# maxgillett/tinysplat

Measured on AMD Instinct MI355X. Metric: Gaussians*pixels/s fwd+bwd, higher is better.
Workload: dtype f32; 1 GPU; 1000000 random Gaussians, SH degree 3, 1920x1080, fwd+bwd (RGB), BASELINE configs[2]; max_per_tile=614, parallelism=single GPU, tile_lists=16x16 (gsplat's) (auto), gaussian_order=as generated (i.i.d.)

## Files before the change

### include/tinysplat_hip.h

```cpp
#ifndef TINYSPLAT_HIP_H
#define TINYSPLAT_HIP_H

#include <stdint.h>

#ifdef __cplusplus
extern "C" {
#endif

#define TS_ABI_VERSION 8

#define TS_E_BADARG (-1)
#define TS_E_DEGREE (-2)

#define TS_TILE 16
#define TS_SPLAT_RECORD_FLOATS 12
#define TS_PARTIAL_ROW_FLOATS 12

int ts_abi_version(void);

typedef struct ts_camera {
    float fx, fy, cx, cy;
    int32_t img_width, img_height;
    int32_t tile_bounds_x, tile_bounds_y;
    int32_t tile_row0, tile_rows;
    float glob_scale;
    float clip_thresh;
    int32_t wide_tiles;
    int32_t hints;
} ts_camera;
#define TS_HINT_BALANCED_WALK 1
#define TS_HINT_COOP_SPLIT (1 << 20)
#define TS_CAM_LIST_SEGMENTS(s) (((s) & 15) << 8)
#define TS_CAM_WHOLE_TILES(w16) (((w16) & 15) << 12)
#define TS_CAM_COOP_TILES(c16) (((c16) & 15) << 16)
int64_t ts_final_floats(const ts_camera* cam_host, int32_t channels);
int32_t ts_cut_tiles(const ts_camera* cam_host, int32_t* band, int32_t* whole);
int32_t ts_num_tiles(const ts_camera* cam_host);


#define TS_PROJECT_LOG_SCALES 1
#define TS_PROJECT_RAW_QUATS 2

int ts_project_fwd(int32_t n, const float* means3d, const float* scales, const float* quats,
                   const float* viewmat, const float* projmat, const ts_camera* cam_host,
                   int32_t flags, float* xys, float* depths, int32_t* radii, float* conics,
                   int32_t* num_tiles_hit, float* cov3d, void* stream);

int ts_project_bwd(int32_t n, const float* means3d, const float* scales, const float* quats,
                   const float* viewmat, const float* projmat, const ts_camera* cam_host,
                   int32_t flags, const int32_t* radii, const float* v_xy, const float* v_depth,
                   const float* v_conic, const float* v_cov3d,
                   float* v_means3d, float* v_scales, float* v_quats, void* stream);


int ts_sh_fwd(int32_t n, int32_t degrees_to_use, int32_t num_bases, const float* viewdirs,
              const float* coeffs, float* colors, void* stream);

int ts_sh_bwd(int32_t n, int32_t degrees_to_use, int32_t num_bases, const float* viewdirs,
              const float* v_colors, float* v_coeffs, void* stream);

int ts_sh_colors_fwd(int32_t n, int32_t degrees_to_use, int32_t num_bases, const float* means3d,
                     const float* origin, const float* colors_dc, const float* colors_rest,
                     float* colors, uint8_t* clamp_mask, const int32_t* live, void* stream);
int ts_sh_colors_bwd(int32_t n, int32_t degrees_to_use, int32_t num_bases, const float* means3d,
                     const float* origin, const uint8_t* clamp_mask, const float* v_colors,
                     float* v_colors_dc, float* v_colors_rest, void* stream);
int ts_colors_pack_fwd(int32_t n, int32_t degrees_to_use, int32_t num_bases, const float* means3d,
                       const float* origin, const float* colors_dc, const float* colors_rest,
                       uint8_t* clamp_mask, const int32_t* live, int32_t channels, int32_t flags,
                       const float* xys, const int32_t* radii, const float* conics, const float* opacity,
                       const int32_t* cum_tiles_hit, const ts_camera* cam_host, const float* depths,
                       float* splats, void* stream);


int64_t ts_scan_ws_ints(int32_t n);
int ts_scan_tiles(int32_t n, const int32_t* num_tiles_hit, int32_t* cum_tiles_hit,
                  int32_t* scan_ws, int32_t* total_out, void* stream);

int64_t ts_bin_ws_ints(int32_t n, int32_t num_tiles);

int ts_bin_count(int32_t n, const float* xys, const int32_t* radii, const float* splats,
                 const ts_camera* cam_host, int32_t* bin_ws, void* stream);

int ts_tile_offsets(int32_t n, int32_t num_tiles, int32_t* bin_ws, int32_t* tile_bins,
                    const int32_t* cum_tiles_hit, int64_t capacity, void* stream);
int ts_tile_offsets_stats(int32_t n, int32_t num_tiles, int32_t* bin_ws, int32_t* tile_bins,
                          const int32_t* cum_tiles_hit, int64_t capacity, int32_t* longest_list, void* stream);

int ts_bin_scatter(int32_t n, const float* xys, const int32_t* radii, const float* splats,
                   const ts_camera* cam_host, const int32_t* bin_ws, int32_t* bucket_ids, int32_t* scratch,
                   void* stream);

int ts_sort_tiles(int32_t num_tiles, const int32_t* tile_bins, const float* depths,
                  const int32_t* bucket_ids, int32_t* gaussian_ids_sorted, int32_t* sort_ws,
                  int32_t* zeroed_counter, void* stream);
int ts_sort_tiles_above(int32_t num_tiles, const int32_t* tile_bins, const float* depths,
                        const int32_t* bucket_ids, int32_t* gaussian_ids_sorted, int32_t* sort_ws,
                        int32_t* zeroed_counter, void* stream);

int32_t ts_bin_group_form(int32_t n);
int ts_bin_count_groups(int32_t n, const float* xys, const int32_t* radii, const float* splats,
                        const ts_camera* cam_host, int32_t* bin_ws, void* stream);
int ts_group_offsets(int32_t n, int32_t num_tiles, int32_t* bin_ws, int32_t* tile_bins,
                     const int32_t* cum_tiles_hit, int64_t capacity, int32_t* longest_list, void* stream);
int ts_bin_scatter_groups(int32_t n, const float* xys, const int32_t* radii, const float* splats,
                          const ts_camera* cam_host, int32_t* bin_ws, int32_t* tile_bins, int32_t* bucket_ids,
                          int32_t* scratch, void* stream);
int32_t ts_bin_one_walk_form(int32_t n, int32_t num_tiles);
int32_t ts_bin_stage_capacity(void);
int ts_bin_emit_groups(int32_t n, const float* xys, const int32_t* radii, const float* splats,
                       const ts_camera* cam_host, const int32_t* cum_tiles_hit, int64_t capacity, int32_t* bin_ws,
                       int32_t* scratch, void* stream);
int ts_emit_offsets(int32_t n, int32_t num_tiles, int32_t* bin_ws, int32_t* tile_bins,
                    const int32_t* cum_tiles_hit, int64_t capacity, int32_t* longest_list, void* stream);
int ts_bin_gather_groups(int32_t n, int32_t num_tiles, int32_t* bin_ws, int32_t* tile_bins, int32_t* bucket_ids,
                         const int32_t* scratch, void* stream);
int ts_sort_tiles_stats(int32_t num_tiles, const int32_t* tile_bins, const float* depths,
                        const int32_t* bucket_ids, int32_t* gaussian_ids_sorted, int32_t* sort_ws,
                        int32_t* zeroed_counter, int32_t n, const int32_t* bin_ws, int32_t* longest_list,
                        void* stream);
int ts_sort_tiles_above_stats(int32_t num_tiles, const int32_t* tile_bins, const float* depths,
                              const int32_t* bucket_ids, int32_t* gaussian_ids_sorted, int32_t n,
                              const int32_t* bin_ws, int32_t* longest_list, void* stream);

#define TS_RASTER_LOGIT_OPACITY 1

int ts_pack_splats(int32_t n, int32_t channels, int32_t flags, const float* xys, const int32_t* radii,
                   const float* conics, const float* colors, const float* opacity,
                   const int32_t* cum_tiles_hit, const ts_camera* cam_host, const float* depths,
                   float* splats, void* stream);

#define TS_RASTER_CLAMP_RGB 2
#define TS_RASTER_SPLIT_BLOCKS 4
#define TS_RASTER_NARROW_WAVES 8
#define TS_RASTER_FLAG_GEN(g) (((g) & 0xff) << 8)
int ts_raster_fwd(int32_t channels, int32_t flags, const ts_camera* cam_host, const int32_t* tile_bins,
                  const int32_t* gaussian_ids_sorted, const float* splats, const float* background,
                  float* out_img, float* final_Ts, int32_t* final_index, uint8_t* clamp_mask,
                  void* stream);
int ts_raster_fwd_planes(int32_t channels, int32_t flags, const ts_camera* cam_host, const int32_t* tile_bins,
                         const int32_t* gaussian_ids_sorted, const float* splats, const float* background,
                         float* out_img, float* out_depth, float* final_Ts, int32_t* final_index,
                         uint8_t* clamp_mask, void* stream);

int ts_raster_fwd_sort(int32_t channels, int32_t flags, const ts_camera* cam_host, const int32_t* tile_bins,
                       const int32_t* bucket_ids, const float* depths, int32_t* gaussian_ids_sorted,
                       const float* splats, const float* background, float* out_img, float* out_depth,
                       float* final_Ts, int32_t* final_index, uint8_t* clamp_mask, void* stream);

int ts_raster_bwd(int32_t channels, int32_t flags, int64_t num_intersects, const ts_camera* cam_host,
                  const int32_t* tile_bins, const int32_t* gaussian_ids_sorted, const float* splats,
                  const float* background, const float* final_Ts, const int32_t* final_index,
                  const float* v_out_img, const float* v_out_alpha, const uint8_t* clamp_mask,
                  float* partials, uint8_t* row_flags, void* stream);
int ts_raster_bwd_planes(int32_t channels, int32_t flags, int64_t num_intersects, const ts_camera* cam_host,
                         const int32_t* tile_bins, const int32_t* gaussian_ids_sorted, const float* splats,
                         const float* background, const float* final_Ts, const int32_t* final_index,
                         const float* v_out_img, const float* v_out_depth, int32_t planes,
                         const float* v_out_alpha, const uint8_t* clamp_mask,
                         float* partials, uint8_t* row_flags, void* stream);

int ts_reduce_partials(int32_t n, int32_t channels, int32_t flags, const int32_t* num_tiles_hit,
                       const int32_t* cum_tiles_hit, const float* partials,
                       const uint8_t* row_flags, const float* splats, float* v_xy, float* v_conic,
                       float* v_colors, float* v_opacity, float* v_depth, const uint8_t* color_mask,
                       void* stream);

#define TS_FRAME_TIGHT 1
#define TS_FRAME_SPLIT 2
#define TS_FRAME_NARROW_WAVES 8
#define TS_FRAME_DIRECT_SCATTER 32
#define TS_FRAME_PLANES 64
#define TS_FRAME_LIST_STATS 256
#define TS_FRAME_SEPARATE_SORT 128
#define TS_FRAME_STRIPE 16
#define TS_FRAME_GROUP_COUNTS 1024
#define TS_FRAME_ONE_WALK 2048
#define TS_FRAME_SURVIVORS 512
typedef struct ts_frame {
    int32_t n, num_bases, sh_degree, channels, flags;
    int32_t flag_gen;
    ts_camera cam;
    const float *means, *scales, *quats, *opacities, *colors_dc, *colors_rest;
    const float *view34, *projview, *origin, *background;
    float *xys, *depths, *conics, *colors, *splats;
    int32_t *radii, *num_tiles_hit, *cum_tiles_hit;
    uint8_t* sh_mask;
    int32_t *scan_ws, *bin_ws, *tile_bins;
    int32_t* total_host;
    int64_t num_intersects;
    int64_t capacity;
    int32_t *bucket_ids, *gaussian_ids_sorted;
    float *out_img, *final_Ts;
    int32_t* final_index;
    uint8_t* clamp_mask;
    const float* v_out_img;
    float* partials;
    uint8_t* row_flags;
    float *v_xy, *v_conic, *v_colors, *v_depth, *v_opacity;
    float *v_means, *v_scales, *v_quats, *v_colors_dc, *v_colors_rest;
    float* out_depth;
    const float* v_out_depth;
    int32_t* survivors;
} ts_frame;
int32_t ts_frame_struct_bytes(void);
int ts_frame_fwd_project(const ts_frame* f, void* stream);
int ts_frame_fwd_prepare(const ts_frame* f, void* stream);
int ts_frame_fwd_composite(const ts_frame* f, void* stream);
int ts_frame_bwd_composite(const ts_frame* f, void* stream);
int ts_frame_bwd_params(const ts_frame* f, void* stream);

typedef void (*ts_entry_probe)(const char* entry, int32_t end, void* user);
int ts_set_entry_probe(ts_entry_probe fn, void* user);

#define TS_MAX_RANKS 16
#define TS_EXPORT_RECORD_FLOATS 16
typedef struct ts_stripes {
    int32_t num;
    int32_t row[TS_MAX_RANKS + 1];
} ts_stripes;
int64_t ts_route_ws_ints(int32_t n, int32_t num_ranks);
int ts_route_count(int32_t n, const float* xys, const int32_t* radii, const ts_camera* cam_host,
                   const ts_stripes* stripes_host, int32_t* route_ws, int32_t* counts, void* stream);
int ts_route_count_padded(int32_t n, const float* xys, const int32_t* radii, const ts_camera* cam_host,
                          const ts_stripes* stripes_host, const int32_t* group_base_host, int32_t* route_ws,
                          int32_t* counts, void* stream);
int ts_route_pack(int32_t n, int32_t gid_base, const float* xys, const int32_t* radii, const float* depths,
                  const float* splats, const ts_camera* cam_host, const ts_stripes* stripes_host,
                  const int32_t* route_ws, float* records, void* stream);
int ts_import_records(int32_t m, const float* records, const ts_camera* cam_host, float* xys, float* depths,
                      int32_t* radii, int32_t* num_tiles_hit, void* stream);
int ts_import_pack(int32_t m, const float* records, const int32_t* cum_tiles_hit, const ts_camera* cam_host,
                   float* splats, void* stream);
int ts_reduce_partials_rows(int32_t n, int32_t channels, int32_t flags, const int32_t* num_tiles_hit,
                            const int32_t* cum_tiles_hit, const float* partials, const uint8_t* row_flags,
                            const float* splats, float* grad_rows, void* stream);
int ts_route_accumulate(int32_t n, int32_t channels, const float* xys, const int32_t* radii, const float* splats,
                        const uint8_t* color_mask, const ts_camera* cam_host, const ts_stripes* stripes_host,
                        const int32_t* route_ws, const float* grad_rows, float* v_xy, float* v_conic,
                        float* v_colors, float* v_depth, float* v_opacity, void* stream);

int ts_shard_owner_fwd(const ts_frame* fo, const ts_stripes* stripes_host, int32_t* route_ws, int32_t* counts,
                       void* stream);
int ts_shard_owner_fwd_padded(const ts_frame* fo, const ts_stripes* stripes_host, const int32_t* group_base_host,
                              int32_t* route_ws, int32_t* counts, void* stream);
int ts_shard_owner_fwd_fused(int32_t n, int32_t degrees_to_use, int32_t num_bases, const float* means3d,
                             const float* scales, const float* quats, const float* view34, const float* projview,
                             const ts_camera* cam_host, int32_t project_flags, const float* origin,
                             const float* colors_dc, const float* colors_rest, const float* opacity, int32_t channels,
                             int32_t raster_flags, float* xys, float* depths, int32_t* radii, float* conics,
                             int32_t* num_tiles_hit, uint8_t* clamp_mask, float* splats, const ts_stripes* stripes_host,
                             const int32_t* group_base_host, int32_t* route_ws, int32_t* counts, void* stream);
int ts_shard_owner_bwd_fused(int32_t n, int32_t channels, int32_t degrees_to_use, int32_t num_bases, const float* means3d,
                             const float* scales, const float* quats, const float* view34, const float* projview,
                             const float* origin, const float* xys, const int32_t* radii, const float* splats,
                             const uint8_t* color_mask, const ts_camera* cam_host, const ts_stripes* stripes_host,
                             const int32_t* route_ws, const float* grad_rows, float* v_xy, float* v_conic,
                             float* v_colors, float* v_depth, float* v_opacity, float* v_colors_dc, float* v_colors_rest,
                             float* v_means3d, float* v_scales, float* v_quats, void* stream);
int ts_shard_stripe_fwd_import(const ts_frame* fs, const float* records, void* stream);
int ts_shard_stripe_bwd(const ts_frame* fs, float* grad_rows, void* stream);
int ts_shard_owner_bwd(const ts_frame* fo, const ts_stripes* stripes_host, const int32_t* route_ws,
                       const float* grad_rows, void* stream);

typedef struct ts_rank_step {
    ts_stripes stripes;
    int32_t group_base[TS_MAX_RANKS + 1];
    int32_t gid_base;
    int32_t send_rows, recv_rows;
    int32_t* route_ws;
    int32_t* counts;
    float *send, *recv;
    float *grad_rows, *back;
} ts_rank_step;
int32_t ts_rank_step_struct_bytes(void);
int ts_shard_rank_fwd_a(const ts_frame* fo, const ts_rank_step* r, void* stream);
int ts_shard_rank_fwd_b(const ts_frame* fs, const ts_rank_step* r, void* stream);
int ts_shard_rank_bwd_a(const ts_frame* fs, const ts_rank_step* r, void* stream);
int ts_shard_rank_bwd_b(const ts_frame* fo, const ts_rank_step* r, void* stream);


int64_t ts_photometric_ws_floats(int32_t height, int32_t width);
int ts_photometric_loss_rgbd(int32_t height, int32_t width, int32_t pixel_floats, const float* image,
                             const float* target, const float* depth_target, float w_l1,
                             float w_ssim, float w_depth, float* ws, float* v_image, void* stream);
int ts_photometric_loss(int32_t height, int32_t width, const float* image, const float* target,
                        float w_l1, float w_ssim, float* ws, float* v_image, void* stream);
int ts_photometric_loss_planes(int32_t height, int32_t width, const float* image, const float* depth,
                               const float* target, const float* depth_target, float w_l1, float w_ssim,
                               float w_depth, float* ws, float* v_image, float* v_depth, void* stream);
int ts_photometric_loss_reduce(int32_t height, int32_t width, float w_l1, float w_ssim, float w_depth,
                               const float* ws, float* out4, void* stream);

#define TS_ADAM_MAX_TENSORS 8
int ts_adam_step(int32_t num_tensors, float* const* params_host, const float* const* grads_host,
                 float* const* exp_avg_host, float* const* exp_avg_sq_host, const int64_t* numel_host,
                 const float* lr_host, const int32_t* steps_host, float beta1, float beta2, float eps,
                 void* stream);

#define TS_ADAM_MEANS 0
#define TS_ADAM_COLORS_DC 1
#define TS_ADAM_COLORS_REST 2
#define TS_ADAM_SCALES 3
#define TS_ADAM_QUATS 4
#define TS_ADAM_OPACITIES 5
typedef struct ts_adam {
    float* exp_avg[6];
    float* exp_avg_sq[6];
    float lr[6];
    int32_t step[6];
    float beta1, beta2, eps;
} ts_adam;
int ts_sh_colors_bwd_adam(int32_t n, int32_t degrees_to_use, int32_t num_bases, const float* means3d,
                          const float* origin, const uint8_t* clamp_mask, const float* v_colors,
                          float* colors_dc, float* colors_rest, const ts_adam* adam_host, void* stream);
int ts_project_bwd_adam(int32_t n, float* means3d, float* scales, float* quats, const float* viewmat,
                        const float* projmat, const ts_camera* cam_host, int32_t flags, const int32_t* radii,
                        const float* v_xy, const float* v_depth, const float* v_conic, float* opacities,
                        const float* v_opacity, const ts_adam* adam_host, void* stream);
int ts_frame_bwd_params_adam(const ts_frame* f, const ts_adam* adam_host, void* stream);

#define TS_DENSIFY_CLONE 1
#define TS_DENSIFY_SPLIT 2
#define TS_DENSIFY_PRUNE 4

typedef struct ts_densify_policy {
    float interval_densify;
    float max_dim;
    float tau_means;
    float scale_thresh;
} ts_densify_policy;

int ts_grad_accum(int32_t n, const float* v_xy, float* accum, void* stream);

int ts_densify_classify(int32_t n, const float* accum, const float* scales, const float* opacities,
                        const ts_densify_policy* policy, uint8_t* flags, void* stream);

int64_t ts_densify_ws_ints(int32_t n);
int ts_densify_plan(int32_t n, const uint8_t* flags, int32_t* ws, int32_t* counts, int32_t* src_of,
                    void* stream);

#define TS_GATHER_MAX_TENSORS 8
int ts_gather_rows(int32_t num_tensors, const float* const* src_host, float* const* dst_host,
                   const int32_t* row_floats_host, int32_t dst_rows, int32_t copy_rows,
                   const int32_t* src_of, void* stream);

int ts_split_fixup(int32_t rows, const int32_t* src_of_split, const float* means, const float* scales,
                   const float* quats, const float* z, float* means_out, float* scales_out,
                   void* stream);

int32_t ts_ply_row_floats(int32_t k_rest);
int ts_ply_pack_rows(int32_t n, int32_t k_rest, const float* means, const float* colors_dc,
                     const float* colors_rest, const float* opacities, const float* scales,
                     const float* quats, float* rows, void* stream);
int ts_ply_unpack_rows(int32_t n, int32_t k_rest, const float* rows, float* means, float* colors_dc,
                       float* colors_rest, float* opacities, float* scales, float* quats,
// ... 171 lines not shown
```

### tinysplat_amd/_lib.py

```python
from __future__ import annotations

import ctypes
import os
from ctypes import POINTER, c_double, c_float, c_int32, c_int64, c_void_p
from pathlib import Path

LIB_PATH = Path(os.environ["TS_LIB_PATH"]) if os.environ.get("TS_LIB_PATH") else \
    Path(__file__).resolve().parent / "csrc" / "libtinysplat_hip.so"
ABI_VERSION = 8
HINT_BALANCED_WALK = 1
HINT_COOP_SPLIT = 1 << 20
RASTER_LOGIT_OPACITY = 1
RASTER_CLAMP_RGB = 2
RASTER_SPLIT_BLOCKS = 4
RASTER_NARROW_WAVES = 8
FRAME_TIGHT = 1
FRAME_SPLIT = 2
FRAME_NARROW_WAVES = 8
FRAME_STRIPE = 16
FRAME_DIRECT_SCATTER = 32
FRAME_PLANES = 64
FRAME_SEPARATE_SORT = 128
FRAME_LIST_STATS = 256
FRAME_SURVIVORS = 512
FRAME_GROUP_COUNTS = 1024
FRAME_ONE_WALK = 2048
PARTIAL_ROW_FLOATS = 12


class TsCamera(ctypes.Structure):
    _fields_ = [
        ("fx", c_float), ("fy", c_float), ("cx", c_float), ("cy", c_float),
        ("img_width", c_int32), ("img_height", c_int32),
        ("tile_bounds_x", c_int32), ("tile_bounds_y", c_int32),
        ("tile_row0", c_int32), ("tile_rows", c_int32),
        ("glob_scale", c_float), ("clip_thresh", c_float),
        ("wide_tiles", c_int32), ("hints", c_int32),
    ]


_P = c_void_p
_CAM = POINTER(TsCamera)


class TsDensifyPolicy(ctypes.Structure):
    _fields_ = [("interval_densify", c_float), ("max_dim", c_float), ("tau_means", c_float),
                ("scale_thresh", c_float)]


class TsFrame(ctypes.Structure):
    _fields_ = ([("n", c_int32), ("num_bases", c_int32), ("sh_degree", c_int32), ("channels", c_int32),
                 ("flags", c_int32), ("flag_gen", c_int32), ("cam", TsCamera)]
                + [(name, c_void_p) for name in (
                    "means", "scales", "quats", "opacities", "colors_dc", "colors_rest",
                    "view34", "projview", "origin", "background",
                    "xys", "depths", "conics", "colors", "splats",
                    "radii", "num_tiles_hit", "cum_tiles_hit", "sh_mask",
                    "scan_ws", "bin_ws", "tile_bins", "total_host")]
                + [("num_intersects", c_int64), ("capacity", c_int64)]
                + [(name, c_void_p) for name in (
                    "bucket_ids", "gaussian_ids_sorted", "out_img", "final_Ts", "final_index", "clamp_mask",
                    "v_out_img", "partials", "row_flags",
                    "v_xy", "v_conic", "v_colors", "v_depth", "v_opacity",
                    "v_means", "v_scales", "v_quats", "v_colors_dc", "v_colors_rest",
                    "out_depth", "v_out_depth", "survivors")])


_FRAME = POINTER(TsFrame)


class TsAdam(ctypes.Structure):
    _fields_ = [("exp_avg", c_void_p * 6), ("exp_avg_sq", c_void_p * 6), ("lr", c_float * 6), ("step", c_int32 * 6),
                ("beta1", c_float), ("beta2", c_float), ("eps", c_float)]


_ADAM = POINTER(TsAdam)

MAX_RANKS = 16


class TsStripes(ctypes.Structure):
    _fields_ = [("num", c_int32), ("row", c_int32 * (MAX_RANKS + 1))]


_STRIPES = POINTER(TsStripes)


class TsRankStep(ctypes.Structure):
    _fields_ = [("stripes", TsStripes), ("group_base", c_int32 * (MAX_RANKS + 1)), ("gid_base", c_int32),
                ("send_rows", c_int32), ("recv_rows", c_int32), ("route_ws", c_void_p), ("counts", c_void_p),
                ("send", c_void_p), ("recv", c_void_p), ("grad_rows", c_void_p), ("back", c_void_p)]


_RANK = POINTER(TsRankStep)

TSDF_NO_CULL = 1
TSDF_PLANES = 6


class TsTsdfCamera(ctypes.Structure):
    _fields_ = [("view", c_float * 12), ("proj", c_float * 12), ("planes", c_float * (TSDF_PLANES * 5)),
                ("width", c_int32), ("height", c_int32), ("depth", c_void_p)]

ENTRY_PROBE = ctypes.CFUNCTYPE(None, ctypes.c_char_p, c_int32, c_void_p)

SIGNATURES = {
    "ts_abi_version": (c_int32, []),
    "ts_project_fwd": (c_int32, [c_int32, _P, _P, _P, _P, _P, _CAM, c_int32, _P, _P, _P, _P, _P, _P, _P]),
    "ts_project_bwd": (c_int32, [c_int32, _P, _P, _P, _P, _P, _CAM, c_int32, _P, _P, _P, _P, _P, _P, _P, _P, _P]),
    "ts_sh_fwd": (c_int32, [c_int32, c_int32, c_int32, _P, _P, _P, _P]),
    "ts_sh_bwd": (c_int32, [c_int32, c_int32, c_int32, _P, _P, _P, _P]),
    "ts_sh_colors_fwd": (c_int32, [c_int32, c_int32, c_int32, _P, _P, _P, _P, _P, _P, _P, _P]),
    "ts_sh_colors_bwd": (c_int32, [c_int32, c_int32, c_int32, _P, _P, _P, _P, _P, _P, _P]),
    "ts_scan_ws_ints": (c_int64, [c_int32]),
    "ts_scan_tiles": (c_int32, [c_int32, _P, _P, _P, _P, _P]),
    "ts_bin_ws_ints": (c_int64, [c_int32, c_int32]),
    "ts_bin_count": (c_int32, [c_int32, _P, _P, _P, _CAM, _P, _P]),
    "ts_tile_offsets": (c_int32, [c_int32, c_int32, _P, _P, _P, c_int64, _P]),
    "ts_tile_offsets_stats": (c_int32, [c_int32, c_int32, _P, _P, _P, c_int64, _P, _P]),
    "ts_bin_scatter": (c_int32, [c_int32, _P, _P, _P, _CAM, _P, _P, _P, _P]),
    "ts_sort_tiles": (c_int32, [c_int32, _P, _P, _P, _P, _P, _P, _P]),
    "ts_sort_tiles_above": (c_int32, [c_int32, _P, _P, _P, _P, _P, _P, _P]),
    "ts_bin_group_form": (c_int32, [c_int32]),
    "ts_bin_count_groups": (c_int32, [c_int32, _P, _P, _P, _CAM, _P, _P]),
    "ts_group_offsets": (c_int32, [c_int32, c_int32, _P, _P, _P, c_int64, _P, _P]),
    "ts_bin_scatter_groups": (c_int32, [c_int32, _P, _P, _P, _CAM, _P, _P, _P, _P, _P]),
    "ts_bin_one_walk_form": (c_int32, [c_int32, c_int32]),
    "ts_bin_stage_capacity": (c_int32, []),
    "ts_bin_emit_groups": (c_int32, [c_int32, _P, _P, _P, _CAM, _P, c_int64, _P, _P, _P]),
    "ts_emit_offsets": (c_int32, [c_int32, c_int32, _P, _P, _P, c_int64, _P, _P]),
    "ts_bin_gather_groups": (c_int32, [c_int32, c_int32, _P, _P, _P, _P, _P]),
    "ts_sort_tiles_stats": (c_int32, [c_int32, _P, _P, _P, _P, _P, _P, c_int32, _P, _P, _P]),
    "ts_sort_tiles_above_stats": (c_int32, [c_int32, _P, _P, _P, _P, c_int32, _P, _P, _P]),
    "ts_num_tiles": (c_int32, [_CAM]),
    "ts_final_floats": (c_int64, [_CAM, c_int32]),
    "ts_cut_tiles": (c_int32, [_CAM, _P, _P]),
    "ts_colors_pack_fwd": (c_int32, [c_int32, c_int32, c_int32, _P, _P, _P, _P, _P, _P, c_int32, c_int32,
                                     _P, _P, _P, _P, _P, _CAM, _P, _P, _P]),
    "ts_pack_splats": (c_int32, [c_int32, c_int32, c_int32, _P, _P, _P, _P, _P, _P, _CAM, _P, _P, _P]),
    "ts_raster_fwd": (c_int32, [c_int32, c_int32, _CAM, _P, _P, _P, _P, _P, _P, _P, _P, _P]),
    "ts_raster_bwd": (c_int32, [c_int32, c_int32, c_int64, _CAM, _P, _P, _P, _P, _P, _P, _P, _P, _P, _P, _P, _P]),
    "ts_raster_fwd_planes": (c_int32, [c_int32, c_int32, _CAM, _P, _P, _P, _P, _P, _P, _P, _P, _P, _P]),
    "ts_raster_fwd_sort": (c_int32, [c_int32, c_int32, _CAM, _P, _P, _P, _P, _P, _P, _P, _P, _P, _P, _P, _P]),
    "ts_raster_bwd_planes": (c_int32, [c_int32, c_int32, c_int64, _CAM, _P, _P, _P, _P, _P, _P, _P, _P, c_int32,
                                       _P, _P, _P, _P, _P]),
    "ts_bench_stream_read": (c_int32, [_P, c_int64, _P, _P]),
    "ts_bench_gather48": (c_int32, [_P, _P, c_int64, _P, _P]),
    "ts_photometric_ws_floats": (c_int64, [c_int32, c_int32]),
    "ts_photometric_loss": (c_int32, [c_int32, c_int32, _P, _P, c_float, c_float, _P, _P, _P]),
    "ts_photometric_loss_rgbd": (c_int32, [c_int32, c_int32, c_int32, _P, _P, _P, c_float, c_float, c_float, _P, _P, _P]),
    "ts_photometric_loss_planes": (c_int32, [c_int32, c_int32, _P, _P, _P, _P, c_float, c_float, c_float, _P, _P, _P,
                                             _P]),
    "ts_photometric_loss_reduce": (c_int32, [c_int32, c_int32, c_float, c_float, c_float, _P, _P, _P]),
    "ts_adam_step": (c_int32, [c_int32, _P, _P, _P, _P, _P, _P, _P, c_float, c_float, c_float, _P]),
    "ts_sh_colors_bwd_adam": (c_int32, [c_int32, c_int32, c_int32, _P, _P, _P, _P, _P, _P, _ADAM, _P]),
    "ts_project_bwd_adam": (c_int32, [c_int32, _P, _P, _P, _P, _P, _CAM, c_int32, _P, _P, _P, _P, _P, _P, _ADAM, _P]),
    "ts_frame_bwd_params_adam": (c_int32, [_FRAME, _ADAM, _P]),
    "ts_grad_accum": (c_int32, [c_int32, _P, _P, _P]),
    "ts_densify_classify": (c_int32, [c_int32, _P, _P, _P, POINTER(TsDensifyPolicy), _P, _P]),
    "ts_densify_ws_ints": (c_int64, [c_int32]),
    "ts_densify_plan": (c_int32, [c_int32, _P, _P, _P, _P, _P]),
    "ts_gather_rows": (c_int32, [c_int32, _P, _P, _P, c_int32, c_int32, _P, _P]),
    "ts_split_fixup": (c_int32, [c_int32, _P, _P, _P, _P, _P, _P, _P, _P]),
    "ts_ply_row_floats": (c_int32, [c_int32]),
    "ts_ply_pack_rows": (c_int32, [c_int32, c_int32, _P, _P, _P, _P, _P, _P, _P, _P]),
    "ts_ply_unpack_rows": (c_int32, [c_int32, c_int32, _P, _P, _P, _P, _P, _P, _P, _P]),
    "ts_reduce_partials": (c_int32, [c_int32, c_int32, c_int32, _P, _P, _P, _P, _P, _P, _P, _P, _P, _P, _P, _P]),
    "ts_route_ws_ints": (c_int64, [c_int32, c_int32]),
    "ts_route_count": (c_int32, [c_int32, _P, _P, _CAM, _STRIPES, _P, _P, _P]),
    "ts_route_count_padded": (c_int32, [c_int32, _P, _P, _CAM, _STRIPES, _P, _P, _P, _P]),
    "ts_route_pack": (c_int32, [c_int32, c_int32, _P, _P, _P, _P, _CAM, _STRIPES, _P, _P, _P]),
    "ts_import_records": (c_int32, [c_int32, _P, _CAM, _P, _P, _P, _P, _P]),
    "ts_import_pack": (c_int32, [c_int32, _P, _P, _CAM, _P, _P]),
    "ts_reduce_partials_rows": (c_int32, [c_int32, c_int32, c_int32, _P, _P, _P, _P, _P, _P, _P]),
    "ts_route_accumulate": (c_int32, [c_int32, c_int32, _P, _P, _P, _P, _CAM, _STRIPES, _P, _P, _P, _P, _P, _P, _P, _P]),
    "ts_shard_owner_fwd": (c_int32, [_FRAME, _STRIPES, _P, _P, _P]),
    "ts_shard_owner_fwd_padded": (c_int32, [_FRAME, _STRIPES, _P, _P, _P, _P]),
    "ts_shard_owner_fwd_fused": (c_int32, [c_int32, c_int32, c_int32, _P, _P, _P, _P, _P, _CAM, c_int32, _P, _P, _P, _P,
                                           c_int32, c_int32, _P, _P, _P, _P, _P, _P, _P, _STRIPES, _P, _P, _P, _P]),
    "ts_shard_owner_bwd_fused": (c_int32, [c_int32, c_int32, c_int32, c_int32, _P, _P, _P, _P, _P, _P, _P, _P, _P, _P,
                                           _CAM, _STRIPES, _P, _P, _P, _P, _P, _P, _P, _P, _P, _P, _P, _P, _P]),
    "ts_shard_stripe_fwd_import": (c_int32, [_FRAME, _P, _P]),
    "ts_shard_stripe_bwd": (c_int32, [_FRAME, _P, _P]),
    "ts_shard_owner_bwd": (c_int32, [_FRAME, _STRIPES, _P, _P, _P]),
    "ts_rank_step_struct_bytes": (c_int32, []),
    "ts_shard_rank_fwd_a": (c_int32, [_FRAME, _RANK, _P]),
    "ts_shard_rank_fwd_b": (c_int32, [_FRAME, _RANK, _P]),
    "ts_shard_rank_bwd_a": (c_int32, [_FRAME, _RANK, _P]),
    "ts_shard_rank_bwd_b": (c_int32, [_FRAME, _RANK, _P]),
    "ts_frame_struct_bytes": (c_int32, []),
    "ts_frame_fwd_project": (c_int32, [_FRAME, _P]),
    "ts_frame_fwd_prepare": (c_int32, [_FRAME, _P]),
    "ts_frame_fwd_composite": (c_int32, [_FRAME, _P]),
    "ts_frame_bwd_composite": (c_int32, [_FRAME, _P]),
    "ts_frame_bwd_params": (c_int32, [_FRAME, _P]),
    "ts_set_entry_probe": (c_int32, [_P, _P]),
    "ts_knn_ws_bytes": (c_int64, [c_int32, c_int32, c_int32]),
    "ts_knn": (c_int32, [c_int32, _P, c_int32, _P, c_int32, _P, _P, _P, _P, _P]),
    "ts_init_from_points": (c_int32, [c_int32, c_int32, _P, _P, _P, _P, _P, _P, _P, _P, _P, _P, _P, _P, _P, _P]),
    "ts_opacity_entropy_ws_bytes": (c_int64, [c_int32]),
    "ts_opacity_entropy": (c_int32, [c_int32, _P, _P, _P, _P, _P]),
    "ts_density_sample_ws_bytes": (c_int64, [c_int32]),
    "ts_density_sample": (c_int32, [c_int32, c_int32, c_int32, _P, _P, _P, _P, _P, _P, _P, _P, _P, _P, _P]),
    "ts_density_loss_ws_bytes": (c_int64, [c_int32]),
    "ts_density_loss": (c_int32, [c_int32, c_int32, _P, _P, _P, _P, _P, _P, _P, _P, c_int32, c_int32, _P, _P, c_int32,
                                  c_float, _P, _P, _P, _P, _P, _P, _P, _P, _P, _P]),
    "ts_segment_sum_ws_bytes": (c_int64, [c_int64, c_int32]),
    "ts_segment_sum": (c_int32, [c_int64, c_int32, c_int32, _P, _P, _P, _P, _P, _P, _P]),
    "ts_extract_pack": (c_int32, [c_int32, _P, _P, _P, _P, _P, _P, _P]),
    "ts_extract_rays": (c_int32, [c_int32, _P, c_int32, c_int32, _P, c_int32, _P, _P, _P, _P, _P, _P]),
    "ts_extract_samples": (c_int32, [c_int32, c_int32, c_int32, c_float, _P, _P, _P, _P, _P, _P, _P]),
    "ts_extract_march": (c_int32, [c_int32, c_int32, c_int32, c_float, c_float, _P, _P, _P, _P, _P, _P, _P, _P, _P, _P,
                                   _P, _P, _P]),
    "ts_extract_normals": (c_int32, [c_int32, c_int32, _P, _P, _P, _P, _P]),
    "ts_extract_chunk_bytes": (c_int64, [c_int32, c_int32, c_int32]),
    "ts_mesh_boxes": (c_int32, [c_int32, _P, _P, _P, c_float, _P, _P]),
    "ts_mesh_mark": (c_int32, [c_int32, _P, _P, _P, _P, _P]),
    "ts_mesh_chunk_bytes": (c_int64, [c_int32, c_int32]),
    "ts_mesh_corners": (c_int32, [c_int32, _P, _P, _P, _P, _P]),
    "ts_mesh_density": (c_int32, [c_int32, c_int32, _P, _P, _P, _P, _P, _P, _P, _P]),
    "ts_mesh_count": (c_int32, [c_int32, _P, _P, _P, c_float, _P, _P, _P]),
    "ts_mesh_emit": (c_int32, [c_int32, _P, _P, _P, c_float, _P, _P, _P, _P, _P, _P]),
    "ts_tsdf_camera_bytes": (c_int32, []),
    "ts_tsdf_mark": (c_int32, [c_int32, _P, c_int64, _P, _P, c_float, c_float, _P, _P]),
    "ts_tsdf_chunk_bytes": (c_int64, [c_int32]),
    "ts_tsdf_integrate": (c_int32, [c_int32, _P, _P, _P, _P, c_int32, c_int32, c_float, c_float, c_float, c_int32, _P, _P,
                                    _P]),
    "ts_tsdf_field": (c_int32, [c_int32, _P, _P, c_int32, _P, _P]),
    "ts_mesh_count_observed": (c_int32, [c_int32, _P, _P, _P, c_float, _P, _P, _P]),
    "ts_mesh_emit_observed": (c_int32, [c_int32, _P, _P, _P, c_float, _P, _P, _P, _P, _P, _P]),
    "ts_field_colors": (c_int32, [c_int32, c_int32, _P, _P, _P, _P, _P, _P, c_int32, c_int32, _P, _P]),
    "ts_simplify_count": (c_int32, [c_int32, c_int32, _P, _P, _P, _P, _P, _P]),
    "ts_simplify_keys": (c_int32, [c_int32, _P, _P, _P, _P, _P]),
    "ts_simplify_ws_bytes": (c_int64, [c_int64]),
    "ts_simplify_accumulate": (c_int32, [c_int32, c_int32, c_int32, _P, _P, _P, _P, c_int32, c_int64, _P, _P, c_int64,
                                         c_int64, _P, _P, _P]),
    "ts_simplify_solve": (c_int32, [c_int32, _P, _P, _P, _P, _P, c_double, _P, _P]),
    "ts_simplify_faces": (c_int32, [c_int32, c_int32, _P, _P, _P, _P, _P]),
    "ts_clean_degenerate": (c_int32, [c_int32, _P, _P, _P]),
    "ts_clean_edge_keys": (c_int32, [c_int32, c_int32, _P, _P, _P]),
    "ts_clean_face_weights": (c_int32, [c_int32, c_int32, _P, _P, _P, _P]),
    "ts_clean_mark": (c_int32, [c_int32, c_int64, _P, _P, _P, _P]),
    "ts_clean_components": (c_int32, [c_int32, c_int32, _P, _P, _P, _P]),
    "ts_splat_keys": (c_int32, [c_int32, _P, _P, _P, _P]),
    "ts_splat_pack": (c_int32, [c_int32, c_int32, _P, _P, _P, _P, _P, _P, _P, _P]),
    "ts_splat_unpack": (c_int32, [c_int32, _P, _P, _P, _P, _P, _P, _P]),
    "ts_undistort_image": (c_int32, [_P, c_int32, c_int32, POINTER(c_float), POINTER(c_float), POINTER(c_float),
                                     c_int32, c_int32, c_int32, _P, _P]),
    "ts_jpeg_ws_bytes": (c_int64, [c_int32, c_int32, c_int32, c_int32]),
    "ts_jpeg_max_bytes": (c_int64, [c_int32, c_int32, c_int32, c_int32]),
    "ts_jpeg_header": (c_int64, [c_int32, c_int32, c_int32, c_int32, c_int32, _P, c_int64]),
    "ts_jpeg_encode": (c_int32, [_P, c_int32, c_int32, c_int32, c_int32, c_int32, c_int32, c_int32, _P, _P, c_int64, _P,
                                 _P, _P]),
    "ts_image_metrics_ws_bytes": (c_int64, [c_int32, c_int32]),
    "ts_image_metrics": (c_int32, [c_int32, c_int32, c_int32, _P, _P, c_int32, _P, _P, _P]),
    "ts_depth_prior_project": (c_int32, [c_int32, c_int64, c_int64, _P, _P, _P, _P, _P, _P, _P, _P, _P, _P]),
    "ts_depth_prior_mark": (c_int32, [c_int64, _P, _P, _P]),
    "ts_depth_prior_gather": (c_int32, [c_int64, _P, _P, _P, _P, _P, _P, _P, _P, _P, _P, _P, _P, _P, _P]),
    "ts_depth_prior_fit": (c_int32, [c_int32, _P, _P, _P, _P, c_int32, _P, _P]),
    "ts_depth_prior_apply": (c_int32, [_P, c_int32, c_int32, c_int32, c_int32, _P, c_int32, _P, _P]),
    "ts_label_votes": (c_int32, [c_int32, _CAM, _P, _P, _P, _P, _P, c_int32, _P, _P]),
    "ts_votes_labels": (c_int32, [c_int32, c_int32, _P, c_double, _P, _P, _P]),
}

_lib = None


class HipLibraryError(RuntimeError):
    pass


def load() -> ctypes.CDLL:
    global _lib
    if _lib is not None:
        return _lib
    if not LIB_PATH.exists():
        raise HipLibraryError(
            f"{LIB_PATH} is missing: tinysplat_amd has no CPU or PyTorch fallback. "
            "Build it with `python -m tinysplat_amd._build` (needs hipcc, targets gfx950).")
    stamp = LIB_PATH.with_suffix(LIB_PATH.suffix + ".flags")
    if stamp.exists() and "-DTS_" in stamp.read_text() and os.environ.get("TS_ALLOW_VARIANT_LIB") != "1":
        raise HipLibraryError(
            f"{LIB_PATH} was built with developer -DTS_* overrides (ablation variant; its results may be "
            "wrong). Rebuild with `python -m tinysplat_amd._build`, or set TS_ALLOW_VARIANT_LIB=1.")
    lib = ctypes.CDLL(str(LIB_PATH))
    for name, (res, args) in SIGNATURES.items():
        try:
            fn = getattr(lib, name)
        except AttributeError as e:
            raise HipLibraryError(f"{LIB_PATH} does not export {name}") from e
        fn.restype = res
# ... 23 lines not shown
```

### tinysplat_amd/csrc/binning.hip

```cpp
#include <hip/hip_runtime.h>

#include "../../include/tinysplat_hip.h"
#include "host_util.h"
#include "pack.h"
#include "splat_math.h"

namespace {

constexpr int kThreads = 256;
constexpr int kScanItems = 4;
constexpr int kScanBlock = kThreads * kScanItems;

__device__ __forceinline__ int wave_inclusive_scan(int v) {
    const int lane = threadIdx.x & 63;
#pragma unroll
    for (int d = 1; d < 64; d <<= 1) {
        const int u = __shfl_up(v, d, 64);
        if (lane >= d) v += u;
    }
    return v;
}

template <int WAVES = 4>
__device__ __forceinline__ int block_inclusive_scan(int v, int* total) {
    __shared__ int wave_sums[WAVES];
    const int lane = threadIdx.x & 63, wave = threadIdx.x >> 6;
    int inc = wave_inclusive_scan(v);
    if (lane == 63) wave_sums[wave] = inc;
    __syncthreads();
    int add = 0, tot = 0;
#pragma unroll
    for (int w = 0; w < WAVES; ++w) {
        const int s = wave_sums[w];
        if (w < wave) add += s;
        tot += s;
    }
    *total = tot;
    __syncthreads();
    return inc + add;
}

__global__ __launch_bounds__(kThreads) void scan_local_kernel(int n, const int* __restrict__ in,
                                                              int* __restrict__ out,
                                                              int* __restrict__ block_sums,
                                                              int* __restrict__ total_out) {
    const int base = blockIdx.x * kScanBlock + threadIdx.x * kScanItems;
    int v[kScanItems];
    int sum = 0;
#pragma unroll
    for (int k = 0; k < kScanItems; ++k) {
        v[k] = (base + k < n) ? in[base + k] : 0;
        sum += v[k];
        v[k] = sum;
    }
    int total;
    const int inc = block_inclusive_scan(sum, &total);
    const int excl = inc - sum;
#pragma unroll
    for (int k = 0; k < kScanItems; ++k)
        if (base + k < n) {
            out[base + k] = v[k] + excl;
            if (total_out && gridDim.x == 1 && base + k == n - 1)
                __hip_atomic_store(total_out, v[k] + excl, __ATOMIC_RELEASE, __HIP_MEMORY_SCOPE_SYSTEM);
        }
    if (threadIdx.x == 0) block_sums[blockIdx.x] = total;
}

__global__ __launch_bounds__(kThreads) void scan_add_kernel(int n, int* __restrict__ out,
                                                            const int* __restrict__ block_sums,
                                                            int* __restrict__ total_out) {
    __shared__ int red[kThreads / 64];
    int part = 0;
    for (int j = threadIdx.x; j < (int)blockIdx.x; j += kThreads) part += block_sums[j];
#pragma unroll
    for (int d = 32; d >= 1; d >>= 1) part += __shfl_xor(part, d, 64);
    if ((threadIdx.x & 63) == 0) red[threadIdx.x >> 6] = part;
    __syncthreads();
    int add = 0;
#pragma unroll
    for (int w = 0; w < kThreads / 64; ++w) add += red[w];
    const int base = blockIdx.x * kScanBlock + threadIdx.x * kScanItems;
#pragma unroll
    for (int k = 0; k < kScanItems; ++k)
        if (base + k < n) {
            const int v = out[base + k] + add;
            if (blockIdx.x != 0) out[base + k] = v;
            if (total_out && base + k == n - 1)
                __hip_atomic_store(total_out, v, __ATOMIC_RELEASE, __HIP_MEMORY_SCOPE_SYSTEM);
        }
}

#ifndef TS_BIN_THREADS
#define TS_BIN_THREADS 1024
#endif
constexpr int kBinThreads = TS_BIN_THREADS;
#ifndef TS_BIN_CHUNK
#define TS_BIN_CHUNK 4096
#endif
constexpr int kBinChunkMin = TS_BIN_CHUNK;
constexpr int kBinMaxChunks = 512;
constexpr int kBinWindowMax = 36864;
constexpr int kBinTargetBlocks = 1;

__host__ __device__ inline int bin_num_chunks(int n) {
    int per = n / 192;
    per = per < 1024 ? 1024 : (per > kBinChunkMin ? kBinChunkMin : per);
    int b = (n + per - 1) / per;
    if (b < 1) b = 1;
    if (b > kBinMaxChunks) b = kBinMaxChunks;
    return b;
}

inline int bin_window_tiles(int n, int num_tiles) {
    const int chunks = bin_num_chunks(n);
    int nwin = (kBinTargetBlocks + chunks - 1) / chunks;
    const int max_win = (num_tiles + 255) / 256;
    if (nwin > max_win) nwin = max_win;
    if (nwin < 1) nwin = 1;
    int window = (num_tiles + nwin - 1) / nwin;
    window = (window + 63) & ~63;
    if (window > kBinWindowMax) window = kBinWindowMax;
    return window;
}

using ts::TightTest;

#ifndef TS_BIN_PRE
#define TS_BIN_PRE 2
#endif
constexpr int kBinPre = TS_BIN_PRE;
template <typename Emit>
__device__ __forceinline__ void walk_chunk(int g0, int g1, const float* __restrict__ xys,
                                           const int* __restrict__ radii,
                                           const float4* __restrict__ splats, const ts_camera& cam,
                                           Emit emit) {
    const int ws = cam.wide_tiles ? 1 : 0;
    const int tbx = (cam.tile_bounds_x + ws) >> ws;
    const bool tight_lists = splats != nullptr;
    for (int base = g0 + threadIdx.x; base < g1; base += kBinPre * kBinThreads) {
        int r[kBinPre];
        float2 xy[kBinPre];
        float4 q0[kBinPre], q1[kBinPre];
#pragma unroll
        for (int u = 0; u < kBinPre; ++u) {
            const int i = base + u * kBinThreads;
            r[u] = i < g1 ? radii[i] : 0;
        }
#pragma unroll
        for (int u = 0; u < kBinPre; ++u) {
            const int i = base + u * kBinThreads;
            xy[u] = make_float2(0.f, 0.f);
            q0[u] = q1[u] = make_float4(0.f, 0.f, 0.f, 0.f);
            if (r[u] > 0) {
                xy[u] = reinterpret_cast<const float2*>(xys)[i];
                if (tight_lists) { q0[u] = splats[3 * (size_t)i]; q1[u] = splats[3 * (size_t)i + 1]; }
            }
        }
// ... 471 lines not shown
struct PassRanks {
    unsigned int r[(ITEMS + 1) / 2];
    __device__ __forceinline__ PassRanks() {
#pragma unroll
        for (int u = 0; u < (ITEMS + 1) / 2; ++u) r[u] = 0u;
    }
    __device__ __forceinline__ void set(int u, int v) { r[u / 2] |= (unsigned int)v << (16 * (u & 1)); }
    __device__ __forceinline__ int get(int u) const { return (int)((r[u / 2] >> (16 * (u & 1))) & 0xffffu); }
};

template <int ITEMS, typename Load>
__device__ __forceinline__ void place_pass(FineGroup& sh, unsigned int* buf, int m, Load load, bool publish,
                                           const GroupLists& g, int* __restrict__ bucket_ids) {
    static_assert(ITEMS * kFineThreads <= 65536, "16-bit ranks inside a pass");
    const int tid = threadIdx.x;
    unsigned int w[ITEMS];
    PassRanks<ITEMS> rank;
#pragma unroll
    for (int u = 0; u < ITEMS; ++u) {
        const int k = u * kFineThreads + tid;
        if (k < m) w[u] = load(k);
    }
#pragma unroll
    for (int u = 0; u < ITEMS; ++u) {
        const int k = u * kFineThreads + tid;
        if (k < m) rank.set(u, atomicAdd(&sh.hist[w[u] >> kCoarseIdBits], 1));
    }
    __syncthreads();
    if (tid < 64) {
        int c;
        const int ex = scan_lists(sh.hist, tid, c);
        if (publish) publish_lists(sh, g, tid, c, ex);
        if (tid < kCoarseTiles) {
            sh.loff[tid] = ex;
            sh.gbase[tid] = sh.cursor[tid];
            sh.cursor[tid] += c;
            sh.hist[tid] = 0;
        }
    }
    __syncthreads();
#pragma unroll
    for (int u = 0; u < ITEMS; ++u) {
        const int k = u * kFineThreads + tid;
        if (k < m) buf[sh.loff[w[u] >> kCoarseIdBits] + rank.get(u)] = w[u];
    }
    __syncthreads();
#pragma unroll
    for (int u = 0; u < ITEMS; ++u) {
        const int k = u * kFineThreads + tid;
        if (k < m) {
            const unsigned int e = buf[k];
            const int t = (int)(e >> kCoarseIdBits);
            bucket_ids[sh.gbase[t] + (k - sh.loff[t])] = (int)(e & kCoarseIdMask);
        }
    }
    __syncthreads();
}

__global__ __launch_bounds__(kFineThreads) void bin_scatter_fine_kernel(int num_tiles,
                                                                        const int* __restrict__ tile_start,
                                                                        const int* __restrict__ scratch,
                                                                        int* __restrict__ bucket_ids) {
    __shared__ FineGroup sh;
    __shared__ unsigned int buf[kFinePass];
    const int t0 = blockIdx.x << kCoarseShift, t1 = min(num_tiles, t0 + kCoarseTiles);
    if ((int)threadIdx.x < t1 - t0) sh.cursor[threadIdx.x] = tile_start[t0 + threadIdx.x];
    const int begin = tile_start[t0], end = tile_start[t1];
    if ((int)threadIdx.x < kCoarseTiles) sh.hist[threadIdx.x] = 0;
    __syncthreads();
    for (int c0 = begin; c0 < end; c0 += kFinePass)
        place_pass<kFineAhead>(sh, buf, min(kFinePass, end - c0),
                               [&](int k) { return (unsigned int)scratch[c0 + k]; }, false, GroupLists{}, bucket_ids);
}

__global__ __launch_bounds__(kFineThreads) void bin_scatter_fine_groups_kernel(int num_tiles,
                                                                               int* __restrict__ tile_start,
                                                                               int* __restrict__ tile_bins,
                                                                               int* __restrict__ group_max,
                                                                               const int* __restrict__ scratch,
                                                                               int* __restrict__ bucket_ids) {
    if (tile_start[num_tiles + 1] != 0) return;
    __shared__ FineGroup sh;
    __shared__ unsigned int buf[kFinePass];
    const int t0 = blockIdx.x << kCoarseShift, t1 = min(num_tiles, t0 + kCoarseTiles);
    const int begin = tile_start[t0], end = tile_start[t1];
    if ((int)threadIdx.x < kCoarseTiles) {
        sh.hist[threadIdx.x] = 0;
        sh.cursor[threadIdx.x] = 0;
    }
    __syncthreads();
    const GroupLists lists{t0, t1, begin, tile_start, tile_bins, group_max};
    const bool counted = end - begin > kFinePass || end == begin;
    if (counted) {
        for (int c0 = begin; c0 < end; c0 += kFinePass) {
            const int m = min(kFinePass, end - c0);
            unsigned int w[kFineAhead];
#pragma unroll
            for (int u = 0; u < kFineAhead; ++u) {
                const int k = u * kFineThreads + (int)threadIdx.x;
                if (k < m) w[u] = (unsigned int)scratch[c0 + k];
            }
#pragma unroll
            for (int u = 0; u < kFineAhead; ++u) {
                const int k = u * kFineThreads + (int)threadIdx.x;
                if (k < m) atomicAdd(&sh.hist[w[u] >> kCoarseIdBits], 1);
            }
        }
        publish_counted(sh, lists);
    }
    for (int c0 = begin; c0 < end; c0 += kFinePass)
        place_pass<kFineAhead>(sh, buf, min(kFinePass, end - c0),
                               [&](int k) { return (unsigned int)scratch[c0 + k]; }, !counted, lists, bucket_ids);
}

#ifndef TS_STAGE_CAP
#define TS_STAGE_CAP 20480
#endif
constexpr int kStageCap = TS_STAGE_CAP;
constexpr int kEmitMaxGroups = 2048;
static_assert((size_t)kStageCap * 6 + (size_t)kEmitMaxGroups * 8 <= 144 * 1024, "LDS budget of a binning workgroup");
static_assert(kEmitMaxGroups <= 2 * kBinThreads && kEmitMaxGroups <= 65536, "two groups per thread, 16-bit group index");
static_assert(kEmitMaxGroups <= kGoLdsGroups, "the offsets launch keeps the column totals in LDS");

struct BinGeometry {
    int chunks, chunk, groups;
    long long tile_start, guard, spare;
    long long group_totals, group_max;
    long long counts, starts, col_total, rows_end;
};
inline BinGeometry bin_geometry(int n, int num_tiles) {
    const long long nt = num_tiles < 0 ? 0 : num_tiles;
    BinGeometry g;
    g.chunks = bin_num_chunks(n);
    g.chunk = n > 0 ? (n + g.chunks - 1) / g.chunks : 1;
    g.groups = (int)((nt + kCoarseTiles - 1) >> kCoarseShift);
    const long long rows = (long long)g.chunks * g.groups;
    g.tile_start = g.chunks * nt;
    g.guard = g.tile_start + nt + 1;
    g.spare = g.guard + 1;
    g.group_totals = rows;
    g.group_max = nt + 1;
    g.counts = g.group_max + g.groups;
    g.starts = g.counts + rows;
    g.col_total = g.starts + rows;
    g.rows_end = g.col_total + g.groups;
    return g;
}
inline bool one_walk_form(int n, int num_tiles) {
    if (!two_hop(n) || num_tiles <= 0) return false;
    const BinGeometry g = bin_geometry(n, num_tiles);
    return g.groups <= kEmitMaxGroups && g.rows_end <= g.tile_start;
}

__global__ __launch_bounds__(kBinThreads) void bin_scatter_emit_kernel(
    int n, int chunk, const float* __restrict__ xys, const int* __restrict__ radii,
    const float4* __restrict__ splats, const ts_camera cam, int groups, const int* __restrict__ cum,
    long long capacity, int* __restrict__ counts, int* __restrict__ starts, int* __restrict__ scratch) {
    extern __shared__ int lds[];
    __shared__ int staged;
    const int g0 = min(n, (int)blockIdx.x * chunk), g1 = min(n, g0 + chunk);
    const int total = cum[n - 1];
    const int chunk_base = g0 > 0 ? cum[g0 - 1] : 0;
    const int chunk_end = g1 > g0 ? cum[g1 - 1] : chunk_base;
    int* hist = lds;
    int* cursor = lds + groups;
    unsigned int* words = reinterpret_cast<unsigned int*>(lds + 2 * groups);
    unsigned short* grp = reinterpret_cast<unsigned short*>(words + kStageCap);
    const int tid = threadIdx.x;
    for (int j = tid; j < groups; j += kBinThreads) hist[j] = 0;
    if (tid == 0) staged = 0;
    __syncthreads();
    if (total < 0 || (capacity >= 0 && (long long)total > capacity)) return;
    const int room = chunk_end - chunk_base;
    walk_chunk(g0, g1, xys, radii, splats, cam, [&](int t, int i) {
        const int g = t >> kCoarseShift;
        atomicAdd(&hist[g], 1);
        const unsigned long long m = __ballot(1);
        const int rank = (int)__builtin_amdgcn_mbcnt_hi((unsigned int)(m >> 32),
                                                        __builtin_amdgcn_mbcnt_lo((unsigned int)m, 0u));
        int base = 0;
        if (rank == 0) base = atomicAdd(&staged, (int)__popcll(m));
        base = __builtin_amdgcn_readfirstlane(base);
        const int slot = base + rank;
        if (slot < kStageCap) {
            words[slot] = (unsigned int)i | ((unsigned int)(t & (kCoarseTiles - 1)) << kCoarseIdBits);
            grp[slot] = (unsigned short)g;
        }
    });
    __syncthreads();
    const int pairs = staged;
    const bool sound = pairs <= room;
    {
        const int a = 2 * tid;
        const int h0 = a < groups ? hist[a] : 0, h1 = a + 1 < groups ? hist[a + 1] : 0;
        int all;
        const int ex = block_inclusive_scan<kBinThreads / 64>(h0 + h1, &all) - h0 - h1;
        int* crow = counts + (size_t)blockIdx.x * groups;
        int* srow = starts + (size_t)blockIdx.x * groups;
        if (a < groups) {
            cursor[a] = ex;
            crow[a] = sound ? h0 : 0;
            srow[a] = chunk_base + ex;
        }
        if (a + 1 < groups) {
            cursor[a + 1] = ex + h0;
            crow[a + 1] = sound ? h1 : 0;
            srow[a + 1] = chunk_base + ex + h0;
        }
    }
    __syncthreads();
    if (!sound) return;
    int* dst = scratch + chunk_base;
    if (pairs <= kStageCap) {
        constexpr int kPer = kStageCap / kBinThreads;
        static_assert(kStageCap % kBinThreads == 0, "whole staging rounds");
        unsigned int w[kPer];
        int at[kPer];
#pragma unroll
        for (int u = 0; u < kPer; ++u) {
            const int j = u * kBinThreads + tid;
            if (j < pairs) {
                w[u] = words[j];
                at[u] = atomicAdd(&cursor[grp[j]], 1);
            }
        }
        __syncthreads();
#pragma unroll
        for (int u = 0; u < kPer; ++u)
            if (u * kBinThreads + tid < pairs) words[at[u]] = w[u];
        __syncthreads();
#pragma unroll
        for (int u = 0; u < kPer; ++u) {
            const int j = u * kBinThreads + tid;
            if (j < pairs) dst[j] = (int)words[j];
        }
    } else {
        walk_chunk(g0, g1, xys, radii, splats, cam, [&](int t, int i) {
            dst[atomicAdd(&cursor[t >> kCoarseShift], 1)] = i | ((t & (kCoarseTiles - 1)) << kCoarseIdBits);
        });
    }
}

#ifndef TS_RUN_AHEAD
#define TS_RUN_AHEAD 20
#endif
constexpr int kRunItems = TS_RUN_AHEAD;
constexpr int kRunPass = kFineThreads * kRunItems;
#ifndef TS_RUNS_IN_FLIGHT
#define TS_RUNS_IN_FLIGHT 8
#endif
constexpr int kRunAhead = TS_RUNS_IN_FLIGHT;
__global__ __launch_bounds__(kFineThreads) void bin_scatter_fine_runs_kernel(
    int num_tiles, int groups, int chunks, const int* __restrict__ counts, const int* __restrict__ starts,
    int* __restrict__ tile_start, int* __restrict__ tile_bins, int* __restrict__ group_max,
    const int* __restrict__ scratch, int* __restrict__ bucket_ids) {
    extern __shared__ unsigned int buf[];
    const int my_count = (int)threadIdx.x < chunks ? counts[(size_t)threadIdx.x * groups + blockIdx.x] : 0;
    const int my_start = (int)threadIdx.x < chunks ? starts[(size_t)threadIdx.x * groups + blockIdx.x] : 0;
    const int begin = tile_start[min(num_tiles, (int)(blockIdx.x << kCoarseShift))];
    if (tile_start[num_tiles + 1] != 0) return;
    __shared__ FineGroup sh;
    __shared__ int roff[kBinMaxChunks + 1], rsrc[kBinMaxChunks];
    constexpr int kWaves = kFineThreads / 64;
    const int tid = threadIdx.x, lane = tid & 63, wave = tid >> 6;
    const int t0 = blockIdx.x << kCoarseShift, t1 = min(num_tiles, t0 + kCoarseTiles);
    if (tid < kCoarseTiles) {
        sh.hist[tid] = 0;
        sh.cursor[tid] = 0;
    }
    int total;
    {
        const int c = my_count;
        const int inc = block_inclusive_scan<kWaves>(c, &total);
        if (tid < chunks) {
            roff[tid] = inc - c;
            rsrc[tid] = my_start;
        }
        if (tid == 0) roff[chunks] = total;
    }
    __syncthreads();
    auto for_runs = [&](int c0, int m, auto op) {
#pragma unroll 1
        for (int b0 = wave; b0 < chunks; b0 += kWaves * kRunAhead) {
            int len[kRunAhead], src[kRunAhead], dst[kRunAhead];
            unsigned int v[kRunAhead];
#pragma unroll
            for (int u = 0; u < kRunAhead; ++u) {
                const int b = b0 + u * kWaves;
                len[u] = src[u] = dst[u] = 0;
                if (b < chunks) {
                    const int o = roff[b], c = roff[b + 1] - o;
                    const int lo = max(0, c0 - o) + lane;
                    len[u] = min(c, c0 + m - o) - lo;
                    src[u] = rsrc[b] + lo;
                    dst[u] = o - c0 + lo;
                }
            }
#pragma unroll
            for (int u = 0; u < kRunAhead; ++u)
                if (len[u] > 0) v[u] = (unsigned int)scratch[src[u]];
#pragma unroll
            for (int u = 0; u < kRunAhead; ++u)
                if (len[u] > 0) op(dst[u], v[u]);
#pragma unroll
            for (int u = 0; u < kRunAhead; ++u)
                for (int j = 64; j < len[u]; j += 64) op(dst[u] + j, (unsigned int)scratch[src[u] + j]);
        }
    };
    const GroupLists lists{t0, t1, begin, tile_start, tile_bins, group_max};
    const bool counted = total > kRunPass || total == 0;
    if (counted) {
        for_runs(0, total, [&](int, unsigned int w) { atomicAdd(&sh.hist[w >> kCoarseIdBits], 1); });
        publish_counted(sh, lists);
    }
    for (int c0 = 0; c0 < total; c0 += kRunPass) {
        const int m = min(kRunPass, total - c0);
        for_runs(c0, m, [&](int k, unsigned int w) { buf[k] = w; });
        __syncthreads();
        place_pass<kRunItems>(sh, buf, m, [&](int k) { return buf[k]; }, !counted, lists, bucket_ids);
    }
}

struct ListStats {
    const int* group_max;
    const int* guard;
    int* longest_out;
    int groups;
};
__device__ __forceinline__ void store_longest(const ListStats& st) {
    __shared__ int longest;
    if (threadIdx.x == 0) longest = 0;
    __syncthreads();
    int m = 0;
    for (int g = threadIdx.x; g < st.groups; g += kThreads) m = max(m, st.group_max[g]);
#pragma unroll
    for (int d = 32; d >= 1; d >>= 1) m = max(m, __shfl_xor(m, d, 64));
    if ((threadIdx.x & 63) == 0) atomicMax(&longest, m);
    __syncthreads();
    if (threadIdx.x == 0 && *st.guard == 0) *st.longest_out = longest;
}

constexpr int kSortCap = 4096;

#include "sort_network.h"

struct IdKeyArray {
    volatile int* ids;
    const float* depths;
};

__device__ __forceinline__ void cmpswap(IdKeyArray a, int i, int j) {
    const int x = a.ids[i], y = a.ids[j];
    if (make_key(a.depths, x) > make_key(a.depths, y)) { a.ids[i] = y; a.ids[j] = x; }
}

template <typename Ptr>
__device__ __forceinline__ void bitonic_network(Ptr a, int n) {
    int lg = 0;
    while ((1 << lg) < n) ++lg;
    const int half = (1 << lg) >> 1;
    for (int lk = 1; lk <= lg; ++lk) {
        const int k = 1 << lk, hk = k >> 1;
        for (int p = threadIdx.x; p < half; p += kThreads) {
            const int base = (p >> (lk - 1)) << lk, off = p & (hk - 1);
            const int i = base + off, j = base + k - 1 - off;
            if (j < n) cmpswap(a, i, j);
        }
        __syncthreads();
        for (int ld = lk - 2; ld >= 0; --ld) {
            const int d = 1 << ld;
            for (int p = threadIdx.x; p < half; p += kThreads) {
                const int i = ((p >> ld) << (ld + 1)) | (p & (d - 1)), j = i + d;
                if (j < n) cmpswap(a, i, j);
            }
            __syncthreads();
        }
    }
}

template <int E>
__device__ __forceinline__ void sort_tile_regs(const int* g, const float* __restrict__ depths,
                                               int* out, int n, unsigned long long* lds) {
    const int t = threadIdx.x;
    unsigned long long k[E];
#pragma unroll
    for (int e = 0; e < E; ++e) {
        const int i = t * E + e;
        k[e] = i < n ? make_key(depths, g[i]) : ~0ull;
    }
    __syncthreads();
    bitonic_regs<E, kThreads>(k, t, min(pow2_at_least(n), kThreads * E), lds);
// ... 190 lines not shown
        c0 = colors[3 * i]; c1 = colors[3 * i + 1]; c2 = colors[3 * i + 2];
        if (a.channels == 4) c3 = a.depths[i];
    }
    ts::pack_one(a, i, c0, c1, c2, c3);
}

}

extern "C" {

int32_t ts_num_tiles(const ts_camera* cam) {
    if (!cam) return 0;
    const int tbx = cam->wide_tiles ? (cam->tile_bounds_x + 1) / 2 : cam->tile_bounds_x;
    return cam->tile_rows * tbx;
}

int64_t ts_scan_ws_ints(int32_t n) {
    return n <= 0 ? 1 : (int64_t)((n + kScanBlock - 1) / kScanBlock);
}

int ts_scan_tiles(int32_t n, const int32_t* num_tiles_hit, int32_t* cum_tiles_hit,
                  int32_t* scan_ws, int32_t* total_out, void* stream) {
    if (n < 0) return TS_E_BADARG;
    if (n == 0) return 0;
    if (!num_tiles_hit || !cum_tiles_hit || !scan_ws) return TS_E_BADARG;
    hipStream_t s = (hipStream_t)stream;
    const int nb = (n + kScanBlock - 1) / kScanBlock;
    hipLaunchKernelGGL(scan_local_kernel, dim3(nb), dim3(kThreads), 0, s, n, num_tiles_hit,
                       cum_tiles_hit, scan_ws, total_out);
    if (nb > 1)
        hipLaunchKernelGGL(scan_add_kernel, dim3(nb), dim3(kThreads), 0, s, n, cum_tiles_hit, scan_ws,
                           total_out);
    return launch_status();
}

int64_t ts_bin_ws_ints(int32_t n, int32_t num_tiles) { return bin_geometry(n, num_tiles).spare + 1; }

int ts_bin_count(int32_t n, const float* xys, const int32_t* radii, const float* splats,
                 const ts_camera* cam, int32_t* bin_ws, void* stream) {
    if (n < 0 || !cam || !bin_ws) return TS_E_BADARG;
    const int nt = ts_num_tiles(cam);
    if (nt <= 0) return 0;
    if (n > 0 && (!xys || !radii)) return TS_E_BADARG;
    const BinGeometry g = bin_geometry(n, nt);
    const int window = bin_window_tiles(n, nt);
    const int windows = (nt + window - 1) / window;
    const size_t lds = (size_t)window * sizeof(int);
    if (lds > 64 * 1024)
        (void)hipFuncSetAttribute(reinterpret_cast<const void*>(&bin_count_kernel),
                                  hipFuncAttributeMaxDynamicSharedMemorySize, (int)lds);
    hipLaunchKernelGGL(bin_count_kernel, dim3(g.chunks, windows), dim3(kBinThreads), lds,
                       (hipStream_t)stream, n, g.chunk, xys, radii,
                       reinterpret_cast<const float4*>(splats), *cam, nt, window, bin_ws);
    return launch_status();
}

int ts_tile_offsets(int32_t n, int32_t num_tiles, int32_t* bin_ws, int32_t* tile_bins,
                    const int32_t* cum_tiles_hit, int64_t capacity, void* stream) {
    return ts_tile_offsets_stats(n, num_tiles, bin_ws, tile_bins, cum_tiles_hit, capacity, nullptr, stream);
}

int ts_tile_offsets_stats(int32_t n, int32_t num_tiles, int32_t* bin_ws, int32_t* tile_bins,
                          const int32_t* cum_tiles_hit, int64_t capacity, int32_t* longest_list, void* stream) {
    if (n < 0 || num_tiles < 0) return TS_E_BADARG;
    if (num_tiles == 0) return 0;
    if (!bin_ws || !tile_bins) return TS_E_BADARG;
    const BinGeometry g = bin_geometry(n, num_tiles);
    int* tile_total = bin_ws + g.tile_start;
    const int per_group = (g.chunks + kScanGroups - 1) / kScanGroups;
    hipStream_t s = (hipStream_t)stream;
    hipLaunchKernelGGL(column_scan_kernel, dim3((num_tiles + kColTiles - 1) / kColTiles),
                       dim3(kColTiles * kScanGroups), 0, s, num_tiles, g.chunks, per_group, bin_ws, tile_total, true);
    hipLaunchKernelGGL(tile_offsets_kernel, dim3(1), dim3(kOffsetsThreads), 0, s, num_tiles, tile_total,
                       tile_bins, bin_ws + g.spare,
                       (cum_tiles_hit && n > 0) ? cum_tiles_hit + (n - 1) : nullptr, (long long)capacity, longest_list);
    return launch_status();
}

int32_t ts_bin_group_form(int32_t n) { return two_hop(n) ? 1 : 0; }

int ts_bin_count_groups(int32_t n, const float* xys, const int32_t* radii, const float* splats,
                        const ts_camera* cam, int32_t* bin_ws, void* stream) {
    if (!cam || !bin_ws || !xys || !radii || !two_hop(n)) return TS_E_BADARG;
    const int nt = ts_num_tiles(cam);
    if (nt <= 0) return 0;
    const BinGeometry g = bin_geometry(n, nt);
    hipLaunchKernelGGL(group_bin_count_kernel, dim3(g.chunks), dim3(kBinThreads), (size_t)g.groups * sizeof(int),
                       (hipStream_t)stream, n, g.chunk, xys, radii, reinterpret_cast<const float4*>(splats), *cam,
                       g.groups, bin_ws);
    return launch_status();
}

}

namespace {
template <bool BASES>
int group_offsets(const BinGeometry& g, int num_tiles, int* bin_ws, int* tile_bins, const int* total_ptr,
                  long long capacity, int* longest_list, hipStream_t s) {
    int* counts = bin_ws + (BASES ? 0 : g.counts);
    int* col_total = nullptr;
    if ((long long)g.chunks * g.groups > kGoSingleMax || g.groups > kGoLdsGroups) {
        col_total = bin_ws + (BASES ? g.group_totals : g.col_total);
        const int per_group = (g.chunks + kScanGroups - 1) / kScanGroups;
        hipLaunchKernelGGL(column_scan_kernel, dim3((g.groups + kColTiles - 1) / kColTiles),
                           dim3(kColTiles * kScanGroups), 0, s, g.groups, g.chunks, per_group, counts, col_total, BASES);
        counts = nullptr;
    }
    hipLaunchKernelGGL(group_tile_offsets_kernel<BASES>, dim3(1), dim3(kGoThreads), 0, s, num_tiles, g.groups, g.chunks,
                       counts, (const int*)col_total, bin_ws + g.tile_start, tile_bins, bin_ws + g.spare, total_ptr,
                       capacity, longest_list);
    return launch_status();
}
}

extern "C" {

int ts_group_offsets(int32_t n, int32_t num_tiles, int32_t* bin_ws, int32_t* tile_bins,
                     const int32_t* cum_tiles_hit, int64_t capacity, int32_t* longest_list, void* stream) {
    if (num_tiles < 0 || !two_hop(n)) return TS_E_BADARG;
    if (num_tiles == 0) return 0;
    if (!bin_ws || !tile_bins) return TS_E_BADARG;
    return group_offsets<true>(bin_geometry(n, num_tiles), num_tiles, bin_ws, tile_bins,
                               cum_tiles_hit ? cum_tiles_hit + (n - 1) : nullptr, (long long)capacity, longest_list,
                               (hipStream_t)stream);
}

int ts_bin_scatter_groups(int32_t n, const float* xys, const int32_t* radii, const float* splats,
                          const ts_camera* cam, int32_t* bin_ws, int32_t* tile_bins, int32_t* bucket_ids,
                          int32_t* scratch, void* stream) {
    if (!cam || !xys || !radii || !bin_ws || !tile_bins || !bucket_ids || !scratch || !two_hop(n))
        return TS_E_BADARG;
    const int nt = ts_num_tiles(cam);
    if (nt <= 0) return 0;
    const BinGeometry g = bin_geometry(n, nt);
    int* tile_start = bin_ws + g.tile_start;
    hipStream_t s = (hipStream_t)stream;
    const auto coarse = (cam->hints & TS_HINT_BALANCED_WALK) ? bin_scatter_coarse_kernel<true, true>
                                                             : bin_scatter_coarse_kernel<false, true>;
    hipLaunchKernelGGL(coarse, dim3(g.chunks), dim3(kBinThreads), (size_t)g.groups * sizeof(int), s, n, g.chunk, xys,
                       radii, reinterpret_cast<const float4*>(splats), *cam, nt, (const int*)bin_ws,
                       (const int*)tile_start, scratch);
    hipLaunchKernelGGL(bin_scatter_fine_groups_kernel, dim3(g.groups), dim3(kFineThreads), 0, s, nt, tile_start,
                       tile_bins, bin_ws + g.group_max, (const int*)scratch, bucket_ids);
    return launch_status();
}

int32_t ts_bin_one_walk_form(int32_t n, int32_t num_tiles) { return one_walk_form(n, num_tiles) ? 1 : 0; }

int32_t ts_bin_stage_capacity(void) { return kStageCap; }

int ts_bin_emit_groups(int32_t n, const float* xys, const int32_t* radii, const float* splats,
                       const ts_camera* cam, const int32_t* cum_tiles_hit, int64_t capacity, int32_t* bin_ws,
                       int32_t* scratch, void* stream) {
    if (!cam || !xys || !radii || !cum_tiles_hit || !bin_ws || !scratch) return TS_E_BADARG;
    const int nt = ts_num_tiles(cam);
    if (!one_walk_form(n, nt) || (cam->hints & TS_HINT_BALANCED_WALK)) return TS_E_BADARG;
    const BinGeometry g = bin_geometry(n, nt);
    const size_t lds = (size_t)g.groups * 8 + (size_t)kStageCap * 6;
    (void)hipFuncSetAttribute(reinterpret_cast<const void*>(&bin_scatter_emit_kernel),
                              hipFuncAttributeMaxDynamicSharedMemorySize, (int)lds);
    hipLaunchKernelGGL(bin_scatter_emit_kernel, dim3(g.chunks), dim3(kBinThreads), lds, (hipStream_t)stream, n, g.chunk,
                       xys, radii, reinterpret_cast<const float4*>(splats), *cam, g.groups, cum_tiles_hit,
                       (long long)capacity, bin_ws + g.counts, bin_ws + g.starts, scratch);
    return launch_status();
}

int ts_emit_offsets(int32_t n, int32_t num_tiles, int32_t* bin_ws, int32_t* tile_bins,
                    const int32_t* cum_tiles_hit, int64_t capacity, int32_t* longest_list, void* stream) {
    if (!one_walk_form(n, num_tiles) || !bin_ws || !tile_bins || !cum_tiles_hit) return TS_E_BADARG;
    return group_offsets<false>(bin_geometry(n, num_tiles), num_tiles, bin_ws, tile_bins, cum_tiles_hit + (n - 1),
                                (long long)capacity, longest_list, (hipStream_t)stream);
}

int ts_bin_gather_groups(int32_t n, int32_t num_tiles, int32_t* bin_ws, int32_t* tile_bins, int32_t* bucket_ids,
                         const int32_t* scratch, void* stream) {
    if (!one_walk_form(n, num_tiles) || !bin_ws || !tile_bins || !bucket_ids || !scratch) return TS_E_BADARG;
    const BinGeometry g = bin_geometry(n, num_tiles);
    const size_t lds = (size_t)kRunPass * sizeof(int);
    (void)hipFuncSetAttribute(reinterpret_cast<const void*>(&bin_scatter_fine_runs_kernel),
                              hipFuncAttributeMaxDynamicSharedMemorySize, (int)lds);
    hipLaunchKernelGGL(bin_scatter_fine_runs_kernel, dim3(g.groups), dim3(kFineThreads), lds, (hipStream_t)stream,
                       num_tiles, g.groups, g.chunks, (const int*)(bin_ws + g.counts), (const int*)(bin_ws + g.starts),
                       bin_ws + g.tile_start, tile_bins, bin_ws + g.group_max, scratch, bucket_ids);
    return launch_status();
}

int ts_bin_scatter(int32_t n, const float* xys, const int32_t* radii, const float* splats,
                   const ts_camera* cam, const int32_t* bin_ws, int32_t* bucket_ids, int32_t* scratch,
                   void* stream) {
    if (n < 0 || !cam) return TS_E_BADARG;
    if (n == 0) return 0;
    if (!xys || !radii || !bin_ws || !bucket_ids) return TS_E_BADARG;
    const int nt = ts_num_tiles(cam);
    if (nt <= 0) return 0;
    const BinGeometry g = bin_geometry(n, nt);
    const int* tile_start = bin_ws + g.tile_start;
    hipStream_t s = (hipStream_t)stream;
    if (scratch && two_hop(n)) {
        const auto coarse = (cam->hints & TS_HINT_BALANCED_WALK) ? bin_scatter_coarse_kernel<true, false>
                                                                 : bin_scatter_coarse_kernel<false, false>;
        hipLaunchKernelGGL(coarse, dim3(g.chunks), dim3(kBinThreads), (size_t)g.groups * sizeof(int), s, n, g.chunk, xys,
                           radii, reinterpret_cast<const float4*>(splats), *cam, nt, bin_ws, tile_start, scratch);
        hipLaunchKernelGGL(bin_scatter_fine_kernel, dim3(g.groups), dim3(kFineThreads), 0, s, nt, tile_start,
                           (const int*)scratch, bucket_ids);
        return launch_status();
    }
    const int window = bin_window_tiles(n, nt);
    const int windows = (nt + window - 1) / window;
    const size_t lds = (size_t)window * sizeof(int);
    if (lds > 64 * 1024)
        (void)hipFuncSetAttribute(reinterpret_cast<const void*>(&bin_scatter_kernel),
                                  hipFuncAttributeMaxDynamicSharedMemorySize, (int)lds);
    hipLaunchKernelGGL(bin_scatter_kernel, dim3(g.chunks, windows), dim3(kBinThreads), lds, s, n, g.chunk, xys, radii,
                       reinterpret_cast<const float4*>(splats), *cam, nt, window, bin_ws, tile_start, bucket_ids);
    return launch_status();
}

}

namespace {
inline bool list_stats(int n, int num_tiles, const int32_t* bin_ws, int32_t* longest_list, ListStats* st) {
    *st = ListStats{nullptr, nullptr, nullptr, 0};
    if (!longest_list) return true;
    if (!bin_ws || !two_hop(n) || num_tiles <= 0) return false;
    const BinGeometry g = bin_geometry(n, num_tiles);
    *st = ListStats{bin_ws + g.group_max, bin_ws + g.guard, longest_list, g.groups};
    return true;
}
}

extern "C" {

int ts_sort_tiles(int32_t num_tiles, const int32_t* tile_bins, const float* depths,
                  const int32_t* bucket_ids, int32_t* gaussian_ids_sorted, int32_t* sort_ws,
                  int32_t* zeroed_counter, void* stream) {
    return ts_sort_tiles_stats(num_tiles, tile_bins, depths, bucket_ids, gaussian_ids_sorted, sort_ws, zeroed_counter,
                               0, nullptr, nullptr, stream);
}

int ts_sort_tiles_stats(int32_t num_tiles, const int32_t* tile_bins, const float* depths,
                        const int32_t* bucket_ids, int32_t* gaussian_ids_sorted, int32_t* sort_ws,
                        int32_t* zeroed_counter, int32_t n, const int32_t* bin_ws, int32_t* longest_list,
                        void* stream) {
    if (num_tiles < 0) return TS_E_BADARG;
    if (num_tiles == 0) return 0;
    if (!tile_bins || !depths || !bucket_ids || !gaussian_ids_sorted || !sort_ws) return TS_E_BADARG;
    ListStats stats;
    if (!list_stats(n, num_tiles, bin_ws, longest_list, &stats)) return TS_E_BADARG;
    hipStream_t s = (hipStream_t)stream;
    int32_t* counter = zeroed_counter ? zeroed_counter : sort_ws;
    int32_t* list = zeroed_counter ? sort_ws : sort_ws + 1;
    if (!zeroed_counter) {
        hipError_t e = hipMemsetAsync(sort_ws, 0, sizeof(int32_t), s);
        if (e != hipSuccess) return (int)e;
    }
    hipLaunchKernelGGL(sort_tiles_small_kernel, dim3((num_tiles + kThreads / 64 - 1) / (kThreads / 64)),
                       dim3(kThreads), 0, s, (int)num_tiles, tile_bins, depths, bucket_ids,
                       gaussian_ids_sorted, counter, list, stats);
    hipLaunchKernelGGL(sort_tiles_mid_kernel, dim3(num_tiles), dim3(kThreads), 0, s, tile_bins, depths,
                       bucket_ids, gaussian_ids_sorted, (int*)nullptr, (int*)nullptr);
    const int grid = num_tiles < 768 ? num_tiles : 768;
    hipLaunchKernelGGL(sort_tiles_large_kernel, dim3(grid), dim3(kThreads), 0, s, tile_bins, depths,
                       bucket_ids, gaussian_ids_sorted, counter, list);
    return launch_status();
}

int ts_sort_tiles_above(int32_t num_tiles, const int32_t* tile_bins, const float* depths,
                        const int32_t* bucket_ids, int32_t* gaussian_ids_sorted, int32_t* sort_ws,
                        int32_t* zeroed_counter, void* stream) {
    (void)sort_ws; (void)zeroed_counter;
    return ts_sort_tiles_above_stats(num_tiles, tile_bins, depths, bucket_ids, gaussian_ids_sorted, 0, nullptr, nullptr,
                                     stream);
}

int ts_sort_tiles_above_stats(int32_t num_tiles, const int32_t* tile_bins, const float* depths,
                              const int32_t* bucket_ids, int32_t* gaussian_ids_sorted, int32_t n,
                              const int32_t* bin_ws, int32_t* longest_list, void* stream) {
    if (num_tiles < 0) return TS_E_BADARG;
    if (num_tiles == 0) return 0;
    if (!tile_bins || !depths || !bucket_ids || !gaussian_ids_sorted) return TS_E_BADARG;
    ListStats stats;
    if (!list_stats(n, num_tiles, bin_ws, longest_list, &stats)) return TS_E_BADARG;
    hipLaunchKernelGGL(sort_tiles_above_kernel, dim3(num_tiles), dim3(kThreads), 0, (hipStream_t)stream, tile_bins,
                       depths, bucket_ids, gaussian_ids_sorted, stats);
    return launch_status();
}

int ts_pack_splats(int32_t n, int32_t channels, int32_t flags, const float* xys, const int32_t* radii,
                   const float* conics, const float* colors, const float* opacity,
                   const int32_t* cum_tiles_hit, const ts_camera* cam, const float* depths, float* splats,
                   void* stream) {
    if (n < 0 || !cam || (channels != 3 && channels != 4)) return TS_E_BADARG;
    if (n == 0) return 0;
    if (!xys || !radii || !conics || !colors || !opacity || !cum_tiles_hit || !splats)
        return TS_E_BADARG;
    ts::PackArgs a;
    a.channels = channels; a.flags = (int)flags; a.xys = xys; a.radii = radii; a.conics = conics;
    a.opacity = opacity; a.cum_tiles_hit = cum_tiles_hit; a.depths = depths;
    a.splats = reinterpret_cast<float4*>(splats); a.cam = *cam;
    hipLaunchKernelGGL(pack_splats_kernel, dim3((n + kThreads - 1) / kThreads), dim3(kThreads), 0,
                       (hipStream_t)stream, n, a, colors);
    return launch_status();
}

}
```

### tinysplat_amd/csrc/frame.hip

```cpp
#include <hip/hip_runtime.h>

#include <atomic>
#include <cstdlib>
#if !defined(TS_NO_ROCTX) && __has_include(<rocprofiler-sdk-roctx/roctx.h>)
#include <rocprofiler-sdk-roctx/roctx.h>
#define TS_HAVE_ROCTX 1
#else
#define TS_HAVE_ROCTX 0
#endif

#include "../../include/tinysplat_hip.h"
#include "raster_survivors.h"

struct TsRange {
#if TS_HAVE_ROCTX
    explicit TsRange(const char* name) { roctxRangePush(name); }
    ~TsRange() { roctxRangePop(); }
#else
    explicit TsRange(const char*) {}
#endif
};

static std::atomic<ts_entry_probe> g_probe{nullptr};
static std::atomic<void*> g_probe_user{nullptr};

struct TsEntry {
    explicit TsEntry(const char* label) : fn_(g_probe.load(std::memory_order_relaxed)), label_(label) {
        if (fn_) {
            std::atomic_thread_fence(std::memory_order_acquire);
            user_ = g_probe_user.load(std::memory_order_relaxed);
            fn_(label_, 0, user_);
        }
    }
    ~TsEntry() {
        if (fn_) fn_(label_, 1, user_);
    }
    ts_entry_probe fn_;
    const char* label_;
    void* user_ = nullptr;
};
#define TS_ENTRY(label, call) ((void)TsEntry(label), (call))

#define TS_TRY(call)                 \
    do {                             \
        const int e_ = (call);       \
        if (e_ != 0) return e_;      \
    } while (0)

namespace {
inline bool bad(const ts_frame* f) {
    return !f || f->n < 0 || (f->channels != 3 && f->channels != 4) || f->num_bases < 1;
}
inline int num_tiles(const ts_frame* f) { return ts_num_tiles(&f->cam); }
inline int32_t* mapped_pointer(int32_t* host) {
    static thread_local int32_t* last_host = nullptr;
    static thread_local int32_t* last_dev = nullptr;
    static thread_local int last_device = -1;
    int device = -1;
    if (hipGetDevice(&device) != hipSuccess) return nullptr;
    if (host == last_host && device == last_device) return last_dev;
    void* dev = nullptr;
    if (hipHostGetDevicePointer(&dev, host, 0) != hipSuccess || !dev) {
        (void)hipGetLastError();
        return nullptr;
    }
    last_host = host;
    last_device = device;
    last_dev = static_cast<int32_t*>(dev);
    return last_dev;
}
inline bool segmented(const ts_frame* f) {
    return ((f->cam.hints >> 8) & 15) > 1 && !f->cam.wide_tiles && !(f->flags & TS_FRAME_NARROW_WAVES);
}
inline int bwd_split(const ts_frame* f) {
    return ((f->flags & TS_FRAME_SPLIT) && !segmented(f)) ? TS_RASTER_SPLIT_BLOCKS : 0;
}
inline int small_n_fused() {
    static const int v = [] {
        const char* e = getenv("TS_SMALL_N_FUSED");
        return e ? atoi(e) : 262144;
    }();
    return v;
}
inline bool survivors(const ts_frame* f) {
    return (f->flags & TS_FRAME_SURVIVORS) && f->survivors && f->final_Ts && f->num_intersects > 0 &&
           f->cam.wide_tiles == 0 &&
           !(f->flags & (TS_FRAME_SPLIT | TS_FRAME_NARROW_WAVES | TS_FRAME_SEPARATE_SORT));
}
enum class ListForm { direct, matrix, group, one_walk };
inline ListForm list_form(const ts_frame* f) {
    if ((f->flags & TS_FRAME_DIRECT_SCATTER) || !ts_bin_group_form(f->n)) return ListForm::direct;
    if (!(f->flags & TS_FRAME_GROUP_COUNTS)) return ListForm::matrix;
    if ((f->flags & TS_FRAME_ONE_WALK) && !(f->cam.hints & TS_HINT_BALANCED_WALK) &&
        ts_bin_one_walk_form(f->n, num_tiles(f)))
        return ListForm::one_walk;
    return ListForm::group;
}
inline const float* tight_records(const ts_frame* f) { return (f->flags & TS_FRAME_TIGHT) ? f->splats : nullptr; }
inline int32_t* longest_word(const ts_frame* f) {
    if ((f->flags & TS_FRAME_LIST_STATS) && f->total_host) {
        int32_t* dev = mapped_pointer(f->total_host);
        if (dev) return dev + 1;
    }
    return nullptr;
}
inline int raster_flags(const ts_frame* f) {
    return TS_RASTER_CLAMP_RGB | ((f->flags & TS_FRAME_SPLIT) ? TS_RASTER_SPLIT_BLOCKS : 0) |
           ((f->flags & TS_FRAME_NARROW_WAVES) ? TS_RASTER_NARROW_WAVES : 0);
}
}

extern "C" {

int32_t ts_frame_struct_bytes(void) { return (int32_t)sizeof(ts_frame); }

int ts_set_entry_probe(ts_entry_probe fn, void* user) {
    g_probe_user.store(user, std::memory_order_relaxed);
    g_probe.store(fn, std::memory_order_release);
    return 0;
}

int ts_frame_fwd_project(const ts_frame* f, void* stream) {
    TsRange range_("ts_frame_fwd_project");
    if (bad(f)) return TS_E_BADARG;
    TS_TRY(TS_ENTRY("ts_project_fwd",
                    ts_project_fwd(f->n, f->means, f->scales, f->quats, f->view34, f->projview, &f->cam, 3, f->xys,
                                   f->depths, f->radii, f->conics, f->num_tiles_hit, nullptr, stream)));
    int32_t* total_dev = f->total_host ? mapped_pointer(f->total_host) : nullptr;
    TS_TRY(TS_ENTRY("ts_scan_tiles",
                    ts_scan_tiles(f->n, f->num_tiles_hit, f->cum_tiles_hit, f->scan_ws, total_dev, stream)));
    if (f->n > 0 && f->total_host && !total_dev) {
        const hipError_t e = hipMemcpyAsync(f->total_host, f->cum_tiles_hit + (f->n - 1), sizeof(int32_t),
                                            hipMemcpyDeviceToHost, (hipStream_t)stream);
        if (e != hipSuccess) return (int)e;
    }
    return 0;
}

int ts_frame_fwd_prepare(const ts_frame* f, void* stream) {
    TsRange range_("ts_frame_fwd_prepare");
    if (bad(f)) return TS_E_BADARG;
    TS_TRY(TS_ENTRY("ts_colors_pack_fwd",
                    ts_colors_pack_fwd(f->n, f->sh_degree, f->num_bases, f->means, f->origin, f->colors_dc,
                                       f->num_bases > 1 ? f->colors_rest : nullptr, f->sh_mask,
                                       (f->flags & TS_FRAME_STRIPE) ? f->num_tiles_hit : nullptr, f->channels,
                                       TS_RASTER_LOGIT_OPACITY, f->xys, f->radii, f->conics, f->opacities,
                                       f->cum_tiles_hit, &f->cam, f->channels == 4 ? f->depths : nullptr, f->splats,
                                       stream)));
    const float* tight = tight_records(f);
    switch (list_form(f)) {
    case ListForm::one_walk:
        return 0;
    case ListForm::group:
        TS_TRY(TS_ENTRY("ts_bin_count",
                        ts_bin_count_groups(f->n, f->xys, f->radii, tight, &f->cam, f->bin_ws, stream)));
        return TS_ENTRY("ts_tile_offsets",
                        ts_group_offsets(f->n, num_tiles(f), f->bin_ws, f->tile_bins, f->cum_tiles_hit, f->capacity,
                                         longest_word(f), stream));
    case ListForm::matrix:
    case ListForm::direct:
        TS_TRY(TS_ENTRY("ts_bin_count", ts_bin_count(f->n, f->xys, f->radii, tight, &f->cam, f->bin_ws, stream)));
        return TS_ENTRY("ts_tile_offsets",
                        ts_tile_offsets_stats(f->n, num_tiles(f), f->bin_ws, f->tile_bins, f->cum_tiles_hit,
                                              f->capacity, longest_word(f), stream));
    }
    return TS_E_BADARG;
}

int ts_frame_fwd_composite(const ts_frame* f, void* stream) {
    TsRange range_("ts_frame_fwd_composite");
    if (bad(f) || f->num_intersects < 0) return TS_E_BADARG;
    const bool planes = (f->flags & TS_FRAME_PLANES) != 0;
    if (planes && (f->channels != 4 || !f->out_depth)) return TS_E_BADARG;
    const bool fused_sort = f->num_intersects > 0 && f->cam.wide_tiles == 0 &&
                            !(f->flags & (TS_FRAME_NARROW_WAVES | TS_FRAME_SEPARATE_SORT));
    const ListForm form = list_form(f);
    const float* tight = tight_records(f);
    const bool listed = f->num_intersects > 0;
    int32_t* scratch = f->gaussian_ids_sorted;
    switch (form) {
    case ListForm::one_walk:
        TS_TRY(TS_ENTRY("ts_bin_scatter",
                        ts_bin_emit_groups(f->n, f->xys, f->radii, tight, &f->cam, f->cum_tiles_hit, f->capacity,
                                           f->bin_ws, scratch, stream)));
        TS_TRY(TS_ENTRY("ts_tile_offsets",
                        ts_emit_offsets(f->n, num_tiles(f), f->bin_ws, f->tile_bins, f->cum_tiles_hit, f->capacity,
                                        longest_word(f), stream)));
        if (listed)
            TS_TRY(TS_ENTRY("ts_bin_scatter",
                            ts_bin_gather_groups(f->n, num_tiles(f), f->bin_ws, f->tile_bins, f->bucket_ids, scratch,
                                                 stream)));
        break;
    case ListForm::group:
        if (listed)
            TS_TRY(TS_ENTRY("ts_bin_scatter",
                            ts_bin_scatter_groups(f->n, f->xys, f->radii, tight, &f->cam, f->bin_ws, f->tile_bins,
                                                  f->bucket_ids, scratch, stream)));
        break;
    case ListForm::matrix:
    case ListForm::direct:
        if (listed)
            TS_TRY(TS_ENTRY("ts_bin_scatter",
                            ts_bin_scatter(f->n, f->xys, f->radii, tight, &f->cam, f->bin_ws, f->bucket_ids,
                                           form == ListForm::matrix ? scratch : nullptr, stream)));
        break;
    }
    if (listed) {
        int32_t* counter = f->bin_ws + (ts_bin_ws_ints(f->n, num_tiles(f)) - 1);
        int32_t* longest = (form == ListForm::group || form == ListForm::one_walk) ? longest_word(f) : nullptr;
        if (fused_sort)
            TS_TRY(TS_ENTRY("ts_sort_tiles",
                            ts_sort_tiles_above_stats(num_tiles(f), f->tile_bins, f->depths, f->bucket_ids,
                                                      f->gaussian_ids_sorted, f->n, f->bin_ws, longest, stream)));
        else
            TS_TRY(TS_ENTRY("ts_sort_tiles",
                            ts_sort_tiles_stats(num_tiles(f), f->tile_bins, f->depths, f->bucket_ids,
                                                f->gaussian_ids_sorted, f->bin_ws, counter, f->n, f->bin_ws, longest,
                                                stream)));
    }
    if (fused_sort)
        return TS_ENTRY("ts_raster_fwd",
                        ts_surv::raster_fwd_sort(f->channels, raster_flags(f), &f->cam, f->tile_bins, f->bucket_ids,
                                                 f->depths, f->gaussian_ids_sorted, f->splats, f->background,
                                                 f->out_img, planes ? f->out_depth : nullptr, f->final_Ts,
                                                 f->final_index, f->clamp_mask, survivors(f) ? f->survivors : nullptr,
                                                 stream));
    return TS_ENTRY("ts_raster_fwd",
                    ts_raster_fwd_planes(f->channels, raster_flags(f), &f->cam, f->tile_bins, f->gaussian_ids_sorted,
                                         f->splats, f->background, f->out_img, planes ? f->out_depth : nullptr,
                                         f->final_Ts, f->final_index, f->clamp_mask, stream));
}

int ts_frame_bwd_composite(const ts_frame* f, void* stream) {
    TsRange range_("ts_frame_bwd_composite");
    if (bad(f) || f->num_intersects < 0) return TS_E_BADARG;
    const bool planes = (f->flags & TS_FRAME_PLANES) != 0;
    const bool surv = survivors(f);
    TS_TRY(TS_ENTRY("ts_raster_bwd",
                    ts_surv::raster_bwd(f->channels,
                                        ((raster_flags(f) & ~(TS_RASTER_CLAMP_RGB | TS_RASTER_SPLIT_BLOCKS)) | bwd_split(f)) |
                                            TS_RASTER_FLAG_GEN(f->flag_gen),
                                        f->num_intersects, &f->cam, f->tile_bins, f->gaussian_ids_sorted, f->splats,
                                        f->background, f->final_Ts, f->final_index, f->v_out_img,
                                        planes ? f->v_out_depth : nullptr, planes ? 1 : 0, nullptr, f->clamp_mask,
                                        f->partials, f->row_flags, surv ? f->bucket_ids : nullptr,
                                        surv ? f->survivors : nullptr, stream)));
    const bool stripe = (f->flags & TS_FRAME_STRIPE) != 0;
    return TS_ENTRY("ts_reduce_partials",
                    ts_reduce_partials(f->n, f->channels,
                                       TS_RASTER_LOGIT_OPACITY | bwd_split(f) | TS_RASTER_FLAG_GEN(f->flag_gen),
                                       f->num_tiles_hit, f->cum_tiles_hit, f->partials, f->row_flags, f->splats,
                                       f->v_xy, f->v_conic, f->v_colors, f->v_opacity,
                                       f->channels == 4 ? f->v_depth : nullptr, stripe ? f->sh_mask : nullptr, stream));
}

int ts_frame_bwd_params(const ts_frame* f, void* stream) {
    TsRange range_("ts_frame_bwd_params");
    if (bad(f)) return TS_E_BADARG;
    TS_TRY(TS_ENTRY("ts_sh_colors_bwd",
                    ts_sh_colors_bwd(f->n, f->sh_degree, f->num_bases, f->means, f->origin,
                                     (f->flags & TS_FRAME_STRIPE) ? nullptr : f->sh_mask, f->v_colors, f->v_colors_dc,
                                     f->num_bases > 1 ? f->v_colors_rest : nullptr, stream)));
    return TS_ENTRY("ts_project_bwd",
                    ts_project_bwd(f->n, f->means, f->scales, f->quats, f->view34, f->projview, &f->cam, 3, f->radii,
                                   f->v_xy, f->v_depth, f->v_conic, nullptr, f->v_means, f->v_scales, f->v_quats,
                                   stream));
}

int ts_frame_bwd_params_adam(const ts_frame* f, const ts_adam* adam, void* stream) {
    TsRange range_("ts_frame_bwd_params_adam");
    if (bad(f) || !adam) return TS_E_BADARG;
    TS_TRY(TS_ENTRY("ts_sh_colors_bwd_adam",
                    ts_sh_colors_bwd_adam(f->n, f->sh_degree, f->num_bases, f->means, f->origin,
                                          (f->flags & TS_FRAME_STRIPE) ? nullptr : f->sh_mask, f->v_colors,
                                          const_cast<float*>(f->colors_dc),
                                          f->num_bases > 1 ? const_cast<float*>(f->colors_rest) : nullptr, adam,
                                          stream)));
    return TS_ENTRY("ts_project_bwd_adam",
                    ts_project_bwd_adam(f->n, const_cast<float*>(f->means), const_cast<float*>(f->scales),
                                        const_cast<float*>(f->quats), f->view34, f->projview, &f->cam, 3, f->radii,
                                        f->v_xy, f->v_depth, f->v_conic, const_cast<float*>(f->opacities), f->v_opacity,
                                        adam, stream));
}


int ts_shard_owner_fwd(const ts_frame* fo, const ts_stripes* stripes, int32_t* route_ws, int32_t* counts,
                       void* stream) {
    return ts_shard_owner_fwd_padded(fo, stripes, nullptr, route_ws, counts, stream);
}

int ts_shard_owner_fwd_padded(const ts_frame* fo, const ts_stripes* stripes, const int32_t* group_base,
                              int32_t* route_ws, int32_t* counts, void* stream) {
    TsRange range_("ts_shard_owner_fwd");
    if (bad(fo) || !stripes) return TS_E_BADARG;
    if (fo->n > 0 && fo->n <= small_n_fused())
        return TS_ENTRY("ts_owner_fwd_fused",
                        ts_shard_owner_fwd_fused(fo->n, fo->sh_degree, fo->num_bases, fo->means, fo->scales, fo->quats,
                                                 fo->view34, fo->projview, &fo->cam, 3, fo->origin, fo->colors_dc,
                                                 fo->num_bases > 1 ? fo->colors_rest : nullptr, fo->opacities,
                                                 fo->channels, TS_RASTER_LOGIT_OPACITY, fo->xys, fo->depths, fo->radii,
                                                 fo->conics, fo->num_tiles_hit, fo->sh_mask, fo->splats, stripes,
                                                 group_base, route_ws, counts, stream));
    TS_TRY(TS_ENTRY("ts_project_fwd",
                    ts_project_fwd(fo->n, fo->means, fo->scales, fo->quats, fo->view34, fo->projview, &fo->cam, 3,
                                   fo->xys, fo->depths, fo->radii, fo->conics, fo->num_tiles_hit, nullptr, stream)));
    TS_TRY(TS_ENTRY("ts_colors_pack_fwd",
                    ts_colors_pack_fwd(fo->n, fo->sh_degree, fo->num_bases, fo->means, fo->origin, fo->colors_dc,
                                       fo->num_bases > 1 ? fo->colors_rest : nullptr, fo->sh_mask, nullptr,
                                       fo->channels, TS_RASTER_LOGIT_OPACITY, fo->xys, fo->radii, fo->conics,
                                       fo->opacities, fo->num_tiles_hit, &fo->cam,
                                       fo->channels == 4 ? fo->depths : nullptr, fo->splats, stream)));
    return TS_ENTRY("ts_route_count",
                    ts_route_count_padded(fo->n, fo->xys, fo->radii, &fo->cam, stripes, group_base, route_ws, counts,
                                          stream));
}

int ts_shard_stripe_fwd_import(const ts_frame* fs, const float* records, void* stream) {
    TsRange range_("ts_shard_stripe_fwd_import");
    if (bad(fs)) return TS_E_BADARG;
    if (fs->n > 0) {
        TS_TRY(TS_ENTRY("ts_import_records",
                        ts_import_records(fs->n, records, &fs->cam, fs->xys, fs->depths, fs->radii, fs->num_tiles_hit,
                                          stream)));
        int32_t* total_dev = fs->total_host ? mapped_pointer(fs->total_host) : nullptr;
        TS_TRY(TS_ENTRY("ts_scan_tiles",
                        ts_scan_tiles(fs->n, fs->num_tiles_hit, fs->cum_tiles_hit, fs->scan_ws, total_dev, stream)));
        if (fs->total_host && !total_dev) {
            const hipError_t e = hipMemcpyAsync(fs->total_host, fs->cum_tiles_hit + (fs->n - 1), sizeof(int32_t),
                                                hipMemcpyDeviceToHost, (hipStream_t)stream);
            if (e != hipSuccess) return (int)e;
        }
        TS_TRY(TS_ENTRY("ts_import_pack",
                        ts_import_pack(fs->n, records, fs->cum_tiles_hit, &fs->cam, fs->splats, stream)));
    }
    TS_TRY(TS_ENTRY("ts_bin_count",
                    ts_bin_count(fs->n, fs->xys, fs->radii, tight_records(fs), &fs->cam, fs->bin_ws, stream)));
    return TS_ENTRY("ts_tile_offsets",
// ... 81 lines not shown
```

### tinysplat_amd/csrc/pack.h

```cpp
#pragma once

#include <hip/hip_runtime.h>

#include "../../include/tinysplat_hip.h"
#include "splat_math.h"

namespace ts {

struct PackArgs {
    int channels, flags;
    const float* xys;
    const int* radii;
    const float* conics;
    const float* opacity;
    const int* cum_tiles_hit;
    const float* depths;
    float4* splats;
    ts_camera cam;
};

__device__ __forceinline__ void pack_one(const PackArgs& a, int i, float c0, float c1, float c2, float c3) {
    const int r = a.radii[i];
    if (r <= 0) return;
    const float2 xy = reinterpret_cast<const float2*>(a.xys)[i];
    const TileBox b = tile_bbox(xy.x, xy.y, (float)r, a.cam.tile_bounds_x, a.cam.tile_bounds_y,
                                a.cam.tile_row0, a.cam.tile_rows);
    const int w = b.maxx - b.minx, h = b.maxy - b.miny;
    const int cnt = h > 0 ? w * h : 0;
    if (cnt <= 0) return;
    const int excl = a.cum_tiles_hit[i] - cnt;
    const int slot_base = excl - b.miny * w - b.minx;
    float op = a.opacity[i];
    if (a.flags & TS_RASTER_LOGIT_OPACITY) op = 1.0f / (1.0f + expf(-op));
    a.splats[3 * (size_t)i] = make_float4(xy.x, xy.y, op, a.conics[3 * i]);
    a.splats[3 * (size_t)i + 1] = make_float4(a.conics[3 * i + 1], a.conics[3 * i + 2], c0, c1);
    a.splats[3 * (size_t)i + 2] =
        make_float4(c2, c3, __int_as_float(slot_base), __int_as_float(w | (b.minx << 16)));
}

}
```

### tinysplat_amd/csrc/project.hip

```cpp
#include <hip/hip_runtime.h>

#include "../../include/tinysplat_hip.h"
#include "host_util.h"
#include "pack.h"
#include "splat_math.h"
#include "adam_math.h"

namespace {

constexpr int kThreads = 256;
#ifndef TS_SH_THREADS_FWD
#define TS_SH_THREADS_FWD 128
#endif
#ifndef TS_SH_THREADS_BWD
#define TS_SH_THREADS_BWD 256
#endif
typedef float f4v __attribute__((ext_vector_type(4)));
__device__ __forceinline__ void store4(float4* p, float a, float b, float c, float d) {
    f4v v = {a, b, c, d};
    __builtin_nontemporal_store(v, reinterpret_cast<f4v*>(p));
}
constexpr int kShThreadsFwd = TS_SH_THREADS_FWD, kShThreadsBwd = TS_SH_THREADS_BWD;
__device__ __forceinline__ float4 load4_stream(const float4* p) {
    const f4v v = __builtin_nontemporal_load(reinterpret_cast<const f4v*>(p));
// ... 62 lines not shown
        const float m[3] = {ADAM ? pm[0] : means3d[3 * i], ADAM ? pm[1] : means3d[3 * i + 1], ADAM ? pm[2] : means3d[3 * i + 2]};
        float s[3] = {ADAM ? ps[0] : scales[3 * i], ADAM ? ps[1] : scales[3 * i + 1], ADAM ? ps[2] : scales[3 * i + 2]};
        float4 qv;
        if (ADAM) qv = make_float4(pq[0], pq[1], pq[2], pq[3]);
        else qv = reinterpret_cast<const float4*>(quats)[i];
        float q[4] = {qv.x, qv.y, qv.z, qv.w};
        float inv_n = 1.0f;
        prep_inputs(flags, s, q, &inv_n);
        const float2 vxy = reinterpret_cast<const float2*>(v_xy)[i];
        const float vx[2] = {vxy.x, vxy.y};
        const float vc[3] = {v_conic[3 * i], v_conic[3 * i + 1], v_conic[3 * i + 2]};
        float vcov[6];
        if (v_cov3d) {
            for (int k = 0; k < 6; ++k) vcov[k] = v_cov3d[6 * (size_t)i + k];
        }
        ts::project_one_vjp(C, m, s, q, vx, v_depth ? v_depth[i] : 0.0f, vc, v_cov3d ? vcov : nullptr, g);
        if (flags & TS_PROJECT_LOG_SCALES) {
            g.v_scale[0] *= s[0]; g.v_scale[1] *= s[1]; g.v_scale[2] *= s[2];
        }
        if (flags & TS_PROJECT_RAW_QUATS) {
            const float dotp = q[0] * g.v_quat[0] + q[1] * g.v_quat[1] + q[2] * g.v_quat[2] +
                               q[3] * g.v_quat[3];
            for (int k = 0; k < 4; ++k) g.v_quat[k] = (g.v_quat[k] - q[k] * dotp) * inv_n;
        }
    }
    if (ADAM) {
        float mo[3], vo[3];
#pragma unroll
        for (int k = 0; k < 3; ++k) { mo[k] = ad.m_means[3 * i + k]; vo[k] = ad.v_means[3 * i + k]; }
#pragma unroll
        for (int k = 0; k < 3; ++k) {
            ts::adam_update(pm[k], g.v_mean[k], mo[k], vo[k], ad.c_means);
            ad.means[3 * i + k] = pm[k]; ad.m_means[3 * i + k] = mo[k]; ad.v_means[3 * i + k] = vo[k];
        }
#pragma unroll
        for (int k = 0; k < 3; ++k) { mo[k] = ad.m_scales[3 * i + k]; vo[k] = ad.v_scales[3 * i + k]; }
#pragma unroll
        for (int k = 0; k < 3; ++k) {
            ts::adam_update(ps[k], g.v_scale[k], mo[k], vo[k], ad.c_scales);
            ad.scales[3 * i + k] = ps[k]; ad.m_scales[3 * i + k] = mo[k]; ad.v_scales[3 * i + k] = vo[k];
        }
        float4 mq = reinterpret_cast<float4*>(ad.m_quats)[i], vq = reinterpret_cast<float4*>(ad.v_quats)[i];
        ts::adam_update(pq[0], g.v_quat[0], mq.x, vq.x, ad.c_quats); ts::adam_update(pq[1], g.v_quat[1], mq.y, vq.y, ad.c_quats);
        ts::adam_update(pq[2], g.v_quat[2], mq.z, vq.z, ad.c_quats); ts::adam_update(pq[3], g.v_quat[3], mq.w, vq.w, ad.c_quats);
        reinterpret_cast<float4*>(ad.quats)[i] = make_float4(pq[0], pq[1], pq[2], pq[3]);
        reinterpret_cast<float4*>(ad.m_quats)[i] = mq;
        reinterpret_cast<float4*>(ad.v_quats)[i] = vq;
        if (ad.opacities) {
            float po = ad.opacities[i], mo1 = ad.m_opac[i], vo1 = ad.v_opac[i];
            ts::adam_update(po, ad.v_opacity[i], mo1, vo1, ad.c_opac);
            ad.opacities[i] = po; ad.m_opac[i] = mo1; ad.v_opac[i] = vo1;
        }
        return;
    }
    v_means3d[3 * i] = g.v_mean[0]; v_means3d[3 * i + 1] = g.v_mean[1];
    v_means3d[3 * i + 2] = g.v_mean[2];
    v_scales[3 * i] = g.v_scale[0]; v_scales[3 * i + 1] = g.v_scale[1];
    v_scales[3 * i + 2] = g.v_scale[2];
    reinterpret_cast<float4*>(v_quats)[i] =
        make_float4(g.v_quat[0], g.v_quat[1], g.v_quat[2], g.v_quat[3]);
}

template <int DEG>
__global__ __launch_bounds__(kThreads) void sh_fwd_kernel(
    int n, int num_bases, const float* __restrict__ viewdirs, const float* __restrict__ coeffs,
    float* __restrict__ colors) {
    constexpr int KA = (DEG + 1) * (DEG + 1);
    constexpr int RS = 3 * KA;
    constexpr int RSP = RS | 1;
    extern __shared__ __align__(16) float lds[];
    const int g0 = blockIdx.x * kThreads;
    const int cnt = min(kThreads, n - g0);
    const int tid = threadIdx.x;
    const size_t row = 3 * (size_t)num_bases;
    const float* src = coeffs + (size_t)g0 * row;
    if (num_bases == KA && cnt == kThreads) {
        const float4* src4 = reinterpret_cast<const float4*>(src);
        constexpr int total4 = kThreads * RS / 4;
        for (int f4 = tid; f4 < total4; f4 += kThreads) {
            const float4 v = src4[f4];
            const int f = 4 * f4;
            const float e[4] = {v.x, v.y, v.z, v.w};
#pragma unroll
            for (int u = 0; u < 4; ++u) {
                const int ff = f + u;
                lds[(ff / RS) * RSP + (ff % RS)] = e[u];
            }
        }
    } else {
        const int total = cnt * RS;
        for (int f = tid; f < total; f += kThreads) {
            const int g = f / RS, j = f % RS;
            lds[g * RSP + j] = src[(size_t)g * row + j];
        }
    }
    __syncthreads();
    if (tid >= cnt) return;
    const int i = g0 + tid;
    float Y[KA];
    ts::sh_basis(DEG, viewdirs[3 * i], viewdirs[3 * i + 1], viewdirs[3 * i + 2], Y);
    const float* r = lds + tid * RSP;
    float c0 = Y[0] * r[0], c1 = Y[0] * r[1], c2 = Y[0] * r[2];
#pragma unroll
    for (int k = 1; k < KA; ++k) {
        c0 = c0 + Y[k] * r[3 * k];
        c1 = c1 + Y[k] * r[3 * k + 1];
        c2 = c2 + Y[k] * r[3 * k + 2];
    }
    colors[3 * i] = c0; colors[3 * i + 1] = c1; colors[3 * i + 2] = c2;
}

template <int DEG>
__global__ __launch_bounds__(kThreads) void sh_bwd_kernel(
    int n, int num_bases, const float* __restrict__ viewdirs, const float* __restrict__ v_colors,
    float* __restrict__ v_coeffs) {
    constexpr int KA = (DEG + 1) * (DEG + 1);
    extern __shared__ __align__(16) float lds[];
    const int RS = 3 * num_bases;
    const int RSP = RS | 1;
    const int g0 = blockIdx.x * kThreads;
    const int cnt = min(kThreads, n - g0);
    const int tid = threadIdx.x;
    if (tid < cnt) {
        const int i = g0 + tid;
        float Y[KA];
        ts::sh_basis(DEG, viewdirs[3 * i], viewdirs[3 * i + 1], viewdirs[3 * i + 2], Y);
        const float v0 = v_colors[3 * i], v1 = v_colors[3 * i + 1], v2 = v_colors[3 * i + 2];
        float* r = lds + tid * RSP;
#pragma unroll
        for (int k = 0; k < KA; ++k) {
            r[3 * k] = Y[k] * v0; r[3 * k + 1] = Y[k] * v1; r[3 * k + 2] = Y[k] * v2;
        }
        for (int j = 3 * KA; j < RS; ++j) r[j] = 0.0f;
    }
    __syncthreads();
    float* dst = v_coeffs + (size_t)g0 * RS;
    const int total = cnt * RS;
    if ((total & 3) == 0) {
        float4* dst4 = reinterpret_cast<float4*>(dst);
        for (int f4 = tid; f4 < total / 4; f4 += kThreads) {
            float e[4];
#pragma unroll
            for (int u = 0; u < 4; ++u) {
                const int ff = 4 * f4 + u;
                e[u] = lds[(ff / RS) * RSP + (ff % RS)];
            }
            dst4[f4] = make_float4(e[0], e[1], e[2], e[3]);
        }
    } else {
        for (int f = tid; f < total; f += kThreads) dst[f] = lds[(f / RS) * RSP + (f % RS)];
    }
}

template <int DEG>
__global__ __launch_bounds__(kShThreadsFwd) void sh_colors_fwd_kernel(
    int n, int num_bases, const float* __restrict__ means, const float* __restrict__ origin,
    const float* __restrict__ dc, const float* __restrict__ rest, float* __restrict__ colors,
    unsigned char* __restrict__ mask, const ts::PackArgs pk) {
    constexpr int KA = (DEG + 1) * (DEG + 1);
    constexpr int RS = 3 * (KA - 1);
    constexpr int RSP = RS | 1;
    extern __shared__ __align__(16) float lds[];
    const int g0 = blockIdx.x * kShThreadsFwd;
    const int cnt = min(kShThreadsFwd, n - g0);
    const int tid = threadIdx.x;
    if (RS > 0) {
        const size_t row = 3 * (size_t)(num_bases - 1);
        const float* src = rest + (size_t)g0 * row;
        if (num_bases == KA && cnt == kShThreadsFwd && ((kShThreadsFwd * RS) & 3) == 0) {
            const float4* src4 = reinterpret_cast<const float4*>(src);
            constexpr int total4 = kShThreadsFwd * RS / 4;
            constexpr int per = (total4 + kShThreadsFwd - 1) / kShThreadsFwd;
            float4 v[per > 0 ? per : 1];
#pragma unroll
            for (int u = 0; u < per; ++u) {
                const int f4 = tid + u * kShThreadsFwd;
                v[u] = f4 < total4 ? load4_stream(src4 + f4) : make_float4(0.f, 0.f, 0.f, 0.f);
            }
#pragma unroll
            for (int u = 0; u < per; ++u) {
                const int f4 = tid + u * kShThreadsFwd;
                if (f4 < total4) {
                    const float e[4] = {v[u].x, v[u].y, v[u].z, v[u].w};
#pragma unroll
                    for (int c = 0; c < 4; ++c) {
                        const int ff = 4 * f4 + c;
                        lds[(ff / RS) * RSP + (ff % RS)] = e[c];
                    }
                }
            }
        } else {
            const int total = cnt * RS;
            for (int f = tid; f < total; f += kShThreadsFwd) {
                const int g = f / RS, j = f % RS;
                lds[g * RSP + j] = src[(size_t)g * row + j];
            }
        }
        __syncthreads();
    }
    if (tid >= cnt) return;
    const int i = g0 + tid;
    float Y[KA];
    ts::sh_basis(DEG, means[3 * i] - origin[0], means[3 * i + 1] - origin[1],
                 means[3 * i + 2] - origin[2], Y);
    float c0 = Y[0] * dc[3 * i], c1 = Y[0] * dc[3 * i + 1], c2 = Y[0] * dc[3 * i + 2];
    const float* r = lds + tid * RSP;
#pragma unroll
    for (int k = 1; k < KA; ++k) {
        c0 = c0 + Y[k] * r[3 * (k - 1)];
        c1 = c1 + Y[k] * r[3 * (k - 1) + 1];
        c2 = c2 + Y[k] * r[3 * (k - 1) + 2];
    }
    c0 = c0 + 0.5f; c1 = c1 + 0.5f; c2 = c2 + 0.5f;
    if (mask) mask[i] = (unsigned char)((c0 >= 0.0f ? 1 : 0) | (c1 >= 0.0f ? 2 : 0) | (c2 >= 0.0f ? 4 : 0));
    c0 = fmaxf(c0, 0.0f); c1 = fmaxf(c1, 0.0f); c2 = fmaxf(c2, 0.0f);
    if (colors) { colors[3 * i] = c0; colors[3 * i + 1] = c1; colors[3 * i + 2] = c2; }
    if (pk.splats) ts::pack_one(pk, i, c0, c1, c2, pk.channels == 4 ? pk.depths[i] : 0.0f);
}

template <int DEG>
__global__ __launch_bounds__(kThreads) void sh_colors_fwd_sparse_kernel(
    int n, int num_bases, const int* __restrict__ live, const float* __restrict__ means,
    const float* __restrict__ origin, const float* __restrict__ dc, const float* __restrict__ rest,
    float* __restrict__ colors, unsigned char* __restrict__ mask, const ts::PackArgs pk) {
    constexpr int KA = (DEG + 1) * (DEG + 1);
    const int i = blockIdx.x * kThreads + threadIdx.x;
    if (i >= n || live[i] == 0) return;
    float Y[KA];
    ts::sh_basis(DEG, means[3 * i] - origin[0], means[3 * i + 1] - origin[1],
                 means[3 * i + 2] - origin[2], Y);
    float c0 = Y[0] * dc[3 * i], c1 = Y[0] * dc[3 * i + 1], c2 = Y[0] * dc[3 * i + 2];
    const float* r = rest + (size_t)i * 3 * (num_bases - 1);
#pragma unroll
    for (int k = 1; k < KA; ++k) {
        c0 = c0 + Y[k] * r[3 * (k - 1)];
        c1 = c1 + Y[k] * r[3 * (k - 1) + 1];
        c2 = c2 + Y[k] * r[3 * (k - 1) + 2];
    }
    c0 = c0 + 0.5f; c1 = c1 + 0.5f; c2 = c2 + 0.5f;
    if (mask) mask[i] = (unsigned char)((c0 >= 0.0f ? 1 : 0) | (c1 >= 0.0f ? 2 : 0) | (c2 >= 0.0f ? 4 : 0));
    c0 = fmaxf(c0, 0.0f); c1 = fmaxf(c1, 0.0f); c2 = fmaxf(c2, 0.0f);
    if (colors) { colors[3 * i] = c0; colors[3 * i + 1] = c1; colors[3 * i + 2] = c2; }
    if (pk.splats) ts::pack_one(pk, i, c0, c1, c2, pk.channels == 4 ? pk.depths[i] : 0.0f);
}

struct ShAdam {
    float *dc, *rest, *m_dc, *v_dc, *m_rest, *v_rest;
    ts::AdamCoef c_dc, c_rest;
};
template <int DEG, bool ADAM>
__global__ __launch_bounds__(kShThreadsBwd) void sh_colors_bwd_kernel(
    int n, int num_bases, const float* __restrict__ means, const float* __restrict__ origin,
    const unsigned char* __restrict__ mask, const float* __restrict__ v_colors,
    float* __restrict__ v_dc, float* __restrict__ v_rest, const ShAdam ad) {
    constexpr int KA = (DEG + 1) * (DEG + 1);
    extern __shared__ __align__(16) float lds[];
    const int RS = 3 * (num_bases - 1);
    const int RSP = RS | 1;
    const int g0 = blockIdx.x * kShThreadsBwd;
    const int cnt = min(kShThreadsBwd, n - g0);
    const int tid = threadIdx.x;
    if (tid < cnt) {
        const int i = g0 + tid;
        float Y[KA];
        ts::sh_basis(DEG, means[3 * i] - origin[0], means[3 * i + 1] - origin[1],
                     means[3 * i + 2] - origin[2], Y);
        const int m = mask ? mask[i] : 7;
        const float v0 = (m & 1) ? v_colors[3 * i] : 0.0f, v1 = (m & 2) ? v_colors[3 * i + 1] : 0.0f,
                    v2 = (m & 4) ? v_colors[3 * i + 2] : 0.0f;
        if (ADAM) {
            const float gd[3] = {Y[0] * v0, Y[0] * v1, Y[0] * v2};
#pragma unroll
            for (int c = 0; c < 3; ++c) {
                float p_ = ad.dc[3 * i + c], m_ = ad.m_dc[3 * i + c], s_ = ad.v_dc[3 * i + c];
                ts::adam_update(p_, gd[c], m_, s_, ad.c_dc);
                ad.dc[3 * i + c] = p_; ad.m_dc[3 * i + c] = m_; ad.v_dc[3 * i + c] = s_;
            }
        } else {
            v_dc[3 * i] = Y[0] * v0; v_dc[3 * i + 1] = Y[0] * v1; v_dc[3 * i + 2] = Y[0] * v2;
        }
        float* r = lds + tid * RSP;
#pragma unroll
        for (int k = 1; k < KA; ++k) {
            r[3 * (k - 1)] = Y[k] * v0; r[3 * (k - 1) + 1] = Y[k] * v1; r[3 * (k - 1) + 2] = Y[k] * v2;
        }
        for (int j = 3 * (KA - 1); j < RS; ++j) r[j] = 0.0f;
    }
    if (RS == 0) return;
    __syncthreads();
    const size_t off = (size_t)g0 * RS;
    float* dst = ADAM ? nullptr : v_rest + off;
    const int total = cnt * RS;
    if ((total & 3) == 0 && ((off) & 3) == 0) {
        float4* dst4 = reinterpret_cast<float4*>(dst);
        for (int f4 = tid; f4 < total / 4; f4 += kShThreadsBwd) {
            float e[4];
#pragma unroll
            for (int u = 0; u < 4; ++u) {
                const int ff = 4 * f4 + u;
                e[u] = lds[(ff / RS) * RSP + (ff % RS)];
            }
            if (ADAM) {
                float4* p4 = reinterpret_cast<float4*>(ad.rest + off) + f4;
                float4* m4 = reinterpret_cast<float4*>(ad.m_rest + off) + f4;
                float4* s4 = reinterpret_cast<float4*>(ad.v_rest + off) + f4;
                float4 pp = *p4, mm = *m4, ss = *s4;
                ts::adam_update(pp.x, e[0], mm.x, ss.x, ad.c_rest); ts::adam_update(pp.y, e[1], mm.y, ss.y, ad.c_rest);
                ts::adam_update(pp.z, e[2], mm.z, ss.z, ad.c_rest); ts::adam_update(pp.w, e[3], mm.w, ss.w, ad.c_rest);
                *p4 = pp; *m4 = mm; *s4 = ss;
            } else {
                store4(dst4 + f4, e[0], e[1], e[2], e[3]);
            }
        }
    } else {
        for (int f = tid; f < total; f += kShThreadsBwd) {
            const float e = lds[(f / RS) * RSP + (f % RS)];
            if (ADAM) {
                float p_ = ad.rest[off + f], m_ = ad.m_rest[off + f], s_ = ad.v_rest[off + f];
                ts::adam_update(p_, e, m_, s_, ad.c_rest);
                ad.rest[off + f] = p_; ad.m_rest[off + f] = m_; ad.v_rest[off + f] = s_;
            } else {
                dst[f] = e;
            }
        }
    }
}

__global__ __launch_bounds__(kThreads) void stream_read_kernel(const float4* __restrict__ src,
                                                               size_t n16, float* __restrict__ sink) {
    constexpr int U = 8;
    const size_t stride = (size_t)gridDim.x * kThreads;
    size_t i = (size_t)blockIdx.x * kThreads + threadIdx.x;
    float4 acc[U];
#pragma unroll
    for (int u = 0; u < U; ++u) acc[u] = make_float4(0.f, 0.f, 0.f, 0.f);
    for (; i + (U - 1) * stride < n16; i += U * stride) {
        float4 v[U];
#pragma unroll
        for (int u = 0; u < U; ++u) {
            const f4v t = __builtin_nontemporal_load(reinterpret_cast<const f4v*>(src + i + u * stride));
            v[u] = make_float4(t.x, t.y, t.z, t.w);
        }
#pragma unroll
        for (int u = 0; u < U; ++u) {
            acc[u].x += v[u].x; acc[u].y += v[u].y; acc[u].z += v[u].z; acc[u].w += v[u].w;
        }
    }
    for (; i < n16; i += stride) {
        const float4 v0 = src[i];
        acc[0].x += v0.x; acc[0].y += v0.y; acc[0].z += v0.z; acc[0].w += v0.w;
    }
    float t = 0.f;
#pragma unroll
    for (int u = 0; u < U; ++u) t += (acc[u].x + acc[u].y) + (acc[u].z + acc[u].w);
    if (t == 123456.789f) sink[0] = t;
}

__global__ __launch_bounds__(kThreads) void gather48_kernel(const float4* __restrict__ records,
                                                            const int* __restrict__ ids, size_t m,
                                                            float* __restrict__ sink) {
    const size_t stride = (size_t)gridDim.x * kThreads;
    float4 a = make_float4(0.f, 0.f, 0.f, 0.f);
    for (size_t j = (size_t)blockIdx.x * kThreads + threadIdx.x; j < m; j += stride) {
        const size_t g = (size_t)ids[j];
        const float4 q0 = records[3 * g], q1 = records[3 * g + 1], q2 = records[3 * g + 2];
        a.x += q0.x + q1.x + q2.x; a.y += q0.y + q1.y + q2.y; a.z += q0.z + q1.z + q2.z; a.w += q0.w + q1.w + q2.w;
    }
    if ((a.x + a.y) + (a.z + a.w) == 123456.789f) sink[0] = a.x;
}

}

extern "C" {

int ts_abi_version(void) { return TS_ABI_VERSION; }

int ts_project_fwd(int32_t n, const float* means3d, const float* scales, const float* quats,
                   const float* viewmat, const float* projmat, const ts_camera* cam,
                   int32_t flags, float* xys, float* depths, int32_t* radii, float* conics,
                   int32_t* num_tiles_hit, float* cov3d, void* stream) {
    if (n < 0 || !cam) return TS_E_BADARG;
    if (n == 0) return 0;
    if (!means3d || !scales || !quats || !viewmat || !projmat || !xys || !depths || !radii ||
        !conics || !num_tiles_hit)
        return TS_E_BADARG;
    const int grid = (n + kThreads - 1) / kThreads;
    hipLaunchKernelGGL(project_fwd_kernel, dim3(grid), dim3(kThreads), 0, (hipStream_t)stream, n,
                       means3d, scales, quats, viewmat, projmat, *cam, (int)flags, xys, depths, radii,
                       conics, num_tiles_hit, cov3d);
    return launch_status();
}

int ts_project_bwd(int32_t n, const float* means3d, const float* scales, const float* quats,
                   const float* viewmat, const float* projmat, const ts_camera* cam,
                   int32_t flags, const int32_t* radii, const float* v_xy, const float* v_depth,
                   const float* v_conic, const float* v_cov3d, float* v_means3d, float* v_scales,
                   float* v_quats, void* stream) {
    if (n < 0 || !cam) return TS_E_BADARG;
    if (n == 0) return 0;
    if (!means3d || !scales || !quats || !viewmat || !projmat || !radii || !v_xy ||
        !v_conic || !v_means3d || !v_scales || !v_quats)
        return TS_E_BADARG;
    const int grid = (n + kThreads - 1) / kThreads;
    hipLaunchKernelGGL(project_bwd_kernel<false>, dim3(grid), dim3(kThreads), 0, (hipStream_t)stream, n,
                       means3d, scales, quats, viewmat, projmat, *cam, (int)flags, radii, v_xy, v_depth,
                       v_conic, v_cov3d, v_means3d, v_scales, v_quats, ProjAdam{});
    return launch_status();
}

static bool adam_group_ok(const ts_adam* a, int k) {
    return a->exp_avg[k] && a->exp_avg_sq[k] && a->step[k] >= 1;
}

int ts_project_bwd_adam(int32_t n, float* means3d, float* scales, float* quats, const float* viewmat,
                        const float* projmat, const ts_camera* cam, int32_t flags, const int32_t* radii,
                        const float* v_xy, const float* v_depth, const float* v_conic, float* opacities,
                        const float* v_opacity, const ts_adam* adam, void* stream) {
    if (n < 0 || !cam || !adam) return TS_E_BADARG;
    if (n == 0) return 0;
    if (!means3d || !scales || !quats || !viewmat || !projmat || !radii || !v_xy || !v_conic) return TS_E_BADARG;
    if (!adam_group_ok(adam, TS_ADAM_MEANS) || !adam_group_ok(adam, TS_ADAM_SCALES) || !adam_group_ok(adam, TS_ADAM_QUATS))
        return TS_E_BADARG;
    if (opacities && (!v_opacity || !adam_group_ok(adam, TS_ADAM_OPACITIES))) return TS_E_BADARG;
    ProjAdam ad{};
    ad.means = means3d; ad.scales = scales; ad.quats = quats; ad.opacities = opacities; ad.v_opacity = v_opacity;
    ad.m_means = adam->exp_avg[TS_ADAM_MEANS]; ad.v_means = adam->exp_avg_sq[TS_ADAM_MEANS];
    ad.m_scales = adam->exp_avg[TS_ADAM_SCALES]; ad.v_scales = adam->exp_avg_sq[TS_ADAM_SCALES];
    ad.m_quats = adam->exp_avg[TS_ADAM_QUATS]; ad.v_quats = adam->exp_avg_sq[TS_ADAM_QUATS];
    ad.m_opac = adam->exp_avg[TS_ADAM_OPACITIES]; ad.v_opac = adam->exp_avg_sq[TS_ADAM_OPACITIES];
    auto coef = [&](int k) { return ts::adam_coef(adam->lr[k], adam->step[k], adam->beta1, adam->beta2, adam->eps); };
    ad.c_means = coef(TS_ADAM_MEANS); ad.c_scales = coef(TS_ADAM_SCALES); ad.c_quats = coef(TS_ADAM_QUATS);
    if (opacities) ad.c_opac = coef(TS_ADAM_OPACITIES);
    const int grid = (n + kThreads - 1) / kThreads;
    hipLaunchKernelGGL(project_bwd_kernel<true>, dim3(grid), dim3(kThreads), 0, (hipStream_t)stream, n,
                       means3d, scales, quats, viewmat, projmat, *cam, (int)flags, radii, v_xy, v_depth,
                       v_conic, (const float*)nullptr, (float*)nullptr, (float*)nullptr, (float*)nullptr, ad);
    return launch_status();
}

static int sh_check(int32_t n, int32_t degree, int32_t num_bases) {
    if (n < 0) return TS_E_BADARG;
    if (num_bases != 1 && num_bases != 4 && num_bases != 9 && num_bases != 16 && num_bases != 25)
        return TS_E_DEGREE;
    if (degree < 0 || degree > 4 || (degree + 1) * (degree + 1) > num_bases) return TS_E_DEGREE;
    return 0;
}

int ts_sh_fwd(int32_t n, int32_t degrees_to_use, int32_t num_bases, const float* viewdirs,
              const float* coeffs, float* colors, void* stream) {
    const int chk = sh_check(n, degrees_to_use, num_bases);
    if (chk) return chk;
    if (n == 0) return 0;
    if (!viewdirs || !coeffs || !colors) return TS_E_BADARG;
    const int grid = (n + kThreads - 1) / kThreads;
    const int ka = (degrees_to_use + 1) * (degrees_to_use + 1);
    const size_t lds = (size_t)kThreads * ((3 * ka) | 1) * sizeof(float);
    hipStream_t s = (hipStream_t)stream;
#define TS_SH_FWD(D)                                                                          \
    hipLaunchKernelGGL(sh_fwd_kernel<D>, dim3(grid), dim3(kThreads), lds, s, n, num_bases,     \
                       viewdirs, coeffs, colors)
    switch (degrees_to_use) {
        case 0: TS_SH_FWD(0); break;
        case 1: TS_SH_FWD(1); break;
        case 2: TS_SH_FWD(2); break;
        case 3: TS_SH_FWD(3); break;
        default: {
            (void)hipFuncSetAttribute(reinterpret_cast<const void*>(&sh_fwd_kernel<4>),
                                hipFuncAttributeMaxDynamicSharedMemorySize, (int)lds);
            TS_SH_FWD(4);
        } break;
    }
#undef TS_SH_FWD
    return launch_status();
}

int ts_sh_bwd(int32_t n, int32_t degrees_to_use, int32_t num_bases, const float* viewdirs,
              const float* v_colors, float* v_coeffs, void* stream) {
    const int chk = sh_check(n, degrees_to_use, num_bases);
    if (chk) return chk;
    if (n == 0) return 0;
    if (!viewdirs || !v_colors || !v_coeffs) return TS_E_BADARG;
    const int grid = (n + kThreads - 1) / kThreads;
    const size_t lds = (size_t)kThreads * ((3 * num_bases) | 1) * sizeof(float);
    hipStream_t s = (hipStream_t)stream;
#define TS_SH_BWD(D)                                                                          \
    do {                                                                                      \
        if (lds > 48 * 1024)                                                                  \
            (void)hipFuncSetAttribute(reinterpret_cast<const void*>(&sh_bwd_kernel<D>),           \
                                hipFuncAttributeMaxDynamicSharedMemorySize, (int)lds);        \
        hipLaunchKernelGGL(sh_bwd_kernel<D>, dim3(grid), dim3(kThreads), lds, s, n, num_bases, \
                           viewdirs, v_colors, v_coeffs);                                     \
    } while (0)
    switch (degrees_to_use) {
        case 0: TS_SH_BWD(0); break;
        case 1: TS_SH_BWD(1); break;
        case 2: TS_SH_BWD(2); break;
        case 3: TS_SH_BWD(3); break;
        default: TS_SH_BWD(4); break;
    }
#undef TS_SH_BWD
    return launch_status();
}

static int launch_colors_fwd(int32_t n, int32_t degrees_to_use, int32_t num_bases, const float* means3d,
                             const float* origin, const float* colors_dc, const float* colors_rest,
                             float* colors, uint8_t* clamp_mask, const int32_t* live, const ts::PackArgs& pk,
                             void* stream) {
    const int chk = sh_check(n, degrees_to_use, num_bases);
    if (chk) return chk;
    if (n == 0) return 0;
    if (!means3d || !origin || !colors_dc || (!colors && !pk.splats) || (num_bases > 1 && !colors_rest))
        return TS_E_BADARG;
    const int grid = (n + kThreads - 1) / kThreads;
    hipStream_t s = (hipStream_t)stream;
    if (live) {
#define TS_SHC_SPARSE(D)                                                                           \
        hipLaunchKernelGGL(sh_colors_fwd_sparse_kernel<D>, dim3(grid), dim3(kThreads), 0, s, n,    \
                           num_bases, live, means3d, origin, colors_dc, colors_rest, colors, clamp_mask, pk)
        switch (degrees_to_use) {
            case 0: TS_SHC_SPARSE(0); break;
            case 1: TS_SHC_SPARSE(1); break;
            case 2: TS_SHC_SPARSE(2); break;
            case 3: TS_SHC_SPARSE(3); break;
            default: TS_SHC_SPARSE(4); break;
        }
#undef TS_SHC_SPARSE
        return launch_status();
    }
    const int ka = (degrees_to_use + 1) * (degrees_to_use + 1);
    const size_t lds = (size_t)kShThreadsFwd * ((3 * (ka - 1)) | 1) * sizeof(float);
    const int grid_d = (n + kShThreadsFwd - 1) / kShThreadsFwd;
#define TS_SHC_FWD(D)                                                                             \
    do {                                                                                          \
        if (lds > 48 * 1024)                                                                      \
            (void)hipFuncSetAttribute(reinterpret_cast<const void*>(&sh_colors_fwd_kernel<D>),    \
                                      hipFuncAttributeMaxDynamicSharedMemorySize, (int)lds);      \
        hipLaunchKernelGGL(sh_colors_fwd_kernel<D>, dim3(grid_d), dim3(kShThreadsFwd), lds, s, n,  \
                           num_bases, means3d, origin, colors_dc, colors_rest, colors, clamp_mask, pk); \
    } while (0)
    switch (degrees_to_use) {
        case 0: TS_SHC_FWD(0); break;
        case 1: TS_SHC_FWD(1); break;
        case 2: TS_SHC_FWD(2); break;
        case 3: TS_SHC_FWD(3); break;
        default: TS_SHC_FWD(4); break;
    }
#undef TS_SHC_FWD
    return launch_status();
}

int ts_sh_colors_fwd(int32_t n, int32_t degrees_to_use, int32_t num_bases, const float* means3d,
                     const float* origin, const float* colors_dc, const float* colors_rest,
                     float* colors, uint8_t* clamp_mask, const int32_t* live, void* stream) {
    ts::PackArgs none;
    none.splats = nullptr;
    if (!colors) return TS_E_BADARG;
    return launch_colors_fwd(n, degrees_to_use, num_bases, means3d, origin, colors_dc, colors_rest, colors,
                             clamp_mask, live, none, stream);
}

int ts_colors_pack_fwd(int32_t n, int32_t degrees_to_use, int32_t num_bases, const float* means3d,
                       const float* origin, const float* colors_dc, const float* colors_rest,
                       uint8_t* clamp_mask, const int32_t* live, int32_t channels, int32_t flags,
                       const float* xys, const int32_t* radii, const float* conics, const float* opacity,
                       const int32_t* cum_tiles_hit, const ts_camera* cam, const float* depths,
                       float* splats, void* stream) {
    if (n < 0 || !cam || (channels != 3 && channels != 4)) return TS_E_BADARG;
    if (n > 0 && (!xys || !radii || !conics || !opacity || !cum_tiles_hit || !splats ||
                  (channels == 4 && !depths)))
        return TS_E_BADARG;
    ts::PackArgs pk;
    pk.channels = channels; pk.flags = (int)flags; pk.xys = xys; pk.radii = radii; pk.conics = conics;
    pk.opacity = opacity; pk.cum_tiles_hit = cum_tiles_hit; pk.depths = depths;
    pk.splats = reinterpret_cast<float4*>(splats); pk.cam = *cam;
    return launch_colors_fwd(n, degrees_to_use, num_bases, means3d, origin, colors_dc, colors_rest, nullptr,
                             clamp_mask, live, pk, stream);
}

static int sh_colors_bwd_launch(int32_t n, int32_t degrees_to_use, int32_t num_bases, const float* means3d,
                                const float* origin, const uint8_t* clamp_mask, const float* v_colors,
                                float* v_colors_dc, float* v_colors_rest, const ShAdam* ad, void* stream) {
    const int grid = (n + kShThreadsBwd - 1) / kShThreadsBwd;
    const size_t lds = (size_t)kShThreadsBwd * ((3 * (num_bases - 1)) | 1) * sizeof(float);
    hipStream_t s = (hipStream_t)stream;
#define TS_SHC_BWD2(D, A)                                                                            \
    do {                                                                                             \
        if (lds > 48 * 1024)                                                                         \
            (void)hipFuncSetAttribute(reinterpret_cast<const void*>(&sh_colors_bwd_kernel<D, A>),    \
                                      hipFuncAttributeMaxDynamicSharedMemorySize, (int)lds);         \
        hipLaunchKernelGGL((sh_colors_bwd_kernel<D, A>), dim3(grid), dim3(kShThreadsBwd), lds, s, n, \
                           num_bases, means3d, origin, clamp_mask, v_colors, v_colors_dc,            \
                           v_colors_rest, ad ? *ad : ShAdam{});                                      \
    } while (0)
#define TS_SHC_BWD(D)                                       \
    do {                                                    \
        if (ad) TS_SHC_BWD2(D, true);                       \
        else TS_SHC_BWD2(D, false);                         \
    } while (0)
    switch (degrees_to_use) {
        case 0: TS_SHC_BWD(0); break;
        case 1: TS_SHC_BWD(1); break;
        case 2: TS_SHC_BWD(2); break;
        case 3: TS_SHC_BWD(3); break;
        default: TS_SHC_BWD(4); break;
    }
#undef TS_SHC_BWD
#undef TS_SHC_BWD2
    return launch_status();
}

int ts_sh_colors_bwd(int32_t n, int32_t degrees_to_use, int32_t num_bases, const float* means3d,
                     const float* origin, const uint8_t* clamp_mask, const float* v_colors,
                     float* v_colors_dc, float* v_colors_rest, void* stream) {
    const int chk = sh_check(n, degrees_to_use, num_bases);
    if (chk) return chk;
    if (n == 0) return 0;
    if (!means3d || !origin || !v_colors || !v_colors_dc || (num_bases > 1 && !v_colors_rest))
        return TS_E_BADARG;
    return sh_colors_bwd_launch(n, degrees_to_use, num_bases, means3d, origin, clamp_mask, v_colors, v_colors_dc,
                                v_colors_rest, nullptr, stream);
}

int ts_sh_colors_bwd_adam(int32_t n, int32_t degrees_to_use, int32_t num_bases, const float* means3d,
                          const float* origin, const uint8_t* clamp_mask, const float* v_colors,
                          float* colors_dc, float* colors_rest, const ts_adam* adam, void* stream) {
    const int chk = sh_check(n, degrees_to_use, num_bases);
    if (chk) return chk;
    if (n == 0) return 0;
    if (!adam || !means3d || !origin || !v_colors || !colors_dc || (num_bases > 1 && !colors_rest)) return TS_E_BADARG;
    if (!adam_group_ok(adam, TS_ADAM_COLORS_DC) || (num_bases > 1 && !adam_group_ok(adam, TS_ADAM_COLORS_REST)))
        return TS_E_BADARG;
    ShAdam ad{};
    ad.dc = colors_dc; ad.rest = colors_rest;
    ad.m_dc = adam->exp_avg[TS_ADAM_COLORS_DC]; ad.v_dc = adam->exp_avg_sq[TS_ADAM_COLORS_DC];
    ad.m_rest = adam->exp_avg[TS_ADAM_COLORS_REST]; ad.v_rest = adam->exp_avg_sq[TS_ADAM_COLORS_REST];
    ad.c_dc = ts::adam_coef(adam->lr[TS_ADAM_COLORS_DC], adam->step[TS_ADAM_COLORS_DC], adam->beta1, adam->beta2, adam->eps);
    if (num_bases > 1)
        ad.c_rest = ts::adam_coef(adam->lr[TS_ADAM_COLORS_REST], adam->step[TS_ADAM_COLORS_REST], adam->beta1, adam->beta2,
                                  adam->eps);
    return sh_colors_bwd_launch(n, degrees_to_use, num_bases, means3d, origin, clamp_mask, v_colors, nullptr, nullptr, &ad,
                                stream);
}

int ts_bench_gather48(const float* records, const int32_t* ids, int64_t m, float* sink, void* stream) {
    if (!records || !ids || !sink || m < 1) return TS_E_BADARG;
    hipLaunchKernelGGL(gather48_kernel, dim3(256 * 8), dim3(kThreads), 0, (hipStream_t)stream,
                       reinterpret_cast<const float4*>(records), ids, (size_t)m, sink);
    return launch_status();
}

int ts_bench_stream_read(const float* src, int64_t n_floats, float* sink, void* stream) {
    if (!src || !sink || n_floats < 4) return TS_E_BADARG;
    const size_t n16 = (size_t)n_floats / 4;
    hipLaunchKernelGGL(stream_read_kernel, dim3(256 * 8), dim3(kThreads), 0, (hipStream_t)stream,
                       reinterpret_cast<const float4*>(src), n16, sink);
    return launch_status();
}

}
```

### tinysplat_amd/frame.py

```python
from __future__ import annotations

import ctypes
import os
import threading
from typing import Optional, Tuple

import torch
import torch.distributed as dist
from torch import Tensor

from ._comm import collective_timer
from . import _lib
from ._lib import TsFrame
from .ops import TileBinning, _camera, _f32c, _need_hip, _stream, _stripe_rows, _tile_bounds, deg_from_sh

TIGHT_BINNING = os.environ.get("TS_TIGHT_BINNING", "1") != "0"

SPLIT_BLOCKS_BELOW = int(os.environ.get("TS_SPLIT_BLOCKS_BELOW", "2400"))

_ls = os.environ.get("TS_LIST_SEGMENTS", "auto")
LIST_SEGMENTS = _ls if _ls == "auto" else max(1, min(8, int(_ls)))
LIST_SEGMENTS_FROM = int(os.environ.get("TS_LIST_SEGMENTS_FROM", "192"))
SEGMENT_ITEMS = int(os.environ.get("TS_SEGMENT_ITEMS", "16384"))


HYBRID_FROM = int(os.environ.get("TS_HYBRID_FROM", "4096"))
HYBRID_SEGS = max(1, min(8, int(os.environ.get("TS_HYBRID_SEGS", "8"))))
HYBRID_WHOLE16 = max(1, min(15, int(os.environ.get("TS_HYBRID_WHOLE16", "13"))))
HYBRID_MID_FROM = int(os.environ.get("TS_HYBRID_MID_FROM", "1537"))
HYBRID_MID_WHOLE16 = max(1, min(15, int(os.environ.get("TS_HYBRID_MID_WHOLE16", "6"))))
HYBRID_MID_COOP16 = max(0, min(15, int(os.environ.get("TS_HYBRID_MID_COOP16", "6"))))
HYBRID_COOP16 = max(0, min(15, int(os.environ.get("TS_HYBRID_COOP16", "3"))))
COOP_SPLIT = os.environ.get("TS_COOP_SPLIT", "1") != "0"


def set_launch_hints(cam, segs: int, w16: int, mode: int, split: bool, skewed: bool = False) -> None:
    cam.hints = (cam.hints & ~0x1FFF00) | (((segs << 8) | (w16 << 12)) if segs > 1 else 0)
    tiles16 = cam.tile_rows * cam.tile_bounds_x
    if mode == 0 and not split and tiles16 >= HYBRID_FROM:
        cam.hints |= (HYBRID_MID_COOP16 if skewed else HYBRID_COOP16) << 16
    elif mode == 0 and not split and tiles16 >= HYBRID_MID_FROM:
        cam.hints |= HYBRID_MID_COOP16 << 16
    if mode == 0 and split and COOP_SPLIT:
        cam.hints |= _lib.HINT_COOP_SPLIT


def _list_segments(tiles16: int, mode: int, split: bool, skewed: bool = False):
    if mode != 0 or tiles16 <= 0:
        return 1, 0
    if not split:
        if HYBRID_SEGS > 1 and tiles16 >= HYBRID_FROM:
            return HYBRID_SEGS, (HYBRID_MID_WHOLE16 if skewed else HYBRID_WHOLE16)
        if HYBRID_SEGS > 1 and tiles16 >= HYBRID_MID_FROM:
            return HYBRID_SEGS, HYBRID_MID_WHOLE16
        return 1, 0
    if LIST_SEGMENTS != "auto":
        return int(LIST_SEGMENTS), 0
    return max(2, min(8, SEGMENT_ITEMS // tiles16)), 0


last_segments = {}


def segments_for_count(cam, segs: int, total: int) -> int:
    if segs > 1 and total >= LIST_SEGMENTS_FROM * cam.tile_rows * cam.tile_bounds_x:
        return segs
    cam.hints &= ~0xFF00
    return 1


def backward_segments(cam, segs: int, total: int, dev_index: int = 0) -> int:
    segs = segments_for_count(cam, segs, total)
    last_segments[dev_index] = segs
    return segs

_wt = os.environ.get("TS_WIDE_TILES", "auto")
WIDE_TILES = int(_wt) if _wt.lstrip("+-").isdigit() else _wt
WIDE_LISTS_FROM = int(os.environ.get("TS_WIDE_LISTS_FROM", "2300"))
BALANCED_WALK_FROM = float(os.environ.get("TS_BALANCED_WALK_FROM", "10"))
_pairs_per_tile = {}


MANY_TILES_FROM = int(os.environ.get("TS_MANY_TILES_FROM", "20000"))
LONG_LIST = int(os.environ.get("TS_LONG_LIST", "2048"))
SKEW_FROM = float(os.environ.get("TS_SKEW_FROM", "4"))
_stats_mode = {}
_longest_list = {}


def _list_mode(dev_index: int, tiles16: int) -> int:
    if WIDE_TILES != "auto":
        if WIDE_TILES not in (0, 2):
            raise ValueError(f"TS_WIDE_TILES / frame.WIDE_TILES = {WIDE_TILES!r}: accepted values are 0, 2 and 'auto'")
        return int(WIDE_TILES)
    prev = _pairs_per_tile.get(dev_index)
    if prev is None:
        return 2 if tiles16 >= MANY_TILES_FROM else 0
    if prev >= WIDE_LISTS_FROM:
        return 2
    st = _longest_list.get(dev_index)
    if tiles16 >= MANY_TILES_FROM and st is not None:
        longest, mode = st
        return 2 if longest < (2 * LONG_LIST if mode == 2 else LONG_LIST) else 0
    return 0


def _skewed(dev_index: int, mode: int) -> bool:
    st, prev = _longest_list.get(dev_index), _pairs_per_tile.get(dev_index)
    if WIDE_TILES != "auto" or mode != 0 or st is None or prev is None or st[1] != 0:
        return False
    return st[0] >= SKEW_FROM * max(prev, 1.0)

last_binning = {}

TRACE = None


def _mark(label):
    if TRACE is not None:
        import time
        TRACE.append((label, time.perf_counter()))


_layouts = {}
_pinned_total = {}
_row_flags = {}
_row_flags_lock = threading.Lock()
_row_flags_tick = [0]

FLAG_GENERATIONS = os.environ.get("TS_FLAG_GENERATIONS", "1") != "0"


FLAGS_SHRINK_AFTER = 256


def row_flags_for(dev: torch.device, rows: int):
    if not FLAG_GENERATIONS:
        return torch.empty((rows,), dtype=torch.uint8, device=dev), 0
    key = (dev.index, _stream(dev))
    with _row_flags_lock:
        slot = _row_flags.get(key)
        if slot is not None and slot[0].numel() > 8 * max(rows, 1 << 20):
            slot[2] += 1
            if slot[2] >= FLAGS_SHRINK_AFTER:
                slot = None
        elif slot is not None:
            slot[2] = 0
        if slot is None or slot[0].numel() < rows:
            if key not in _row_flags and len(_row_flags) >= 32:
                _row_flags.pop(min(_row_flags, key=lambda k_: _row_flags[k_][3]))
            slot = _row_flags[key] = [torch.zeros((int(rows * 1.25) + 4096,), dtype=torch.uint8, device=dev), 0, 0, 0]
        _row_flags_tick[0] += 1
        slot[3] = _row_flags_tick[0]
        slot[1] += 1
        if slot[1] > 255:
            slot[0].zero_()
            slot[1] = 1
        return slot[0], slot[1]

_bg_cache = {}

STRIPE_SPARSE = os.environ.get("TS_STRIPE_SPARSE", "1") != "0"

TWO_HOP_SCATTER = os.environ.get("TS_TWO_HOP_SCATTER", "1") != "0"
INLINE_SORT = os.environ.get("TS_INLINE_SORT", "1") != "0"

DIRECT_GRADS = os.environ.get("TS_DIRECT_GRADS", "1") != "0"

SURVIVORS = os.environ.get("TS_SURVIVORS", "1") != "0"

GROUP_COUNTS = os.environ.get("TS_GROUP_COUNTS", "1") != "0"

ONE_WALK = os.environ.get("TS_ONE_WALK", "1") != "0"

CAPACITY_ALLOC = os.environ.get("TS_CAPACITY_ALLOC", "0") != "0"
CAPACITY_GROWTH = 1.25
_capacity = {}

COUNT_WAIT = os.environ.get("TS_COUNT_WAIT", "spin")
_SPIN_LIMIT = 50_000_000


def alloc_quantum(count: int) -> int:
    count = max(int(count), 1)
    if count <= 65536:
        return 65536
    g = 1 << (count.bit_length() - 4)
    return (count + g - 1) // g * g


def _total_slot(dev: torch.device):
    slot = _pinned_total.get(dev.index)
    if slot is None:
        slot = (torch.zeros((4,), dtype=torch.int32, pin_memory=True), torch.cuda.Event(), threading.Lock())
        _pinned_total[dev.index] = slot
    return slot


class _Frame:
    __slots__ = ("fr", "cam", "n", "nb", "ch", "w", "h", "num_tiles", "total", "split", "segs", "keep",
                 "wf", "tile_bins", "ids", "bucket_ids", "out_img", "out_depth", "planes", "xys", "radii", "nth", "cum",
                 "inputs", "bg")


def _forward(means, scales, quats, opacities, colors_dc, colors_rest, view34, projview, origin, background,
             fx, fy, width, height, sh_degree, with_depth, tile_rows, keep: bool, planes: bool = False) -> _Frame:
    _mark("fwd:enter")
    dev = _need_hip(means, scales, quats, opacities, colors_dc, colors_rest, view34, projview, origin, background)
    n = means.shape[0]
    nb = colors_rest.shape[1] + 1
    if sh_degree < 0 or sh_degree > deg_from_sh(nb):
        raise ValueError("sh_degree exceeds the stored coefficients")
    means, scales, quats = _f32c(means), _f32c(scales), _f32c(quats)
    opacities, colors_dc, colors_rest = _f32c(opacities), _f32c(colors_dc), _f32c(colors_rest)
    view34, projview, origin = _f32c(view34), _f32c(projview), _f32c(origin)
    w, h = int(width), int(height)
    cam = _camera(fx, fy, w / 2, h / 2, h, w, _tile_bounds(h, w), 1.0, tile_rows=tile_rows)
    slot_ = _pinned_total.get(dev.index)
    if slot_ is not None and dev.index in _stats_mode:
        _longest_list[dev.index] = (int(ctypes.c_int32.from_address(slot_[0].data_ptr() + 4).value), _stats_mode[dev.index])
    mode = _list_mode(dev.index, cam.tile_rows * cam.tile_bounds_x)
    cam.wide_tiles = 1 if mode else 0
    prev_i = _pairs_per_tile.get(dev.index)
    if prev_i is not None and n > 0 and prev_i * cam.tile_rows * cam.tile_bounds_x >= BALANCED_WALK_FROM * n:
        cam.hints = _lib.HINT_BALANCED_WALK
    ch = 4 if with_depth else 3
    if with_depth:
        key = (background.data_ptr(), background._version, dev.index)
        hit = _bg_cache.get(key)
        if hit is None:
            if len(_bg_cache) > 16:
                _bg_cache.clear()
            hit = _bg_cache[key] = (_f32c(torch.cat([background, background[:1]])), background)
        bg = hit[0]
    else:
        bg = _f32c(background)
    lib = _lib.load()
    s = _stream(dev)
    F = _Frame()
    F.cam, F.n, F.nb, F.ch, F.w, F.h, F.keep = cam, n, nb, ch, w, h, keep
    F.inputs = (means, scales, quats, opacities, colors_dc, colors_rest, view34, projview, origin)
    F.bg = bg
    num_tiles = int(lib.ts_num_tiles(ctypes.byref(cam)))
    F.num_tiles = num_tiles
    F.split = 0 < cam.tile_rows * cam.tile_bounds_x <= SPLIT_BLOCKS_BELOW
    rows = _stripe_rows(cam)
    m = max(n, 1)
    skewed = _skewed(dev.index, mode)
    segs, w16 = _list_segments(cam.tile_rows * cam.tile_bounds_x, mode, F.split, skewed) if keep else (1, 0)
    set_launch_hints(cam, segs, w16, mode, F.split, skewed)
    F.segs = segs
    _mark("fwd:inputs checked")
    cur = torch.cuda.current_device()
    if cur != dev.index:
        torch.cuda.set_device(dev)
    try:
        f32 = dict(dtype=torch.float32, device=dev)
        i32 = dict(dtype=torch.int32, device=dev)
        px = rows * w
        lkey = (n, num_tiles, w, rows, ch, keep, cam.hints & 0xFFFF00, cam.wide_tiles, cam.tile_rows, cam.tile_row0, cam.tile_bounds_x, cam.img_height)
        lay = _layouts.get(lkey)
        if lay is None:
            nscan = int(lib.ts_scan_ws_ints(n))
            nbin = int(lib.ts_bin_ws_ints(n, num_tiles))
            fin_floats = int(lib.ts_final_floats(ctypes.byref(cam), ch)) if keep else px
            sizes = [48 * m, 8 * m, 12 * m, 0, 4 * m, 4 * m, 4 * m, 4 * m, 4 * nscan, 4 * nbin,
                     8 * max(num_tiles, 1)] + ([m, 4 * fin_floats, 4 * px, px] if keep else [])
            offs, off = [], 0
            for sz in sizes:
                offs.append(off)
                off += (sz + 255) & ~255
            if len(_layouts) > 64:
                _layouts.clear()
            lay = _layouts[lkey] = (offs, off)
        offs, off = lay
        _mark("fwd:sizes")
        F.wf = torch.empty((off,), dtype=torch.uint8, device=dev)
        _mark("fwd:workspace allocated")
        base = F.wf.data_ptr()
        ptr = [base + o for o in offs]
        F.planes = bool(planes and with_depth)
        F.out_img = torch.empty((rows, w, 3 if F.planes else ch), **f32)
        F.out_depth = torch.empty((rows, w), **f32) if F.planes else None
        _mark("fwd:image allocated")

        def view(k, dtype, count, shape):
            return F.wf[offs[k]:offs[k] + count * dtype.itemsize].view(dtype).view(shape)
        F.xys = view(1, torch.float32, 2 * n, (n, 2))
        F.radii = view(5, torch.int32, n, (n,))
        F.nth = view(6, torch.int32, n, (n,))
        F.cum = view(7, torch.int32, n, (n,))
        F.tile_bins = view(10, torch.int32, 2 * max(num_tiles, 1), (max(num_tiles, 1), 2))
        host, event, count_lock = _total_slot(dev)
        fr = TsFrame()
        fr.n, fr.num_bases, fr.sh_degree, fr.channels = n, nb, int(sh_degree), ch
        stripe = STRIPE_SPARSE and cam.tile_rows < cam.tile_bounds_y
        full = cam.tile_rows == cam.tile_bounds_y
        fr.flags = ((_lib.FRAME_TIGHT if TIGHT_BINNING else 0) | (_lib.FRAME_SPLIT if F.split else 0)
                    | (_lib.FRAME_NARROW_WAVES if mode == 2 else 0) | (_lib.FRAME_STRIPE if stripe else 0)
                    | (0 if TWO_HOP_SCATTER else _lib.FRAME_DIRECT_SCATTER) | (_lib.FRAME_PLANES if F.planes else 0)
                    | (0 if INLINE_SORT else _lib.FRAME_SEPARATE_SORT)
                    | (_lib.FRAME_LIST_STATS if full else 0))
        surv = SURVIVORS and keep and full and mode == 0 and not F.split and INLINE_SORT
        if surv:
            fr.flags |= _lib.FRAME_SURVIVORS
        if GROUP_COUNTS:
            fr.flags |= _lib.FRAME_GROUP_COUNTS
        if ONE_WALK:
            fr.flags |= _lib.FRAME_ONE_WALK
        if full:
            _stats_mode[dev.index] = mode
        fr.cam = cam
        fr.means, fr.scales, fr.quats, fr.opacities = means.data_ptr(), scales.data_ptr(), quats.data_ptr(), opacities.data_ptr()
        fr.colors_dc, fr.colors_rest = colors_dc.data_ptr(), colors_rest.data_ptr()
        fr.view34, fr.projview, fr.origin, fr.background = view34.data_ptr(), projview.data_ptr(), origin.data_ptr(), bg.data_ptr()
        fr.splats, fr.xys, fr.conics, fr.depths = ptr[0], ptr[1], ptr[2], ptr[4]
        fr.radii, fr.num_tiles_hit, fr.cum_tiles_hit, fr.scan_ws = ptr[5], ptr[6], ptr[7], ptr[8]
        fr.bin_ws, fr.tile_bins = ptr[9], ptr[10]
        fr.total_host = host.data_ptr()
        fr.out_img = F.out_img.data_ptr()
        if F.planes:
            fr.out_depth = F.out_depth.data_ptr()
        if keep:
            fr.sh_mask, fr.final_Ts, fr.final_index, fr.clamp_mask = ptr[11], ptr[12], ptr[13], ptr[14]
        F.fr = fr
        _mark("fwd:allocated + struct")
        spin = COUNT_WAIT == "spin" and n > 0
        cap_key = (dev.index, n, w, h, cam.tile_row0, cam.tile_rows)
        est = _capacity.get(cap_key) if (CAPACITY_ALLOC and n > 0) else None

        def lists(size):
            cap = alloc_quantum(size)
            counts = (8 * num_tiles + 63) // 64 * 64 if surv else 0
            F.bucket_ids = torch.empty(((3 * cap + counts) if surv else 2 * cap,), **i32)
            fr.bucket_ids, fr.gaussian_ids_sorted = F.bucket_ids.data_ptr(), F.bucket_ids.data_ptr() + 4 * cap
            if surv:
                fr.survivors = F.bucket_ids.data_ptr() + 8 * cap
            return cap

        def prepare():
            _lib.check(lib.ts_frame_fwd_prepare(ctypes.byref(fr), s), "ts_frame_fwd_prepare")

        def composite():
            _lib.check(lib.ts_frame_fwd_composite(ctypes.byref(fr), s), "ts_frame_fwd_composite")

        count_lock.acquire()
        issued = consumed = False
        try:
            if spin:
                word = ctypes.c_int32.from_address(host.data_ptr())
                word.value = -(1 << 31)
            _lib.check(lib.ts_frame_fwd_project(ctypes.byref(fr), s), "ts_frame_fwd_project")
            issued = n > 0
            _mark("fwd:call project")
            event.record()
            cap = None
            if est is not None:
                cap = lists(est)
                fr.capacity, fr.num_intersects = cap, cap
                prepare()
                composite()
            else:
                fr.capacity = -1
                prepare()
            _mark("fwd:call prepare")
            total = 0
            if n > 0:
                if spin:
                    k = 0
                    while word.value == -(1 << 31):
                        k += 1
                        if k > _SPIN_LIMIT:
                            event.synchronize()
                            break
                    total = int(word.value)
                else:
                    event.synchronize()
                    total = int(host[0])
            consumed = True
        finally:
            if issued and not consumed:
                try:
                    event.synchronize()
                except Exception:
                    pass
            count_lock.release()
        if total < 0:
            raise OverflowError("more than 2^31-1 tile intersections: num_tiles_hit overflows its "
                                "int32 prefix sum (gsplat's cum_tiles_hit is int32 as well)")
        _mark("fwd:waited for count")
        F.total = total
        _pairs_per_tile[dev.index] = total / max(1, cam.tile_rows * cam.tile_bounds_x)
        if n > 0 and CAPACITY_ALLOC:
            if len(_capacity) > 64:
                _capacity.clear()
            _capacity[cap_key] = int(total * CAPACITY_GROWTH) + 4096
        if cap is None or total > cap:
            redo = cap is not None
            cap = lists(total)
            _mark("fwd:lists allocated")
            fr.capacity, fr.num_intersects = -1, total
            F.segs = segments_for_count(fr.cam, F.segs, total)
            if redo:
                prepare()
            composite()
            _mark("fwd:composite enqueued")
        else:
            fr.num_intersects = total
        F.ids = F.bucket_ids[cap:cap + total]
        _mark("fwd:call composite")
    finally:
        if cur != dev.index:
            torch.cuda.set_device(cur)
    b = TileBinning()
    b.cam, b.n, b.num_tiles, b.num_intersects = cam, n, num_tiles, total
    b.tile_bins, b.gaussian_ids_sorted, b.cum_tiles_hit, b.num_tiles_hit = F.tile_bins[:num_tiles], F.ids, F.cum, F.nth
    last_binning[dev.index] = b
    _mark("fwd:exit")
    return F


class _AdamHook:
    opt = None


_adam_hook = _AdamHook()


class fused_adam:
    def __init__(self, optimizer):
        self.optimizer = optimizer

    def __enter__(self):
        self.prev = getattr(_adam_hook, "opt", None)
        _adam_hook.opt = self.optimizer
        return self

    def __exit__(self, *exc):
        _adam_hook.opt = self.prev
        return False


class _RenderFrame(torch.autograd.Function):
    @staticmethod
    def forward(ctx, means, scales, quats, opacities, colors_dc, colors_rest, view34, projview,
                origin, background, fx, fy, width, height, sh_degree, with_depth, tile_rows, group, planes=False):
        F = _forward(means, scales, quats, opacities, colors_dc, colors_rest, view34, projview, origin,
                     background, fx, fy, width, height, sh_degree, with_depth, tile_rows, keep=True, planes=planes)
        ctx.frame, ctx.group = F, group
        ctx.opacity_shape = opacities.shape
        ctx.rest_shape = colors_rest.shape
        xys, radii = F.xys, F.radii
        ctx.xys_out = xys
        ctx.mark_non_differentiable(xys, radii)
        ctx.set_materialize_grads(False)
        out, F.out_img = F.out_img, None
        depth, F.out_depth = F.out_depth, None
        return out, depth, xys, radii

    @staticmethod
    def backward(ctx, v_img, v_depth_img, _v_xys, _v_radii):
        _mark("bwd:enter")
# ... 104 lines not shown
```

Before: 2064000 billion Gaussians*pixels/s.

## Precompute per-Gaussian tile row spans in pack kernel for one-walk binning

The color/pack kernel now computes a compact 16-byte record per Gaussian holding the first tile row and each row's tight tile column range, up to six rows. A new span-based scatter kernel reads these records instead of re-running the tight ellipse test per row. It also emits runs of consecutive tiles within a coarse group as one staged item with a length, so fewer LDS atomics are needed. This costs an extra 16 bytes per Gaussian of workspace and extra work in the pack kernel, and Gaussians that need more rows or wider columns fall back to the old walk.

```diff
diff --git a/include/tinysplat_hip.h b/include/tinysplat_hip.h
--- a/include/tinysplat_hip.h
+++ b/include/tinysplat_hip.h
@@ -71,6 +71,12 @@
                        const float* xys, const int32_t* radii, const float* conics, const float* opacity,
                        const int32_t* cum_tiles_hit, const ts_camera* cam_host, const float* depths,
                        float* splats, void* stream);
+int ts_colors_pack_spans_fwd(int32_t n, int32_t degrees_to_use, int32_t num_bases, const float* means3d,
+                             const float* origin, const float* colors_dc, const float* colors_rest,
+                             uint8_t* clamp_mask, const int32_t* live, int32_t channels, int32_t flags,
+                             const float* xys, const int32_t* radii, const float* conics, const float* opacity,
+                             const int32_t* cum_tiles_hit, const ts_camera* cam_host, const float* depths,
+                             float* splats, int32_t tight, int32_t* row_spans, void* stream);
 
 
 int64_t ts_scan_ws_ints(int32_t n);
@@ -111,6 +117,9 @@
 int ts_bin_emit_groups(int32_t n, const float* xys, const int32_t* radii, const float* splats,
                        const ts_camera* cam_host, const int32_t* cum_tiles_hit, int64_t capacity, int32_t* bin_ws,
                        int32_t* scratch, void* stream);
+int ts_bin_emit_groups_spans(int32_t n, const float* xys, const int32_t* radii, const float* splats,
+                             const int32_t* row_spans, const ts_camera* cam_host, const int32_t* cum_tiles_hit,
+                             int64_t capacity, int32_t* bin_ws, int32_t* scratch, void* stream);
 int ts_emit_offsets(int32_t n, int32_t num_tiles, int32_t* bin_ws, int32_t* tile_bins,
                     const int32_t* cum_tiles_hit, int64_t capacity, int32_t* longest_list, void* stream);
 int ts_bin_gather_groups(int32_t n, int32_t num_tiles, int32_t* bin_ws, int32_t* tile_bins, int32_t* bucket_ids,
@@ -176,6 +185,7 @@
 #define TS_FRAME_STRIPE 16
 #define TS_FRAME_GROUP_COUNTS 1024
 #define TS_FRAME_ONE_WALK 2048
+#define TS_FRAME_ROW_SPANS (4096)
 #define TS_FRAME_SURVIVORS 512
 typedef struct ts_frame {
     int32_t n, num_bases, sh_degree, channels, flags;
@@ -202,6 +212,7 @@
     float* out_depth;
     const float* v_out_depth;
     int32_t* survivors;
+    int32_t* row_spans;
 } ts_frame;
 int32_t ts_frame_struct_bytes(void);
 int ts_frame_fwd_project(const ts_frame* f, void* stream);
diff --git a/tinysplat_amd/_lib.py b/tinysplat_amd/_lib.py
--- a/tinysplat_amd/_lib.py
+++ b/tinysplat_amd/_lib.py
@@ -25,6 +25,7 @@
 FRAME_SURVIVORS = 512
 FRAME_GROUP_COUNTS = 1024
 FRAME_ONE_WALK = 2048
+FRAME_ROW_SPANS = 4096
 PARTIAL_ROW_FLOATS = 12
 
 
@@ -63,7 +64,7 @@
                     "v_out_img", "partials", "row_flags",
                     "v_xy", "v_conic", "v_colors", "v_depth", "v_opacity",
                     "v_means", "v_scales", "v_quats", "v_colors_dc", "v_colors_rest",
-                    "out_depth", "v_out_depth", "survivors")])
+                    "out_depth", "v_out_depth", "survivors", "row_spans")])
 
 
 _FRAME = POINTER(TsFrame)
@@ -128,6 +129,7 @@
     "ts_bin_one_walk_form": (c_int32, [c_int32, c_int32]),
     "ts_bin_stage_capacity": (c_int32, []),
     "ts_bin_emit_groups": (c_int32, [c_int32, _P, _P, _P, _CAM, _P, c_int64, _P, _P, _P]),
+    "ts_bin_emit_groups_spans": (c_int32, [c_int32, _P, _P, _P, _P, _CAM, _P, c_int64, _P, _P, _P]),
     "ts_emit_offsets": (c_int32, [c_int32, c_int32, _P, _P, _P, c_int64, _P, _P]),
     "ts_bin_gather_groups": (c_int32, [c_int32, c_int32, _P, _P, _P, _P, _P]),
     "ts_sort_tiles_stats": (c_int32, [c_int32, _P, _P, _P, _P, _P, _P, c_int32, _P, _P, _P]),
@@ -137,6 +139,8 @@
     "ts_cut_tiles": (c_int32, [_CAM, _P, _P]),
     "ts_colors_pack_fwd": (c_int32, [c_int32, c_int32, c_int32, _P, _P, _P, _P, _P, _P, c_int32, c_int32,
                                      _P, _P, _P, _P, _P, _CAM, _P, _P, _P]),
+    "ts_colors_pack_spans_fwd": (c_int32, [c_int32, c_int32, c_int32, _P, _P, _P, _P, _P, _P, c_int32, c_int32,
+                                           _P, _P, _P, _P, _P, _CAM, _P, _P, c_int32, _P, _P]),
     "ts_pack_splats": (c_int32, [c_int32, c_int32, c_int32, _P, _P, _P, _P, _P, _P, _CAM, _P, _P, _P]),
     "ts_raster_fwd": (c_int32, [c_int32, c_int32, _CAM, _P, _P, _P, _P, _P, _P, _P, _P, _P]),
     "ts_raster_bwd": (c_int32, [c_int32, c_int32, c_int64, _CAM, _P, _P, _P, _P, _P, _P, _P, _P, _P, _P, _P, _P]),
diff --git a/tinysplat_amd/csrc/binning.hip b/tinysplat_amd/csrc/binning.hip
--- a/tinysplat_amd/csrc/binning.hip
+++ b/tinysplat_amd/csrc/binning.hip
@@ -3,6 +3,7 @@
 #include "../../include/tinysplat_hip.h"
 #include "host_util.h"
 #include "pack.h"
+#include "row_spans.h"
 #include "splat_math.h"
 
 namespace {
@@ -780,6 +781,70 @@
     return g.groups <= kEmitMaxGroups && g.rows_end <= g.tile_start;
 }
 
+constexpr int kSpanPre = 4;
+template <typename Emit>
+__device__ __forceinline__ void walk_gaussian(int i, const float* __restrict__ xys, const int* __restrict__ radii,
+                                              const float4* __restrict__ splats, const ts_camera& cam, Emit emit) {
+    const int ws = cam.wide_tiles ? 1 : 0;
+    const int tbx = (cam.tile_bounds_x + ws) >> ws;
+    const int r = radii[i];
+    if (r <= 0) return;
+    const float2 xy = reinterpret_cast<const float2*>(xys)[i];
+    float4 q0 = make_float4(0.f, 0.f, 0.f, 0.f), q1 = q0;
+    if (splats) { q0 = splats[3 * (size_t)i]; q1 = splats[3 * (size_t)i + 1]; }
+    const ts::TileBox b = ts::tile_bbox(xy.x, xy.y, (float)r, cam.tile_bounds_x, cam.tile_bounds_y, cam.tile_row0,
+                                        cam.tile_rows);
+    if (b.maxy <= b.miny || b.maxx <= b.minx) return;
+    const TightTest tight(splats != nullptr, q0.x, q0.y, q0.z, q0.w, q1.x, q1.y, (float)r);
+    if (tight.cull_all) return;
+    for (int ty = b.miny; ty < b.maxy; ++ty) {
+        int lo, hi;
+        tight.row_range(ty, b.minx, b.maxx, lo, hi);
+        if (hi <= lo) continue;
+        for (int tx = lo >> ws; tx <= (hi - 1) >> ws; ++tx) emit((ty - cam.tile_row0) * tbx + tx, i);
+    }
+}
+template <typename Emit>
+__device__ __forceinline__ void walk_spans(int g0, int g1, const int4* __restrict__ spans,
+                                           const float* __restrict__ xys, const int* __restrict__ radii,
+                                           const float4* __restrict__ splats, const ts_camera& cam, Emit emit) {
+    const int ws = cam.wide_tiles ? 1 : 0;
+    const int tbx = (cam.tile_bounds_x + ws) >> ws;
+    for (int base = g0 + threadIdx.x; base < g1; base += kSpanPre * kBinThreads) {
+        int4 rec[kSpanPre];
+#pragma unroll
+        for (int u = 0; u < kSpanPre; ++u) {
+            const int i = base + u * kBinThreads;
+            rec[u] = i < g1 ? spans[i] : make_int4(0, 0, 0, 0);
+        }
+#pragma unroll
+        for (int u = 0; u < kSpanPre; ++u) {
+            ts::RowSpans s;
+            s.w[0] = (unsigned int)rec[u].x; s.w[1] = (unsigned int)rec[u].y;
+            s.w[2] = (unsigned int)rec[u].z; s.w[3] = (unsigned int)rec[u].w;
+            const int rows = ts::spans_rows(s);
+            if (rows == 0) continue;
+            const int i = base + u * kBinThreads;
+            if (rows == ts::kSpanFallback) {
+                walk_gaussian(i, xys, radii, splats, cam, [&](int t, int id) { emit(t, 1, id); });
+                continue;
+            }
+            int t0 = ts::spans_first_row(s) * tbx;
+            for (int k = 0; k < rows; ++k, t0 += tbx) {
+                int lo, hi;
+                ts::spans_pop_row(s, lo, hi);
+                if (hi <= lo) continue;
+                const int last = t0 + ((hi - 1) >> ws);
+                for (int t = t0 + (lo >> ws); t <= last;) {
+                    const int len = min(last - t + 1, kCoarseTiles - (t & (kCoarseTiles - 1)));
+                    emit(t, len, i);
+                    t += len;
+                }
+            }
+        }
+    }
+}
+
 __global__ __launch_bounds__(kBinThreads) void bin_scatter_emit_kernel(
     int n, int chunk, const float* __restrict__ xys, const int* __restrict__ radii,
     const float4* __restrict__ splats, const ts_camera cam, int groups, const int* __restrict__ cum,
@@ -865,6 +930,105 @@
     } else {
         walk_chunk(g0, g1, xys, radii, splats, cam, [&](int t, int i) {
             dst[atomicAdd(&cursor[t >> kCoarseShift], 1)] = i | ((t & (kCoarseTiles - 1)) << kCoarseIdBits);
+        });
+    }
+}
+
+__global__ __launch_bounds__(kBinThreads) void bin_scatter_spans_kernel(
+    int n, int chunk, const float* __restrict__ xys, const int* __restrict__ radii,
+    const float4* __restrict__ splats, const int4* __restrict__ spans, const ts_camera cam, int groups,
+    const int* __restrict__ cum, long long capacity, int* __restrict__ counts, int* __restrict__ starts,
+    int* __restrict__ scratch) {
+    extern __shared__ int lds[];
+    __shared__ int staged;
+    const int g0 = min(n, (int)blockIdx.x * chunk), g1 = min(n, g0 + chunk);
+    const int total = cum[n - 1];
+    const int chunk_base = g0 > 0 ? cum[g0 - 1] : 0;
+    const int chunk_end = g1 > g0 ? cum[g1 - 1] : chunk_base;
+    int* hist = lds;
+    int* cursor = lds + groups;
+    unsigned int* words = reinterpret_cast<unsigned int*>(lds + 2 * groups);
+    unsigned short* grp = reinterpret_cast<unsigned short*>(words + kStageCap);
+    const int tid = threadIdx.x;
+    for (int j = tid; j < groups; j += kBinThreads) hist[j] = 0;
+    if (tid == 0) staged = 0;
+    __syncthreads();
+    if (total < 0 || (capacity >= 0 && (long long)total > capacity)) return;
+    const int room = chunk_end - chunk_base;
+    auto walk = [&](auto emit) { walk_spans(g0, g1, spans, xys, radii, splats, cam, emit); };
+    static_assert(kEmitMaxGroups <= (1 << 11) && kCoarseTiles <= 32, "group index in 11 bits, len - 1 in 5");
+    walk([&](int t, int len, int i) {
+        const int g = t >> kCoarseShift;
+        atomicAdd(&hist[g], len);
+        const unsigned long long m = __ballot(1);
+        const int rank = (int)__builtin_amdgcn_mbcnt_hi((unsigned int)(m >> 32),
+                                                        __builtin_amdgcn_mbcnt_lo((unsigned int)m, 0u));
+        int base = 0;
+        if (rank == 0) base = atomicAdd(&staged, (int)__popcll(m));
+        base = __builtin_amdgcn_readfirstlane(base);
+        const int slot = base + rank;
+        if (slot < kStageCap) {
+            words[slot] = (unsigned int)i | ((unsigned int)(t & (kCoarseTiles - 1)) << kCoarseIdBits);
+            grp[slot] = (unsigned short)(g | ((len - 1) << 11));
+        }
+    });
+    __syncthreads();
+    const int items = staged;
+    int pairs;
+    bool sound;
+    {
+        const int a = 2 * tid;
+        const int h0 = a < groups ? hist[a] : 0, h1 = a + 1 < groups ? hist[a + 1] : 0;
+        const int ex = block_inclusive_scan<kBinThreads / 64>(h0 + h1, &pairs) - h0 - h1;
+        sound = pairs <= room;
+        int* crow = counts + (size_t)blockIdx.x * groups;
+        int* srow = starts + (size_t)blockIdx.x * groups;
+        if (a < groups) {
+            cursor[a] = ex;
+            crow[a] = sound ? h0 : 0;
+            srow[a] = chunk_base + ex;
+        }
+        if (a + 1 < groups) {
+            cursor[a + 1] = ex + h0;
+            crow[a + 1] = sound ? h1 : 0;
+            srow[a + 1] = chunk_base + ex + h0;
+        }
+    }
+    __syncthreads();
+    if (!sound) return;
+    int* dst = scratch + chunk_base;
+    if (items <= kStageCap && pairs <= kStageCap) {
+        constexpr int kPer = kStageCap / kBinThreads;
+        static_assert(kStageCap % kBinThreads == 0, "whole staging rounds");
+        unsigned int w[kPer];
+        int at[kPer];
+        static_assert(kStageCap <= 65536, "a place in 16 bits");
+#pragma unroll
+        for (int u = 0; u < kPer; ++u) {
+            const int j = u * kBinThreads + tid;
+            if (j < items) {
+                w[u] = words[j];
+                const int gl = grp[j], len1 = gl >> 11;
+                at[u] = atomicAdd(&cursor[gl & 2047], len1 + 1) | (len1 << 16);
+            }
+        }
+        __syncthreads();
+#pragma unroll
+        for (int u = 0; u < kPer; ++u)
+            if (u * kBinThreads + tid < items) {
+                const int first = at[u] & 0xffff, len1 = at[u] >> 16;
+                for (int q = 0; q <= len1; ++q) words[first + q] = w[u] + ((unsigned int)q << kCoarseIdBits);
+            }
+        __syncthreads();
+#pragma unroll
+        for (int u = 0; u < kPer; ++u) {
+            const int j = u * kBinThreads + tid;
+            if (j < pairs) dst[j] = (int)words[j];
+        }
+    } else {
+        walk([&](int t, int len, int i) {
+            const int at = atomicAdd(&cursor[t >> kCoarseShift], len);
+            for (int q = 0; q < len; ++q) dst[at + q] = i | (((t + q) & (kCoarseTiles - 1)) << kCoarseIdBits);
         });
     }
 }
@@ -1361,11 +1525,28 @@
 int ts_bin_emit_groups(int32_t n, const float* xys, const int32_t* radii, const float* splats,
                        const ts_camera* cam, const int32_t* cum_tiles_hit, int64_t capacity, int32_t* bin_ws,
                        int32_t* scratch, void* stream) {
+    return ts_bin_emit_groups_spans(n, xys, radii, splats, nullptr, cam, cum_tiles_hit, capacity, bin_ws, scratch,
+                                    stream);
+}
+
+int ts_bin_emit_groups_spans(int32_t n, const float* xys, const int32_t* radii, const float* splats,
+                             const int32_t* row_spans, const ts_camera* cam, const int32_t* cum_tiles_hit,
+                             int64_t capacity, int32_t* bin_ws, int32_t* scratch, void* stream) {
     if (!cam || !xys || !radii || !cum_tiles_hit || !bin_ws || !scratch) return TS_E_BADARG;
+    if (row_spans && ((uintptr_t)row_spans & 15)) return TS_E_BADARG;
     const int nt = ts_num_tiles(cam);
     if (!one_walk_form(n, nt) || (cam->hints & TS_HINT_BALANCED_WALK)) return TS_E_BADARG;
     const BinGeometry g = bin_geometry(n, nt);
     const size_t lds = (size_t)g.groups * 8 + (size_t)kStageCap * 6;
+    if (row_spans) {
+        (void)hipFuncSetAttribute(reinterpret_cast<const void*>(&bin_scatter_spans_kernel),
+                                  hipFuncAttributeMaxDynamicSharedMemorySize, (int)lds);
+        hipLaunchKernelGGL(bin_scatter_spans_kernel, dim3(g.chunks), dim3(kBinThreads), lds, (hipStream_t)stream, n,
+                           g.chunk, xys, radii, reinterpret_cast<const float4*>(splats),
+                           reinterpret_cast<const int4*>(row_spans), *cam, g.groups, cum_tiles_hit, (long long)capacity,
+                           bin_ws + g.counts, bin_ws + g.starts, scratch);
+        return launch_status();
+    }
     (void)hipFuncSetAttribute(reinterpret_cast<const void*>(&bin_scatter_emit_kernel),
                               hipFuncAttributeMaxDynamicSharedMemorySize, (int)lds);
     hipLaunchKernelGGL(bin_scatter_emit_kernel, dim3(g.chunks), dim3(kBinThreads), lds, (hipStream_t)stream, n, g.chunk,
diff --git a/tinysplat_amd/csrc/frame.hip b/tinysplat_amd/csrc/frame.hip
--- a/tinysplat_amd/csrc/frame.hip
+++ b/tinysplat_amd/csrc/frame.hip
@@ -95,6 +95,9 @@
         ts_bin_one_walk_form(f->n, num_tiles(f)))
         return ListForm::one_walk;
     return ListForm::group;
+}
+inline int32_t* row_spans(const ts_frame* f) {
+    return ((f->flags & TS_FRAME_ROW_SPANS) && list_form(f) == ListForm::one_walk) ? f->row_spans : nullptr;
 }
 inline const float* tight_records(const ts_frame* f) { return (f->flags & TS_FRAME_TIGHT) ? f->splats : nullptr; }
 inline int32_t* longest_word(const ts_frame* f) {
@@ -140,14 +143,14 @@
 int ts_frame_fwd_prepare(const ts_frame* f, void* stream) {
     TsRange range_("ts_frame_fwd_prepare");
     if (bad(f)) return TS_E_BADARG;
+    const float* tight = tight_records(f);
     TS_TRY(TS_ENTRY("ts_colors_pack_fwd",
-                    ts_colors_pack_fwd(f->n, f->sh_degree, f->num_bases, f->means, f->origin, f->colors_dc,
-                                       f->num_bases > 1 ? f->colors_rest : nullptr, f->sh_mask,
-                                       (f->flags & TS_FRAME_STRIPE) ? f->num_tiles_hit : nullptr, f->channels,
-                                       TS_RASTER_LOGIT_OPACITY, f->xys, f->radii, f->conics, f->opacities,
-                                       f->cum_tiles_hit, &f->cam, f->channels == 4 ? f->depths : nullptr, f->splats,
-                                       stream)));
-    const float* tight = tight_records(f);
+                    ts_colors_pack_spans_fwd(f->n, f->sh_degree, f->num_bases, f->means, f->origin, f->colors_dc,
+                                             f->num_bases > 1 ? f->colors_rest : nullptr, f->sh_mask,
+                                             (f->flags & TS_FRAME_STRIPE) ? f->num_tiles_hit : nullptr, f->channels,
+                                             TS_RASTER_LOGIT_OPACITY, f->xys, f->radii, f->conics, f->opacities,
+                                             f->cum_tiles_hit, &f->cam, f->channels == 4 ? f->depths : nullptr,
+                                             f->splats, tight ? 1 : 0, row_spans(f), stream)));
     switch (list_form(f)) {
     case ListForm::one_walk:
         return 0;
@@ -181,8 +184,8 @@
     switch (form) {
     case ListForm::one_walk:
         TS_TRY(TS_ENTRY("ts_bin_scatter",
-                        ts_bin_emit_groups(f->n, f->xys, f->radii, tight, &f->cam, f->cum_tiles_hit, f->capacity,
-                                           f->bin_ws, scratch, stream)));
+                        ts_bin_emit_groups_spans(f->n, f->xys, f->radii, tight, row_spans(f), &f->cam,
+                                                 f->cum_tiles_hit, f->capacity, f->bin_ws, scratch, stream)));
         TS_TRY(TS_ENTRY("ts_tile_offsets",
                         ts_emit_offsets(f->n, num_tiles(f), f->bin_ws, f->tile_bins, f->cum_tiles_hit, f->capacity,
                                         longest_word(f), stream)));
diff --git a/tinysplat_amd/csrc/pack.h b/tinysplat_amd/csrc/pack.h
--- a/tinysplat_amd/csrc/pack.h
+++ b/tinysplat_amd/csrc/pack.h
@@ -3,6 +3,7 @@
 #include <hip/hip_runtime.h>
 
 #include "../../include/tinysplat_hip.h"
+#include "row_spans.h"
 #include "splat_math.h"
 
 namespace ts {
@@ -17,7 +18,50 @@
     const float* depths;
     float4* splats;
     ts_camera cam;
+    int4* row_spans = nullptr;
+    int tight = 0;
 };
+
+struct PackIn {
+    int r;
+    float2 xy;
+    float op, cxx, cxy, cyy;
+};
+
+__device__ __forceinline__ PackIn pack_load(const PackArgs& a, int i) {
+    PackIn in;
+    in.r = a.radii[i];
+    in.xy = reinterpret_cast<const float2*>(a.xys)[i];
+    in.op = a.opacity[i];
+    in.cxx = a.conics[3 * i]; in.cxy = a.conics[3 * i + 1]; in.cyy = a.conics[3 * i + 2];
+    return in;
+}
+__device__ __forceinline__ float pack_opacity(const PackArgs& a, float op) {
+    if (a.flags & TS_RASTER_LOGIT_OPACITY) op = 1.0f / (1.0f + expf(-op));
+    return op;
+}
+
+__device__ __forceinline__ void store_row_spans(const PackArgs& a, int i, const PackIn& in) {
+    const RowSpans s = make_row_spans(a.tight != 0, in.xy.x, in.xy.y, in.op, in.cxx, in.cxy, in.cyy, in.r,
+                                      a.cam.tile_bounds_x, a.cam.tile_bounds_y, a.cam.tile_row0, a.cam.tile_rows);
+    a.row_spans[i] = make_int4((int)s.w[0], (int)s.w[1], (int)s.w[2], (int)s.w[3]);
+}
+
+__device__ __forceinline__ void pack_store(const PackArgs& a, int i, const PackIn& in, float c0, float c1, float c2,
+                                           float c3) {
+    if (in.r <= 0) return;
+    const TileBox b = tile_bbox(in.xy.x, in.xy.y, (float)in.r, a.cam.tile_bounds_x, a.cam.tile_bounds_y,
+                                a.cam.tile_row0, a.cam.tile_rows);
+    const int w = b.maxx - b.minx, h = b.maxy - b.miny;
+    const int cnt = h > 0 ? w * h : 0;
+    if (cnt <= 0) return;
+    const int excl = a.cum_tiles_hit[i] - cnt;
+    const int slot_base = excl - b.miny * w - b.minx;
+    a.splats[3 * (size_t)i] = make_float4(in.xy.x, in.xy.y, in.op, in.cxx);
+    a.splats[3 * (size_t)i + 1] = make_float4(in.cxy, in.cyy, c0, c1);
+    a.splats[3 * (size_t)i + 2] =
+        make_float4(c2, c3, __int_as_float(slot_base), __int_as_float(w | (b.minx << 16)));
+}
 
 __device__ __forceinline__ void pack_one(const PackArgs& a, int i, float c0, float c1, float c2, float c3) {
     const int r = a.radii[i];
diff --git a/tinysplat_amd/csrc/project.hip b/tinysplat_amd/csrc/project.hip
--- a/tinysplat_amd/csrc/project.hip
+++ b/tinysplat_amd/csrc/project.hip
@@ -238,7 +238,7 @@
     }
 }
 
-template <int DEG>
+template <int DEG, bool SPANS>
 __global__ __launch_bounds__(kShThreadsFwd) void sh_colors_fwd_kernel(
     int n, int num_bases, const float* __restrict__ means, const float* __restrict__ origin,
     const float* __restrict__ dc, const float* __restrict__ rest, float* __restrict__ colors,
@@ -250,6 +250,15 @@
     const int g0 = blockIdx.x * kShThreadsFwd;
     const int cnt = min(kShThreadsFwd, n - g0);
     const int tid = threadIdx.x;
+    if (SPANS) __builtin_assume(tid < kShThreadsFwd);
+    ts::PackIn in{};
+    if (SPANS) in = ts::pack_load(pk, min(g0 + tid, n - 1));
+    auto write_spans = [&]() {
+        if (!SPANS) return;
+        in.op = ts::pack_opacity(pk, in.op);
+        if (tid < cnt) ts::store_row_spans(pk, g0 + tid, in);
+    };
+    if (RS == 0) write_spans();
     if (RS > 0) {
         const size_t row = 3 * (size_t)(num_bases - 1);
         const float* src = rest + (size_t)g0 * row;
@@ -263,6 +272,7 @@
                 const int f4 = tid + u * kShThreadsFwd;
                 v[u] = f4 < total4 ? load4_stream(src4 + f4) : make_float4(0.f, 0.f, 0.f, 0.f);
             }
+            write_spans();
 #pragma unroll
             for (int u = 0; u < per; ++u) {
                 const int f4 = tid + u * kShThreadsFwd;
@@ -276,6 +286,7 @@
                 }
             }
         } else {
+            write_spans();
             const int total = cnt * RS;
             for (int f = tid; f < total; f += kShThreadsFwd) {
                 const int g = f / RS, j = f % RS;
@@ -301,7 +312,11 @@
     if (mask) mask[i] = (unsigned char)((c0 >= 0.0f ? 1 : 0) | (c1 >= 0.0f ? 2 : 0) | (c2 >= 0.0f ? 4 : 0));
     c0 = fmaxf(c0, 0.0f); c1 = fmaxf(c1, 0.0f); c2 = fmaxf(c2, 0.0f);
     if (colors) { colors[3 * i] = c0; colors[3 * i + 1] = c1; colors[3 * i + 2] = c2; }
-    if (pk.splats) ts::pack_one(pk, i, c0, c1, c2, pk.channels == 4 ? pk.depths[i] : 0.0f);
+    if (pk.splats) {
+        const float c3 = pk.channels == 4 ? pk.depths[i] : 0.0f;
+        if (SPANS) ts::pack_store(pk, i, in, c0, c1, c2, c3);
+        else ts::pack_one(pk, i, c0, c1, c2, c3);
+    }
 }
 
 template <int DEG>
@@ -311,7 +326,16 @@
     float* __restrict__ colors, unsigned char* __restrict__ mask, const ts::PackArgs pk) {
     constexpr int KA = (DEG + 1) * (DEG + 1);
     const int i = blockIdx.x * kThreads + threadIdx.x;
-    if (i >= n || live[i] == 0) return;
+    if (i >= n) return;
+    if (live[i] == 0) {
+        if (pk.row_spans) pk.row_spans[i] = make_int4(0, 0, 0, 0);
+        return;
+    }
+    if (pk.row_spans) {
+        ts::PackIn in = ts::pack_load(pk, i);
+        in.op = ts::pack_opacity(pk, in.op);
+        ts::store_row_spans(pk, i, in);
+    }
     float Y[KA];
     ts::sh_basis(DEG, means[3 * i] - origin[0], means[3 * i + 1] - origin[1],
                  means[3 * i + 2] - origin[2], Y);
@@ -618,11 +642,12 @@
     const int grid_d = (n + kShThreadsFwd - 1) / kShThreadsFwd;
 #define TS_SHC_FWD(D)                                                                             \
     do {                                                                                          \
+        const auto kernel = pk.row_spans ? sh_colors_fwd_kernel<D, true> : sh_colors_fwd_kernel<D, false>; \
         if (lds > 48 * 1024)                                                                      \
-            (void)hipFuncSetAttribute(reinterpret_cast<const void*>(&sh_colors_fwd_kernel<D>),    \
+            (void)hipFuncSetAttribute(reinterpret_cast<const void*>(kernel),                      \
                                       hipFuncAttributeMaxDynamicSharedMemorySize, (int)lds);      \
-        hipLaunchKernelGGL(sh_colors_fwd_kernel<D>, dim3(grid_d), dim3(kShThreadsFwd), lds, s, n,  \
-                           num_bases, means3d, origin, colors_dc, colors_rest, colors, clamp_mask, pk); \
+        hipLaunchKernelGGL(kernel, dim3(grid_d), dim3(kShThreadsFwd), lds, s, n, num_bases, means3d, origin, \
+                           colors_dc, colors_rest, colors, clamp_mask, pk);                       \
     } while (0)
     switch (degrees_to_use) {
         case 0: TS_SHC_FWD(0); break;
@@ -651,14 +676,27 @@
                        const float* xys, const int32_t* radii, const float* conics, const float* opacity,
                        const int32_t* cum_tiles_hit, const ts_camera* cam, const float* depths,
                        float* splats, void* stream) {
+    return ts_colors_pack_spans_fwd(n, degrees_to_use, num_bases, means3d, origin, colors_dc, colors_rest, clamp_mask,
+                                    live, channels, flags, xys, radii, conics, opacity, cum_tiles_hit, cam, depths,
+                                    splats, 0, nullptr, stream);
+}
+
+int ts_colors_pack_spans_fwd(int32_t n, int32_t degrees_to_use, int32_t num_bases, const float* means3d,
+                             const float* origin, const float* colors_dc, const float* colors_rest,
+                             uint8_t* clamp_mask, const int32_t* live, int32_t channels, int32_t flags,
+                             const float* xys, const int32_t* radii, const float* conics, const float* opacity,
+                             const int32_t* cum_tiles_hit, const ts_camera* cam, const float* depths,
+                             float* splats, int32_t tight, int32_t* row_spans, void* stream) {
     if (n < 0 || !cam || (channels != 3 && channels != 4)) return TS_E_BADARG;
     if (n > 0 && (!xys || !radii || !conics || !opacity || !cum_tiles_hit || !splats ||
                   (channels == 4 && !depths)))
         return TS_E_BADARG;
+    if (row_spans && ((uintptr_t)row_spans & 15)) return TS_E_BADARG;
     ts::PackArgs pk;
     pk.channels = channels; pk.flags = (int)flags; pk.xys = xys; pk.radii = radii; pk.conics = conics;
     pk.opacity = opacity; pk.cum_tiles_hit = cum_tiles_hit; pk.depths = depths;
     pk.splats = reinterpret_cast<float4*>(splats); pk.cam = *cam;
+    pk.row_spans = reinterpret_cast<int4*>(row_spans); pk.tight = tight ? 1 : 0;
     return launch_colors_fwd(n, degrees_to_use, num_bases, means3d, origin, colors_dc, colors_rest, nullptr,
                              clamp_mask, live, pk, stream);
 }
diff --git a/tinysplat_amd/csrc/row_spans.h b/tinysplat_amd/csrc/row_spans.h
--- /dev/null
+++ b/tinysplat_amd/csrc/row_spans.h
@@ -0,0 +1,68 @@
+#pragma once
+
+#include "splat_math.h"
+
+namespace ts {
+
+constexpr int kSpanRows = 6;
+constexpr int kSpanCols = 256;
+constexpr int kSpanFallback = 0xff;
+constexpr unsigned int kSpanEmptyRow = 1u;
+
+struct RowSpans { unsigned int w[4]; };
+
+TS_HD RowSpans spans_none() {
+    RowSpans s;
+    s.w[0] = s.w[1] = s.w[2] = s.w[3] = 0u;
+    return s;
+}
+TS_HD RowSpans spans_fallback() {
+    RowSpans s = spans_none();
+    s.w[0] = (unsigned int)kSpanFallback << 16;
+    return s;
+}
+TS_HD int spans_rows(const RowSpans& s) { return (int)((s.w[0] >> 16) & 0xffu); }
+TS_HD int spans_first_row(const RowSpans& s) { return (int)(s.w[0] & 0xffffu); }
+TS_HD void spans_row(const RowSpans& s, int k, int& lo, int& hi) {
+    const unsigned int v = (s.w[1 + (k >> 1)] >> (16 * (k & 1))) & 0xffffu;
+    lo = (int)(v & 0xffu);
+    hi = (int)(v >> 8) + 1;
+}
+
+TS_HD void spans_pop_row(RowSpans& s, int& lo, int& hi) {
+    lo = (int)(s.w[1] & 0xffu);
+    hi = (int)((s.w[1] >> 8) & 0xffu) + 1;
+    s.w[1] = (s.w[1] >> 16) | (s.w[2] << 16);
+    s.w[2] = (s.w[2] >> 16) | (s.w[3] << 16);
+    s.w[3] >>= 16;
+}
+
+TS_HD RowSpans make_row_spans(bool tight, float x, float y, float op, float cxx, float cxy, float cyy, int radius,
+                              int tile_bounds_x, int tile_bounds_y, int tile_row0, int tile_rows) {
+    if (radius <= 0) return spans_none();
+    const TileBox b = tile_bbox(x, y, (float)radius, tile_bounds_x, tile_bounds_y, tile_row0, tile_rows);
+    if (b.maxy <= b.miny || b.maxx <= b.minx) return spans_none();
+    const TightTest t(tight, x, y, op, cxx, cxy, cyy, (float)radius);
+    if (t.cull_all) return spans_none();
+    const int rows = b.maxy - b.miny, first = b.miny - tile_row0;
+    if (rows > kSpanRows || first > 0xffff) return spans_fallback();
+    RowSpans s = spans_none();
+    s.w[0] = (unsigned int)first | ((unsigned int)rows << 16);
+    bool fits = true;
+#pragma unroll
+    for (int k = 0; k < kSpanRows; ++k) {
+        if (k < rows) {
+            int lo, hi;
+            t.row_range(b.miny + k, b.minx, b.maxx, lo, hi);
+            unsigned int v = kSpanEmptyRow;
+            if (hi > lo) {
+                fits = fits && hi <= kSpanCols;
+                v = (unsigned int)lo | ((unsigned int)(hi - 1) << 8);
+            }
+            s.w[1 + (k >> 1)] |= (v & 0xffffu) << (16 * (k & 1));
+        }
+    }
+    return fits ? s : spans_fallback();
+}
+
+}
diff --git a/tinysplat_amd/frame.py b/tinysplat_amd/frame.py
--- a/tinysplat_amd/frame.py
+++ b/tinysplat_amd/frame.py
@@ -172,6 +172,8 @@
 GROUP_COUNTS = os.environ.get("TS_GROUP_COUNTS", "1") != "0"
 
 ONE_WALK = os.environ.get("TS_ONE_WALK", "1") != "0"
+
+ROW_SPANS = os.environ.get("TS_ROW_SPANS", "1") != "0"
 
 CAPACITY_ALLOC = os.environ.get("TS_CAPACITY_ALLOC", "0") != "0"
 CAPACITY_GROWTH = 1.25
@@ -258,13 +260,14 @@
         f32 = dict(dtype=torch.float32, device=dev)
         i32 = dict(dtype=torch.int32, device=dev)
         px = rows * w
-        lkey = (n, num_tiles, w, rows, ch, keep, cam.hints & 0xFFFF00, cam.wide_tiles, cam.tile_rows, cam.tile_row0, cam.tile_bounds_x, cam.img_height)
+        lkey = (n, num_tiles, w, rows, ch, keep, cam.hints & 0xFFFF00, cam.wide_tiles, cam.tile_rows, cam.tile_row0, cam.tile_bounds_x, cam.img_height,
+                ROW_SPANS)
         lay = _layouts.get(lkey)
         if lay is None:
             nscan = int(lib.ts_scan_ws_ints(n))
             nbin = int(lib.ts_bin_ws_ints(n, num_tiles))
             fin_floats = int(lib.ts_final_floats(ctypes.byref(cam), ch)) if keep else px
-            sizes = [48 * m, 8 * m, 12 * m, 0, 4 * m, 4 * m, 4 * m, 4 * m, 4 * nscan, 4 * nbin,
+            sizes = [48 * m, 8 * m, 12 * m, 16 * m if ROW_SPANS else 0, 4 * m, 4 * m, 4 * m, 4 * m, 4 * nscan, 4 * nbin,
                      8 * max(num_tiles, 1)] + ([m, 4 * fin_floats, 4 * px, px] if keep else [])
             offs, off = [], 0
             for sz in sizes:
@@ -308,6 +311,9 @@
             fr.flags |= _lib.FRAME_GROUP_COUNTS
         if ONE_WALK:
             fr.flags |= _lib.FRAME_ONE_WALK
+        if ROW_SPANS:
+            fr.flags |= _lib.FRAME_ROW_SPANS
+            fr.row_spans = ptr[3]
         if full:
             _stats_mode[dev.index] = mode
         fr.cam = cam
```

New measurement: 2089000 billion Gaussians*pixels/s, median of 6. 1.2% higher.
